# MurpheyLab/trep

Hardware: AMD Instinct MI355X
Metric: DEL-steps/sec x batch (puppet ~40-DOF, fp64) (higher is better)
Workload: dtype f64

## Files before the change

trep_amd/csrc/mvi_core.hpp:

```cpp
#pragma once
#include <cmath>

#include "program.hpp"
#include "dual.hpp"
#include "lanes.hpp"

#if defined(TG_MOCK_TIMING) || defined(TG_MOCK_REAL_LDS) || defined(TG_MOCK_LDS_D1) || defined(TG_MOCK_LDS_D2) || \
    defined(TG_BBD_FUSED_UPDATE) || defined(TG_BBD_INLINE) || defined(TG_BBD_ASM) || \
    defined(TG_WEV_NO_RC_IDENT) || defined(TG_WEV_CLEAR_EARLY) || defined(TG_WEV_MERGE_C) || \
    defined(TG_NO_BBD) || defined(TG_NO_CMP) || defined(TG_NO_GJ_PANEL) || defined(TG_NO_QUAD_SWEEP) || defined(TG_NO_DUAL_SWEEP) || \
    defined(TG_NO_AB_MFMA) || defined(TG_NO_HZ_MFMA) || defined(GJR_EXEC32) || defined(GJP_SKIP_STEPS) || defined(GJP_SKIP_UPDATE) || \
    defined(TG_FRESH_PHASES) || defined(TG_FRESH_STEP) || \
    defined(TG_CHAIN_PRIO) || defined(TG_PREFIX_GROUP) || defined(TG_LT_TRIPS) || defined(TG_ROLLOUT_WAVES) || defined(TG_DERIV_WAVES)
#error "a retired experiment switch is defined (TG_MOCK_*, TG_BBD_FUSED_UPDATE / _INLINE / _ASM, TG_WEV_*, TG_NO_* except TG_NO_WEV, GJR_ / GJP_*, TG_FRESH_*, or a former -D tunable): these variants were removed -- verdicts in docs/LOG.md, their source in commit 89f6ce0"
#endif

#if defined(TG_HELPER_WAVES)
constexpr int TG_NW = TG_HELPER_WAVES;
#else
constexpr int TG_NW = 1;
#endif

#if defined(__HIPCC__)
__device__ __forceinline__ double *tg_lds_base() {
#if defined(__HIP_DEVICE_COMPILE__)
    typedef __attribute__((address_space(3))) double lds_double;
    extern __shared__ double tg_dynamic_lds[];
    if ((__UINTPTR_TYPE__)(lds_double *)tg_dynamic_lds != 0) __builtin_trap();
    return (double *)((lds_double *)(__UINTPTR_TYPE__)8 - 1);
#else
    return nullptr;
#endif
}
#endif

TG_HD int tg_xcd_block(int b, int G) {
    const int q = G >> 3, r = G & 7, x = b & 7, i = b >> 3;
    const int n = q + (x < r ? 1 : 0);
    const int q2 = n >> 5, r2 = n & 31, u = i & 31, s_ = i >> 5;
    return x * q + (x < r ? x : r) + u * q2 + (u < r2 ? u : r2) + s_;
}

#if defined(__HIP_DEVICE_COMPILE__)
__device__ __forceinline__ int tg_opaque(int x) { asm volatile("" : "+v"(x)); return x; }
#else
inline int tg_opaque(int x) { return x; }
#endif
constexpr int TG_CHAIN_PRIO = 2;
constexpr int TG_PREFIX_GROUP = 5;
constexpr int TG_LT_TRIPS = 4;
#define TG_FOR(idx, n) for (int idx = tg_opaque(lane); idx < (n); idx += TEAM)
#define TG_FORW(idx, n) for (int idx = tg_opaque(lane + TEAM * wave); idx < (n); idx += TEAM * nw)

#if defined(TG_PROFILE) && defined(__HIP_DEVICE_COMPILE__)
#define TG_STAMP(id) do { long long t_ = (long long)__builtin_amdgcn_s_memtime(); prof[id] += t_ - prof_last; prof_last = t_; } while (0)
#ifndef TG_PROF_TRAJ
#define TG_PROF_TRAJ 0
#endif
#else
#define TG_STAMP(id) ((void)0)
#endif

#include <type_traits>
#include "bbd_solve.hpp"
#include "gj_solve.hpp"

namespace tg {
template <class P, class = void> struct tg_static_bbd { static constexpr bool value = false; };
template <class P> struct tg_static_bbd<P, typename std::enable_if<(P::bbd_ok >= 0)>::type> { static constexpr bool value = P::bbd_ok != 0; };
template <bool USE, class P, class = void> struct tg_static_bbd_cols { static constexpr int value = 1; };
template <class P> struct tg_static_bbd_cols<true, P, typename std::enable_if<(P::bbd_ok > 0)>::type> { static constexpr int value = P::bbd_ng + P::bbd_nb; };
template <class P, class = void> struct tg_is_spec { static constexpr bool value = false; };
template <class P> struct tg_is_spec<P, typename std::enable_if<(P::nq >= 0)>::type> { static constexpr bool value = true; };
template <class P, class = void> struct tg_items_aligned { static constexpr bool value = false; };
template <class P> struct tg_items_aligned<P, typename std::enable_if<(P::nq >= 0)>::type> { static constexpr bool value = (P::o_J % 2 == 0) && (P::o_W % 2 == 0); };
template <class P, class = void> struct tg_static_sweep { static constexpr bool value = false; };
template <class P> struct tg_static_sweep<P, typename std::enable_if<(P::sw_ok > 0)>::type> { static constexpr bool value = true; };
template <class P, class = void> struct tg_static_cmp { static constexpr bool value = false; };
template <class P> struct tg_static_cmp<P, typename std::enable_if<(P::cmp_ok >= 0)>::type> { static constexpr bool value = P::cmp_ok != 0 && P::tab_ok != 0; };

template <class P, class = void> struct tg_static_wev { static constexpr bool value = false; };
#if !defined(TG_NO_WEV)
template <class P> struct tg_static_wev<P, typename std::enable_if<(P::wev_ok >= 0)>::type> { static constexpr bool value = P::wev_ok != 0 && P::cmp_ok != 0 && P::tab_ok != 0; };
#endif

template <class P, class = void> struct tg_static_pk { static constexpr bool value = false; };
#if defined(TG_BBD_PACKED)
template <class P> struct tg_static_pk<P, typename std::enable_if<(P::bbd_pk_ok >= 0)>::type> { static constexpr bool value = P::bbd_pk_ok != 0 && tg_static_wev<P>::value && tg_static_bbd<P>::value; };
#endif

template <class P, class = void> struct tg_static_fb { static constexpr bool value = false; };
template <class P> struct tg_static_fb<P, typename std::enable_if<(P::fb_on >= 0)>::type> { static constexpr bool value = P::fb_on != 0 && tg_static_wev<P>::value; };

enum { MODE_ROLLOUT = 0, MODE_CALC_P2 = 1, MODE_CALC_F = 2, MODE_DERIV1 = 3, MODE_DERIV2Z = 4, MODE_DYNAMICS = 5, MODE_DYN_DERIV1 = 6, MODE_ENERGY = 7, MODE_LAGRANGIAN = 8 };

struct RunArgs {
    int batch, n_steps, max_iterations, mode;
    int predictor;
    double dt, t1, t2, tolerance;
    double *q1, *q2, *p1, *p2, *lam, *u1;
    const double *U, *K;
    const double *q2_hint, *lam_hint;
    const double *Kproj, *bX, *bU;
    double *Uout;
    int group_size;
    const int *group_map;
    double *X;
    double *f_out;
    double *d1[12];
    double *A_out, *B_out;
    const double *z;
    double *hz;
    int *iters, *status;
    long long *prof_out;
    const double *dt_steps;
    int dt_period;
    int exact_pivot;
    const double *zl;
    const double *dq_in, *ddqk_in;
    double *ddq_out, *lam_out;
    double *g1[8];
    double *energy_out;
    double *lag1_out, *lag2_out;
    double *mirror;
    int remap_len, remap_stride, remap_off, remap_count;
    int *fallbacks;
    const int *seed1, *seed2;
};
struct ParTable {
    const double *rows;
    int group, stride;
};
template <class ARGS> TG_HD int tg_remap_trajectory(const ARGS &A, int i) {
    if (A.remap_len <= 0) return i;
    return i < A.remap_count ? (i / A.remap_len) * A.remap_stride + A.remap_off + i % A.remap_len : A.batch;
}

#if defined(__HIP_DEVICE_COMPILE__)
typedef const __attribute__((address_space(4))) DevProg CProg;
typedef const RunArgs CArgs;
template <class T> __device__ __forceinline__ T &tg_fresh_always(T &r) { T *p = &r; asm volatile("" : "+s"(p)); return *p; }
typedef const __attribute__((address_space(4))) RunArgs KArgs;
__device__ __forceinline__ KArgs &tg_fresh_args(KArgs &r) { return tg_fresh_always(r); }
template <class T> __device__ __forceinline__ T &tg_fresh_args(T &r) { return r; }
template <class T> __device__ __forceinline__ T &tg_rebind(T &r) { return r; }
#else
typedef const DevProg CProg;
typedef const RunArgs CArgs;
typedef const RunArgs KArgs;
template <class T> inline T &tg_fresh_args(T &r) { return r; }
template <class T> inline T &tg_rebind(T &r) { return r; }
#endif

TG_HD void tg_sincos(double x, double *s, double *c) {
    if (!(fabs(x) < 131072.0)) {
#if defined(__HIP_DEVICE_COMPILE__)
        sincos(x, s, c);
#else
        *s = std::sin(x);
        *c = std::cos(x);
#endif
        return;
    }
    const double kf = rint(x * 6.36619772367581382433e-01);
    double r = fma(-kf, 1.57079632673412561417e+00, x);
    r = fma(-kf, 6.07710050630396597660e-11, r);
    const double t = fma(-kf, 2.02226624871116645580e-21, r);
    const double z = t * t;
    const double ps = fma(z, fma(z, fma(z, fma(z, fma(z, 1.58969099521155010221e-10, -2.50507602534068634195e-08),
                      2.75573137070700676789e-06), -1.98412698298579493134e-04), 8.33333333332248946124e-03), -1.66666666666666324348e-01);
    const double sn = fma(t * z, ps, t);
    const double pc = fma(z, fma(z, fma(z, fma(z, fma(z, -1.13596475577881948265e-11, 2.08757232129817482790e-09),
                      -2.75573143513906633035e-07), 2.48015872894767294178e-05), -1.38888888888741095749e-03), 4.16666666666666019037e-02);
    const double cs = fma(z * z, pc, fma(-0.5, z, 1.0));
    const int q = (int)kf & 3;
// ... 75 lines not shown
    TG_HD int n_wpair() const { return SPRINGS ? P.n_wpair : 0; }
    const double *d2w = nullptr;
    PROG &P;
    Real *S;
    int lane;
    int seed1 = -1, seed2 = -1;
    TG_HD Real seeded(double v, int var) const { return tgdual::Seed<Real>::make(v, var == seed1, var == seed2); }
    double dt;
    int oGc;
    int dsA = 0, dsB = 2;
    int jck[2] = {0, 0}, bio[2] = {0, 0}, tck[2][2] = {{0, 0}, {0, 0}}, tpair[4] = {0, 0, 0, 0};
    int sc_rot2 = 0;
    int sj_n = 0;
    bool sj_quads = false;
    int swc[16] = {0, 0, 0, 0, 0, 0, 0, 0, 0, 0, 0, 0, 0, 0, 0, 0}, swr = 0, swcol = 0;
    bool swact = false;
    double tdamp = 0.0;
    const double *par = nullptr;
    template <class PP> TG_HD double grav_of(PP &Pl, int k) const { if constexpr (PAR) return par[k]; else return Pl.grav[k]; }
    template <class PP> TG_HD double damp_of(PP &Pl, int i) const { if constexpr (PAR) return par[3 + i]; else return Pl.damp[i]; }
    int wvl[4] = {0, 0, 0, 0}, wpair[4] = {0, 0, 0, 0};
    int wfb[2] = {0, 0};
    int wdhx[2] = {0, 0}, wrhs = 0, wone = -1;
    double wev_w[6] = {0.0, 0.0, 0.0, 0.0, 0.0, 0.0};
    bool pk_image = false;
    bool wev_on = false;
    long long prof[16] = {0, 0, 0, 0, 0, 0, 0, 0, 0, 0, 0, 0, 0, 0, 0, 0};
    bool rates_ready = false;
    double res_f2 = 0.0;
    bool res_hoff = false;
    long long prof_last = 0;

    bool d1_compact = false;
    int wave = 0, nw = 1;
    TG_HD void wave_part(int first, int split, int last, int &lo, int &hi) const {
        lo = first; hi = last;
        if (nw > 1) { lo = wave ? split : first; hi = wave ? last : split; }
    }
    TG_HD Core(PROG &p, Real *s, int l, double dt_) : P(p), S(s), lane(l), dt(dt_), oGc(p.o_G), inv_dt(1.0 / dt_) {}
    double inv_dt;
    TG_HD double over_dt(double x) const { const double q = x * inv_dt; return fma(fma(-q, dt, x), inv_dt, q); }

    template <class Compute, class Store>
    TG_HD void for_pairs(int n, Compute compute, Store store) {
        for (int i0 = tg_opaque(lane); i0 < n; i0 += 2 * TEAM) {
            const int i1 = i0 + TEAM;
            const bool two = i1 < n;
            const auto r0 = compute(i0);
            const auto r1 = compute(two ? i1 : i0);
            store(i0, r0);
            if (two) store(i1, r1);
        }
    }

    TG_HD Real qval(int sel, int c) const {
        Real a = S[P.o_q1 + c], b = S[P.o_q2 + c];
        return sel == 0 ? 0.5 * (b + a) : (sel == 1 ? a : b);
    }

    TG_HD void init_sweep_schedule(bool rollout = false) {
        if constexpr (PAR) { TG_FOR(i, 4 * P.n_bodies) S[P.o_I + i] = par[i - 4 * P.n_bodies]; }
        else TG_FOR(i, 4 * P.n_bodies) S[P.o_I + i] = P.b_inertia[i];
        TG_FOR(c, P.nc) S[P.o_ctol + c] = P.c_tol[c];
#if defined(__HIP_DEVICE_COMPILE__)
        if constexpr (TEAM == 64 && tg_static_bbd<typename std::remove_cv<PROG>::type>::value) {
            if (rollout) { int *tab = (int *)(S + P.o_bbd); TG_FOR(i, 128) tab[i] = P.bbd_tab[i]; }
        }
        if constexpr (TEAM == 64 && !SPRINGS && tg_static_cmp<typename std::remove_cv<PROG>::type>::value) {
            if (rollout) { int *tab = (int *)(S + P.o_cmpt); TG_FOR(i, P.nd) { const int it = P.cmp_rep[i]; tab[i] = it | (P.it_pack[4 * (size_t)it] << 12) | (P.cmp_grp[i] << 20); } }
        }
        if (TEAM == 64 && P.tab_ok) {
            sj_n = rollout ? P.n_sj : 2 * P.n_joints;
            if (rollout) sc_rot2 = P.n_sj_rot;
            else { int n_rot = 0; for (int j = 0; j < P.n_joints; j++) n_rot += P.j_kind[j] >= TG_RX ? 1 : 0; sc_rot2 = 2 * n_rot; }
            sj_quads = rollout;
            if constexpr (tg_static_sweep<typename std::remove_cv<PROG>::type>::value) {
                typedef typename std::remove_cv<PROG>::type SP;
                if (rollout) {
                    const int l = tg_opaque(lane);
                    swact = l < 60;
                    const int q = swact ? l / 12 : 4, rc = swact ? l - 12 * q : 0;
                    swr = rc >> 2; swcol = rc & 3;
#pragma unroll
                    for (int i = 0; i < 16; i++) swc[i] = (i & 3) < SP::sw_np[i >> 2] ? sw_code<SP>(i * 5, q) : 15;
                }
            }
#pragma unroll
            for (int u = 0; u < 2; u++) {
                const int pos = lane + u * TEAM;
                jck[u] = pos < sj_n ? (rollout ? P.sj_list[pos] : P.sj_full[pos]) : 0;
                const int n = lane + u * TEAM < P.n_dhr ? lane + u * TEAM : 0;
                if (P.n_dhr) { tck[u][0] = P.dhr_pack[8 * (size_t)n] | (P.dhr_pack[8 * (size_t)n + 7] << 8); tck[u][1] = P.dhr_pack[8 * (size_t)n + 1]; }
            }
            const int b = lane < 6 * P.n_bodies ? lane / 6 : 0;
            bio[0] = P.b_item_off[b]; bio[1] = P.b_item_off[b + 1];
            tdamp = damp_of(P, lane < P.nd ? lane : 0);
            if constexpr (tg_static_wev<typename std::remove_cv<PROG>::type>::value) {
                typedef typename std::remove_cv<PROG>::type SP;
                static_assert((SP::n_cmpairs + TEAM - 1) / TEAM <= 4, "eval_world: at most four trips of config pairs");
                if (rollout) {
#pragma unroll
                    for (int i = 0; i < 4; i++) wvl[i] = P.wev_lane[4 * lane + i];
                    constexpr bool FB = tg_static_fb<SP>::value;
                    constexpr int NP = FB ? SP::fb_npairs : SP::n_cmpairs;
                    const int *pairs = FB ? P.fb_pair : P.cmp_pair, *pairsx = FB ? P.fb_pairx : P.wev_pairx;
                    if constexpr (FB) {
#pragma unroll
                        for (int i = 0; i < 3; i++) wvl[i] = P.fb_lane[4 * lane + i];
#pragma unroll
                        for (int i = 0; i < 2; i++) wfb[i] = P.fb_abx[2 * (lane < SP::nd ? lane : 0) + i];
                        if (lane >= SP::nd) wfb[0] = 0;
                    }
                    constexpr int TP = FB ? (NP + TEAM - 1) / TEAM : 4;
#pragma unroll
                    for (int u = 0; u < TP; u++) wpair[u] = pairs[lane + u * TEAM < NP ? lane + u * TEAM : 0];
                    if constexpr (tg_static_pk<SP>::value) {
#pragma unroll
                        for (int u = 0; u < TP; u++) wpair[u] = pairsx[lane + u * TEAM < NP ? lane + u * TEAM : 0];
#pragma unroll
                        for (int u = 0; u < 2; u++) wdhx[u] = P.wev_dhx[lane + u * TEAM < SP::n_dhr ? lane + u * TEAM : 0];
                        wrhs = P.bbd_map[(lane < SP::nf ? lane : 0) * (SP::nf + 1) + SP::nf];
                        wone = lane < SP::bbd_pk_nones ? P.bbd_ones[lane < SP::bbd_pk_nones ? lane : 0] : -1;
                    }
                }
            }
            if (P.n_npairs) { const int *p0 = P.pair4 + 4 * (size_t)(lane < P.n_npairs ? lane : 0); tpair[0] = p0[0]; tpair[1] = p0[1]; tpair[2] = p0[2]; tpair[3] = p0[3]; }
        }
#endif
        if (!P.sched_ok || TEAM != 64) { TG_SYNC(); return; }
        int *sched = (int *)(S + P.o_sched);
        TG_FOR(idx, 16 * P.n_rounds) {
            const int r = idx >> 4, c = P.round_off[r] + (idx & 15);
            int w0 = 0, w1 = -1;
            if (c < P.round_off[r + 1]) {
                w0 = (12 * P.ch_first[c]) | (P.ch_len[c] << 16);
                w1 = P.ch_parent[c] >= 0 ? 12 * P.ch_parent[c] : -1;
            }
            sched[2 * idx] = w0; sched[2 * idx + 1] = w1;
        }
        TG_SYNC();
    }

    TG_HD void pose_sweep(bool on, int sel) {
        Real *sc = S + P.o_sc, *G = S + P.o_G;
        if (on) TG_FOR(j, P.n_joints) {
            const Real x = qval(sel, P.j_cfg[j]);
            if (P.j_kind[j] >= TG_RX) tg_sincos(x, &sc[2 * j], &sc[2 * j + 1]);
            else { sc[2 * j] = x; sc[2 * j + 1] = 0.0; }
        }
        TG_SYNC();
        if (on) {
            const int n12 = 12 * P.n_joints;
            for (int base = lane; base < n12; base += 4 * TEAM) {
                double k0[4], k1[4], k2[4];
                int jj[4];
#pragma unroll
                for (int u = 0; u < 4; u++) {
                    const int idx = base + u * TEAM;
                    const bool ok = idx < n12;
                    const int j = ok ? idx / 12 : 0, e = ok ? idx % 12 : 0;
                    const double *k = P.jcoef + 4 * (size_t)(16 * j + e);
                    k0[u] = k[0]; k1[u] = k[1]; k2[u] = k[2]; jj[u] = j;
                }
#pragma unroll
                for (int u = 0; u < 4; u++) {
                    const int idx = base + u * TEAM;
                    if (idx < n12) G[idx] = k0[u] + k1[u] * sc[2 * jj[u] + 1] + k2[u] * sc[2 * jj[u]];
                }
            }
        }
        TG_SYNC();
#if defined(__HIP_DEVICE_COMPILE__)
        if (TEAM == 64) {
            const int *sched = (const int *)(S + P.o_sched);
            for (int r = 0; r < P.n_rounds; r++) {
                const int nch = P.sched_ok ? 16 : P.round_off[r + 1] - P.round_off[r];
                if (on) TG_FOR(idx, 4 * nch) {
                    const int row = idx & 3;
                    int o0, len, opar;
                    if (P.sched_ok) {
                        const int w0 = sched[2 * (16 * r + (idx >> 2))];
                        opar = sched[2 * (16 * r + (idx >> 2)) + 1];
                        o0 = w0 & 0xFFFF; len = w0 >> 16;
                    } else {
                        const int ch = P.round_off[r] + (idx >> 2);
                        o0 = 12 * P.ch_first[ch]; len = P.ch_len[ch]; opar = P.ch_parent[ch] >= 0 ? 12 * P.ch_parent[ch] : -1;
                    }
                    if (row < 3 && len > 0) {
                        Real p0, p1, p2, p3;
                        if (opar >= 0) { const Real *gp = G + opar + 4 * row; p0 = gp[0]; p1 = gp[1]; p2 = gp[2]; p3 = gp[3]; }
                        else { p0 = row == 0 ? 1.0 : 0.0; p1 = row == 1 ? 1.0 : 0.0; p2 = row == 2 ? 1.0 : 0.0; p3 = 0.0; }
                        Real m[12];
#pragma unroll
                        for (int e = 0; e < 12; e++) m[e] = G[o0 + e];
                        for (int s = 0; s < len; s++) {
                            Real *gj = G + o0 + 12 * s;
                            Real n[12];
                            const Real *gn = s + 1 < len ? gj + 12 : gj;
#pragma unroll
                            for (int e = 0; e < 12; e++) n[e] = gn[e];
                            const Real v0 = p0 * m[0] + p1 * m[4] + p2 * m[8];
                            const Real v1 = p0 * m[1] + p1 * m[5] + p2 * m[9];
                            const Real v2 = p0 * m[2] + p1 * m[6] + p2 * m[10];
                            const Real v3 = p0 * m[3] + p1 * m[7] + p2 * m[11] + p3;
                            Real *out = gj + 4 * row;
                            out[0] = v0; out[1] = v1; out[2] = v2; out[3] = v3;
                            p0 = v0; p1 = v1; p2 = v2; p3 = v3;
#pragma unroll
                            for (int e = 0; e < 12; e++) m[e] = n[e];
                        }
                    }
                }
                TG_SYNC();
            }
            return;
        }
#endif
        for (int L = 1; L < P.n_levels; L++) {
            const int l0 = P.level_off[L], cnt = P.level_off[L + 1] - l0;
            if (on) TG_FOR(idx, 4 * cnt) {
                const int j = P.lvl_joints[l0 + (idx >> 2)], cc = idx & 3;
                if (P.j_parent[j] < 0) continue;
                const Real *gp = G + 12 * P.j_parent[j];
                Real *gj = G + 12 * j;
                const Real m0 = gj[cc], m1 = gj[4 + cc], m2 = gj[8 + cc], u3 = (cc == 3) ? 1.0 : 0.0;
                const Real v0 = gp[0] * m0 + gp[1] * m1 + gp[2] * m2 + u3 * gp[3];
                const Real v1 = gp[4] * m0 + gp[5] * m1 + gp[6] * m2 + u3 * gp[7];
                const Real v2 = gp[8] * m0 + gp[9] * m1 + gp[10] * m2 + u3 * gp[11];
                gj[cc] = v0; gj[4 + cc] = v1; gj[8 + cc] = v2;
            }
            TG_SYNC();
        }
    }

#if defined(__HIP_DEVICE_COMPILE__)
    TG_HD void pose_sweep_dual(bool on, bool rollout_lists) {
        const int sjn = rollout_lists ? P.n_sj : 2 * P.n_joints;
        double *sc = S + P.o_sc, *sc2 = S + P.o_J, *G = S + P.o_G, *G2 = S + P.o_W;
        const int nj = P.n_joints;
        const int n12 = 12 * nj, n24 = 2 * n12;
        SwDesc sw0;
        if constexpr (tg_static_sweep<typename std::remove_cv<PROG>::type>::value) {
            if (rollout_lists) sw0 = sw_fetch<typename std::remove_cv<PROG>::type, 0>((const int *)(S + P.o_sched));
        }
        if (P.tab_ok) {
            double pr[2][12];
#pragma unroll
            for (int u = 0; u < 2; u++) {
                const double *src = P.j_prm + 12 * (size_t)((jck[u] >> 16) & 0xFFF);
#pragma unroll
                for (int e = 0; e < 12; e++) pr[u][e] = src[e];
            }
            if (on) {
#pragma unroll
                for (int u = 0; u < 2; u++) {
                    const int idx = lane + u * TEAM;
                    if (u * TEAM < sjn && idx < sjn) {
                        const bool second = (jck[u] >> 28) != 0;
                        const int j = (jck[u] >> 16) & 0xFFF, kind = (jck[u] >> 12) & 0xF;
                        const double x = qval(second ? dsB : dsA, jck[u] & 0xFFF);
                        const bool rotary = kind >= TG_RX;
                        const int a = rotary ? kind - TG_RX : kind - TG_TX, b = a == 2 ? 0 : a + 1, c = a == 0 ? 2 : a - 1;
                        double *g = (second ? G2 : G) + 12 * j;
                        if (u * TEAM < sc_rot2) {
                            double sn = 0.0, cs = 1.0;
                            if (rotary) tg_sincos(x, &sn, &cs);
                            const double tq = rotary ? 0.0 : x;
#pragma unroll
                            for (int l = 0; l < 3; l++) {
                                const double A_ = pr[u][4 * l], B_ = pr[u][4 * l + 1], C_ = pr[u][4 * l + 2], D_ = pr[u][4 * l + 3];
                                g[4 * l + a] = A_;
                                g[4 * l + b] = rotary ? fma(C_, sn, B_ * cs) : B_;
                                g[4 * l + c] = rotary ? fma(-B_, sn, C_ * cs) : C_;
                                g[4 * l + 3] = fma(A_, tq, D_);
                            }
                        } else {
#pragma unroll
                            for (int l = 0; l < 3; l++) {
                                const double A_ = pr[u][4 * l], B_ = pr[u][4 * l + 1], C_ = pr[u][4 * l + 2], D_ = pr[u][4 * l + 3];
                                g[4 * l + a] = A_; g[4 * l + b] = B_; g[4 * l + c] = C_;
                                g[4 * l + 3] = fma(A_, x, D_);
                            }
                        }
                    }
                }
            }
            TG_SYNC();
            TG_STAMP(5);
            TG_STAMP(15);
        } else {
        constexpr int LT = TG_LT_TRIPS;
        struct Rows { double k0[LT], k1[LT], k2[LT]; int j[LT]; };
        auto rows_of = [&](int first) {
            Rows r;
#pragma unroll
            for (int u = 0; u < LT; u++) {
                const int idx2 = first + u * TEAM;
                const int idx = idx2 < n24 ? (idx2 >= n12 ? idx2 - n12 : idx2) : 0;
                const int j = idx / 12, e = idx % 12;
                const double *k = P.jcoef + 4 * (size_t)(16 * j + e);
                r.k0[u] = k[0]; r.k1[u] = k[1]; r.k2[u] = k[2]; r.j[u] = j;
            }
            return r;
        };
        Rows cur = rows_of(lane);
        if (on) TG_FOR(idx, 2 * nj) {
            const bool second = idx >= nj;
            const int j = second ? idx - nj : idx;
            const double x = qval(second ? dsB : dsA, P.j_cfg[j]);
            double *dst = (second ? sc2 : sc) + 2 * j;
            if (P.j_kind[j] >= TG_RX) tg_sincos(x, &dst[0], &dst[1]);
            else { dst[0] = x; dst[1] = 0.0; }
        }
        TG_SYNC();
        TG_STAMP(5);
        for (int b0 = 0; b0 < n24; b0 += LT * TEAM) {
            const Rows nxt = b0 + LT * TEAM < n24 ? rows_of(b0 + LT * TEAM + lane) : cur;
            if (on) {
#pragma unroll
                for (int u = 0; u < LT; u++) {
                    const int idx2 = b0 + lane + u * TEAM;
                    if (idx2 < n24) {
                        const bool second = idx2 >= n12;
                        const double *scx = second ? sc2 : sc;
                        (second ? G2 : G)[second ? idx2 - n12 : idx2] = cur.k0[u] + cur.k1[u] * scx[2 * cur.j[u] + 1] + cur.k2[u] * scx[2 * cur.j[u]];
                    }
                }
            }
            cur = nxt;
        }
        TG_SYNC();
        TG_STAMP(15);
        }
        const int *sched = (const int *)(S + P.o_sched);
        if constexpr (tg_static_sweep<typename std::remove_cv<PROG>::type>::value) {
            if (rollout_lists) {
                typedef typename std::remove_cv<PROG>::type SP;
                __builtin_amdgcn_s_setprio(TG_CHAIN_PRIO);
                chain_round_quads<SP, 0>(on, sched, sw0);
                __builtin_amdgcn_s_setprio(0);
                return;
            }
        }
        if (P.sched_ok == 2) {
            double *Gh = lane >= 32 ? G2 : G;
            const int slot = (lane & 31) >> 2, row = lane & 3;
            for (int r = 0; r < P.n_rounds; r++) {
                if (on) {
                    const int w0 = sched[2 * (16 * r + slot)];
                    const int opar = sched[2 * (16 * r + slot) + 1];
                    const int o0 = w0 & 0xFFFF, len = w0 >> 16;
                    if (row < 3 && len > 0) {
                        double p0, p1, p2, p3;
                        if (opar >= 0) { const double *gp = Gh + opar + 4 * row; p0 = gp[0]; p1 = gp[1]; p2 = gp[2]; p3 = gp[3]; }
                        else { p0 = row == 0 ? 1.0 : 0.0; p1 = row == 1 ? 1.0 : 0.0; p2 = row == 2 ? 1.0 : 0.0; p3 = 0.0; }
                        double m[12];
#pragma unroll
                        for (int e = 0; e < 12; e++) m[e] = Gh[o0 + e];
                        for (int s = 0; s < len; s++) {
                            double *gj = Gh + o0 + 12 * s;
                            double n[12];
                            const int nx = s + 1 < len ? 12 : 0;
#pragma unroll
                            for (int e = 0; e < 12; e++) n[e] = gj[nx + e];
                            const double v0 = p0 * m[0] + p1 * m[4] + p2 * m[8];
                            const double v1 = p0 * m[1] + p1 * m[5] + p2 * m[9];
                            const double v2 = p0 * m[2] + p1 * m[6] + p2 * m[10];
                            const double v3 = p0 * m[3] + p1 * m[7] + p2 * m[11] + p3;
                            double *out = gj + 4 * row;
                            out[0] = v0; out[1] = v1; out[2] = v2; out[3] = v3;
                            p0 = v0; p1 = v1; p2 = v2; p3 = v3;
#pragma unroll
                            for (int e = 0; e < 12; e++) m[e] = n[e];
                        }
                    }
                }
                TG_SYNC();
            }
            return;
        }
        for (int r = 0; r < P.n_rounds; r++) {
            if (on) TG_FOR(idx, 64) {
                const int row = idx & 3;
                const int w0 = sched[2 * (16 * r + (idx >> 2))];
                const int opar = sched[2 * (16 * r + (idx >> 2)) + 1];
                const int o0 = w0 & 0xFFFF, len = w0 >> 16;
                if (row < 3 && len > 0) {
                    double p0, p1, p2, p3, q0, q1, q2, q3;
                    if (opar >= 0) {
                        const double *gp = G + opar + 4 * row, *gq = G2 + opar + 4 * row;
                        p0 = gp[0]; p1 = gp[1]; p2 = gp[2]; p3 = gp[3]; q0 = gq[0]; q1 = gq[1]; q2 = gq[2]; q3 = gq[3];
                    } else {
                        p0 = q0 = row == 0 ? 1.0 : 0.0; p1 = q1 = row == 1 ? 1.0 : 0.0; p2 = q2 = row == 2 ? 1.0 : 0.0; p3 = q3 = 0.0;
                    }
                    double m[12], h[12];
#pragma unroll
                    for (int e = 0; e < 12; e++) { m[e] = G[o0 + e]; h[e] = G2[o0 + e]; }
                    for (int s = 0; s < len; s++) {
                        double *gj = G + o0 + 12 * s, *hj = G2 + o0 + 12 * s;
                        double n[12], g[12];
                        const int nxt = s + 1 < len ? 12 : 0;
#pragma unroll
                        for (int e = 0; e < 12; e++) { n[e] = gj[nxt + e]; g[e] = hj[nxt + e]; }
                        const double v0 = p0 * m[0] + p1 * m[4] + p2 * m[8];
                        const double w0_ = q0 * h[0] + q1 * h[4] + q2 * h[8];
                        const double v1 = p0 * m[1] + p1 * m[5] + p2 * m[9];
                        const double w1 = q0 * h[1] + q1 * h[5] + q2 * h[9];
                        const double v2 = p0 * m[2] + p1 * m[6] + p2 * m[10];
                        const double w2 = q0 * h[2] + q1 * h[6] + q2 * h[10];
                        const double v3 = p0 * m[3] + p1 * m[7] + p2 * m[11] + p3;
                        const double w3 = q0 * h[3] + q1 * h[7] + q2 * h[11] + q3;
                        double *out = gj + 4 * row, *out2 = hj + 4 * row;
                        out[0] = v0; out[1] = v1; out[2] = v2; out[3] = v3;
                        out2[0] = w0_; out2[1] = w1; out2[2] = w2; out2[3] = w3;
                        p0 = v0; p1 = v1; p2 = v2; p3 = v3; q0 = w0_; q1 = w1; q2 = w2; q3 = w3;
#pragma unroll
                        for (int e = 0; e < 12; e++) { m[e] = n[e]; h[e] = g[e]; }
                    }
                }
            }
            TG_SYNC();
        }
    }
    struct SwDesc { int w0[4], par[4]; };
    template <class SP> TG_HD static int sw_code(int base, int q) {
        auto w = [&](int i) { const int c = SP::sw_inst[base + i]; return c ? (c & 0x1FF) : 15; };
        return q == 0 ? w(0) : q == 1 ? w(1) : q == 2 ? w(2) : q == 3 ? w(3) : w(4);
    }
    template <class SP, int RD> TG_HD SwDesc sw_fetch(const int *sched) const {
        SwDesc d;
#pragma unroll
        for (int ps = 0; ps < 4; ps++) {
            d.w0[ps] = 0; d.par[ps] = -1;
            if (ps < SP::sw_np[RD < 4 ? RD : 0]) {
                const int slot = swc[4 * (RD < 4 ? RD : 0) + ps] & 0xFF;
                d.w0[ps] = sched[2 * (16 * RD + slot)]; d.par[ps] = sched[2 * (16 * RD + slot) + 1];
            }
        }
        return d;
    }
    template <class SP, int RD> TG_HD void chain_round_quads(bool on, const int *sched, const SwDesc &d) {
        if constexpr (RD < SP::n_rounds) {
            constexpr int NP = SP::sw_np[RD], ML = SP::sw_maxlen;
            SwDesc nxt = d;
            if constexpr (RD + 1 < SP::n_rounds) nxt = sw_fetch<SP, RD + 1>(sched);
            const int r = swr, c = swcol;
            const bool act = swact;
            if (on) {
                double m[4][ML][3], p[4];
                int base[4], lim[4];
                const int dead = P.o_sc + (lane < 2 * P.n_joints ? lane : 0);
#pragma unroll
                for (int ps = 0; ps < 4; ps++) {
                    if (ps < NP) {
                        const int set = (swc[4 * RD + ps] >> 8) ? P.o_W : P.o_G, opar = d.par[ps];
                        lim[ps] = act ? d.w0[ps] >> 16 : 0;
                        base[ps] = set + (d.w0[ps] & 0xFFFF);
                        const double pv = S[set + (opar >= 0 ? opar : 0) + 4 * r + c];
                        p[ps] = opar >= 0 ? pv : (r == c ? 1.0 : 0.0);
#pragma unroll
                        for (int s = 0; s < ML; s++) {
                            if (s < SP::sw_len[4 * RD + ps]) {
                                const int o = base[ps] + 12 * s + c;
                                m[ps][s][0] = S[o]; m[ps][s][1] = S[o + 4]; m[ps][s][2] = S[o + 8];
                            }
                        }
                    }
                }
#pragma unroll
                for (int s = 0; s < ML; s++) {
#pragma unroll
                    for (int ps = 0; ps < 4; ps++) {
                        if (ps < NP && s < SP::sw_len[4 * RD + ps]) {
                            const double b0 = tg_quad_bcast<0>(p[ps]), b1 = tg_quad_bcast<1>(p[ps]), b2 = tg_quad_bcast<2>(p[ps]);
                            const double last = c == 3 ? p[ps] : 0.0;
                            const double v = fma(b2, m[ps][s][2], fma(b1, m[ps][s][1], fma(b0, m[ps][s][0], last)));
                            S[s < lim[ps] ? base[ps] + 12 * s + 4 * r + c : dead] = v;
                            p[ps] = v;
                        }
                    }
                }
            }
            TG_SYNC();
            chain_round_quads<SP, RD + 1>(on, sched, nxt);
        }
    }
    TG_HD bool dual_ok() const { return TEAM == 64 && !SPRINGS && P.sched_ok && P.nc > 0 && 6 * P.n_items >= 12 * P.n_joints; }

    TG_HD void eval_both(bool on) {
        if (on) TG_FOR(i, P.nq) S[P.o_dq + i] = (S[P.o_q2 + i] - S[P.o_q1 + i]) / dt;
        TG_SYNC();
        TG_STAMP(0);
        pose_sweep_dual(on, true);
        TG_STAMP(1);
        oGc = P.o_W;
        attach_points(on, true, true);
        constraints(on, 2, true, S + P.o_Dh2, 0);
        oGc = P.o_G;
        TG_STAMP(6);
        jacobians(on);
        TG_STAMP(2);
        velocities(on);
        TG_STAMP(3);
        residual_dyn(on);
        TG_STAMP(4);
    }
    struct AttachTab { double ce[2], c0[2], c1[2], c2[2]; int ga[2]; double o0, o1, o2, orr; int ea; };
    struct ConTab { int e1, e2, type, comp, cfg; double dist; int rec[2][6]; };
    struct ItemTab { int rec[2][4]; };
    struct ResTab { int n0, n1; int look[8]; };
    TG_HD AttachTab fetch_attach() const {
        AttachTab t;
        const int l = tg_opaque(lane);
#pragma unroll
        for (int u = 0; u < 2; u++) {
            const int ii = l + u * TEAM < 12 * P.n_bodies ? l + u * TEAM : 0;
            const double *C = P.at_d + 4 * (size_t)ii;
            t.ce[u] = C[0]; t.c0[u] = C[1]; t.c1[u] = C[2]; t.c2[u] = C[3]; t.ga[u] = P.at_i[ii];
        }
        const int ii = l < 3 * P.n_endpoints ? l : 0;
        const double *o = P.ae_d + 4 * (size_t)ii;
        t.o0 = o[0]; t.o1 = o[1]; t.o2 = o[2]; t.orr = o[3]; t.ea = P.ae_i[ii];
        return t;
    }
    TG_HD ConTab fetch_constraints() const {
        ConTab t;
        const int l = tg_opaque(lane);
        const int c = l < P.nc ? l : 0;
        t.e1 = P.c_e1[c]; t.e2 = P.c_e2[c]; t.type = P.c_type[c]; t.comp = P.c_comp[c]; t.cfg = P.c_cfg[c]; t.dist = P.c_dist[c];
#pragma unroll
        for (int u = 0; u < 2; u++) {
            const int *rec = P.dhr_pack + 8 * (size_t)(l + u * TEAM < P.n_dhr ? l + u * TEAM : 0);
#pragma unroll
            for (int i = 1; i < 6; i++) t.rec[u][i] = rec[i];
            t.rec[u][0] = rec[7];
        }
        return t;
    }
    TG_HD ItemTab fetch_items() const {
        ItemTab t;
        const int l = tg_opaque(lane);
#pragma unroll
        for (int u = 0; u < 2; u++) {
            const int *rec = P.it_pack + 4 * (size_t)(l + u * TEAM < P.n_items ? l + u * TEAM : 0);
#pragma unroll
            for (int i = 0; i < 4; i++) t.rec[u][i] = rec[i];
        }
        return t;
    }
    TG_HD ResTab fetch_residual() const {
        ResTab t;
        const int l = tg_opaque(lane);
        const int i = l < P.nd ? l : 0;
        t.n0 = P.cfg_item_off[i]; t.n1 = P.cfg_item_off[i + 1];
#pragma unroll
        for (int c = 0; c < 8; c++) t.look[c] = c < P.nc ? P.dh_lookup[c * P.nq + i] : -1;
// ... 3381 lines not shown
```

trep_amd/csrc/program.hpp:

```cpp
#pragma once
#include <cmath>
#include <cstdlib>
#include <cstdint>
#include <algorithm>
#include <cstring>
#include <functional>
#include <map>
#include <stdexcept>
#include <string>
#include <vector>

#include "../../include/trep_amd.h"
#include "bbd.hpp"

namespace tg {

struct DevProg {
    int nq, nd, nk, nu, nc, nf, nX;
    int n_joints, n_levels, n_bodies, n_items, n_pairs, n_endpoints, n_dh, n_cf, n_cfgitems;
    double grav[3];
    const int *level_off;
    const int *lvl_joints;
    const int *round_off, *ch_first, *ch_len, *ch_parent;
    int n_rounds, n_chains;
// ... 8 lines not shown
    const double *b_C;
    const double *b_inertia;
    const int *b_item_off;
    const int *b_pair_off;
    const int *it_body;
    const int *it_joint;
    const int *it_cfg;
    const int *pair_a;
    const int *pair_b;
    const int *pair4;
    int n_npairs;
    const int *tri4, *cpair4;
    const int *it_pack, *dh_pack;
    const double *at_d, *ae_d;
    const int *at_i, *ae_i;
    const int *dhr_pack;
    int n_dhr;
    const int *cpath_off, *cpath_items, *dh_pos;
    int n_cpath, o_cps;
    const int *tchunk, *tri_off;
    int n_tchunk, o_tps;
    int n_tri, n_cpair;
    const int *wp_a, *wp_b, *wt_a, *wt_b, *wt_split, *wcp4;
    int wp_split, wc_split;
    const int *cfg_item_off;
    const int *cfg_items;
    const int *it_slot;
    const int *e_anchor;
    const double *e_off;
    const int *c_type, *c_e1, *c_e2, *c_cfg, *c_comp;
    const double *c_dist, *c_tol;
    const int *dh_lookup;
    const int *dh_c, *dh_cfg, *dh_joint, *dh_side;
    const double *damp;
    const int *cf_cfg, *cf_in;
    int o_q1, o_q2, o_p1, o_lam, o_u, o_dq, o_f, o_sc, o_G, o_gB, o_pE, o_J, o_W, o_vB, o_gam, o_Ldq, o_Lddq,
        o_Dh1, o_Dh2, o_Df, o_scal, o_misc, o_dqi, o_nu, o_sched, o_I, o_ctol, gjc_ok;
    int tab_ok;
    int sched_ok;
    int df_ld;
    int dh_ld;
    int lds_per_team;
    int d_o_Dh1, d_o_Dh2, d_o_AUG, d_aug_ld, d_o_T12, d_o_T22, d_nrhs, d_lds_per_team;
    const int *cu_off;
    const double *cs_k, *cs_kq0;
    const double *s_k, *s_x0;
    int n_springs, n_sdh, n_spair, o_sV, o_sH, has_cs;
    int g_nrhs, g_ld, g_o_AUG, g_o_P, g_o_X, g_o_aF, g_o_x, g_lds_per_team, g_max_cu;
    const double *c_nloc;
    int has_plane, o_nE;
    const int *wr_in; const double *wr_const;
    const int *wr_kind;
    const double *wr_Rloc; int o_wR;
    int n_wrenches, n_wdh, n_wpair, o_wF, o_wH, o_wD, e_o_wT, e_o_Hu;
    const double *s_c; int has_damper, o_sX, o_sVq, o_sXX, o_svel, o_sF;
    int n_true_springs, e_o_sT, e_o_sWX, e_o_sWXq;
    const int *tab_i; const double *tab_d; int n_tab_i, n_tab_d;
    int e_o_H11, e_o_H12, e_o_H22, e_o_G1, e_o_w, e_o_zq, e_o_zp, e_o_vec, e_o_vec2, e_lds_per_team;
    const double *cs_c0;
    const int *ncs_i; const double *ncs_mb, *ncs_tab; int n_ncs;
    int cmp_ok, n_cgroups, n_cmpairs, o_cmp, o_csw, o_ccz, o_cmpt;
    int cmp_gmask[32];
    const int *cmp_rep, *cmp_grp, *cmp_goff, *cmp_gbody, *cmp_pair;
    int sw_ok, sw_maxlen;
    int sw_np[4];
    int sw_len[16];
    int sw_inst[80];
    int n_sj, n_sj_rot;
    const int *sj_list;
    const int *sj_full;
    int max_cfg_items;
    int bbd_ok, bbd_g, bbd_ng, bbd_nb, bbd_t, o_bbd;
    int bbd_tvar[16];
    const int *bbd_tab;
    int wev_ok, wev_depth, wev_rc_ident;
    const int *wev_lane;
    int bbd_pk_ok, bbd_pk_nr, bbd_pk_nc2, bbd_pk_tb, bbd_pk_tc2, bbd_pk_xs, bbd_pk_size, bbd_pk_nones;
    const int *bbd_map, *bbd_ones, *wev_pairx, *wev_dhx;
    int fb_n, fb_on, fb_npairs, fb_depth, dhr_sides, dhr_types;
    int fb_cfg[3];
    int fb_axis[3];
    const int *fb_pair, *fb_pairx, *fb_abx, *fb_lane;
    int a_ok, a_o_T12, a_o_AUG, a_aug_ld, a_o_T22, a_lds_per_team;
};

struct HostProgram {
    DevProg p{};
    std::vector<int> level_off, lvl_joints, round_off, ch_first, ch_len, ch_parent, j_parent, j_kind, j_cfg, j_pre_ident;
    std::vector<double> j_pre;
    std::vector<int> b_anchor;
    std::vector<double> b_C, b_inertia;
    std::vector<int> b_item_off, b_pair_off, it_body, it_joint, it_cfg, pair_a, pair_b, cfg_item_off, cfg_items, it_slot, pair4, tri4, cpair4, it_pack, dh_pack, cpath_off, cpath_items, dh_pos, tchunk, tri_off, dhr_pack, at_i, ae_i, sj_list, sj_full;
    std::vector<int> wp_a, wp_b, wt_a, wt_b, wt_split, wcp4;
    std::vector<int> e_anchor;
    std::vector<double> e_off;
    std::vector<int> c_type, c_e1, c_e2, c_cfg, c_comp;
    std::vector<double> c_dist, c_tol;
    std::vector<int> dh_c, dh_cfg, dh_joint, dh_side, dh_lookup, cu_off;
    std::vector<double> damp, cs_k, cs_kq0, cs_c0, s_k, s_x0, s_c, c_nloc, wr_const, wr_Rloc, ncs_mb, ncs_tab;
    std::vector<int> ncs_i, bbd_tab, cmp_rep, cmp_grp, cmp_goff, cmp_gbody, cmp_pair, wev_lane, bbd_map, bbd_ones, wev_pairx, wev_dhx;
    std::vector<int> fb_pair, fb_pairx, fb_abx, fb_lane;
    std::vector<unsigned char> newton_pattern;
    std::vector<int> wr_in, wr_kind;
    std::vector<int> cf_cfg, cf_in;
    std::vector<double> jcoef;
    std::vector<double> at_d, ae_d;
    std::vector<double> j_prm;
    int max_depth = 0;
    std::vector<int> ipool;
    std::vector<double> dpool;
    std::vector<size_t> ioff, doff;
    void pack();
    void bind(DevProg &P, const int *I, const double *D) const;
};

namespace detail {
struct M34 {
    double m[12];
};
inline M34 ident() {
    M34 r{};
    r.m[0] = r.m[5] = r.m[10] = 1.0;
    return r;
}
inline M34 mul(const M34 &a, const M34 &b) {
    M34 r{};
    for (int i = 0; i < 3; i++)
        for (int j = 0; j < 4; j++) {
            double s = (j == 3) ? a.m[4 * i + 3] : 0.0;
            for (int k = 0; k < 3; k++) s += a.m[4 * i + k] * b.m[4 * k + j];
            r.m[4 * i + j] = s;
        }
    return r;
}
inline bool is_ident(const M34 &a) {
    M34 i = ident();
    return std::memcmp(a.m, i.m, sizeof(a.m)) == 0;
}
inline M34 fixed_local(const tg_system_desc *d, int f) {
    int t = d->frame_transform[f];
    M34 r = ident();
    double x = d->frame_value[f];
    if (t == TG_CONST_SE3) {
        std::memcpy(r.m, d->frame_lg + 12 * (size_t)f, sizeof(r.m));
    } else if (t == TG_TX || t == TG_TY || t == TG_TZ) {
        r.m[4 * (t - TG_TX) + 3] = x;
    } else if (t == TG_RX) {
        r.m[5] = std::cos(x); r.m[6] = -std::sin(x); r.m[9] = std::sin(x); r.m[10] = std::cos(x);
    } else if (t == TG_RY) {
        r.m[0] = std::cos(x); r.m[2] = std::sin(x); r.m[8] = -std::sin(x); r.m[10] = std::cos(x);
    } else if (t == TG_RZ) {
        r.m[0] = std::cos(x); r.m[1] = -std::sin(x); r.m[4] = std::sin(x); r.m[5] = std::cos(x);
    }
    return r;
}
}

inline HostProgram build_program(const tg_system_desc *d) {
    using namespace detail;
    HostProgram H;
    const int nfr = d->n_frames, nq = d->n_configs, nd = d->n_dyn, nc = d->n_constraints;
    if (nd + d->n_kin != nq) throw std::runtime_error("n_dyn + n_kin != n_configs");
    for (int f = 0; f < nfr; f++) {
        int t = d->frame_transform[f];
        if (t < TG_WORLD || t > TG_CONST_SE3) throw std::runtime_error("unknown frame transform");
        if (d->frame_config[f] >= 0 && (t < TG_TX || t > TG_RZ)) throw std::runtime_error("config on a non-parametric frame");
        if (f > 0 && (d->frame_parent[f] < 0 || d->frame_parent[f] >= f)) throw std::runtime_error("frames must be listed parent-first");
    }
    std::vector<int> jframes;
    int n_levels = 0;
    for (int f = 0; f < nfr; f++)
        if (d->frame_config[f] >= 0) {
            jframes.push_back(f);
            n_levels = std::max(n_levels, d->config_gen[d->frame_config[f]] + 1);
        }
    std::vector<int> order;
    {
        std::vector<int> vparent(nfr, -1);
        std::vector<int> nearest(nfr, -1);
        for (int f = 1; f < nfr; f++) {
            const int p = d->frame_parent[f];
            vparent[f] = nearest[p];
            nearest[f] = d->frame_config[f] >= 0 ? f : nearest[p];
        }
// ... 626 lines not shown
                    H.fb_abx[2 * b] = (int)((unsigned)m << 30);
                }
                if ((int)H.cmp_pair.size() - P.fb_npairs != closed || listed != closed) throw std::runtime_error("floating-base prefix: pair bookkeeping error");
            }
        }
    }
    {
        const int nf = P.nf;
        H.bbd_tab.assign(128, 0);
        for (int i = 0; i < 16; i++) P.bbd_tvar[i] = 0;
        P.bbd_ok = 0; P.bbd_g = P.bbd_ng = P.bbd_nb = P.bbd_t = 0; P.o_bbd = 0;
        if (nf >= 17 && nf <= 31 && nd >= 2) {
            std::vector<unsigned char> pat((size_t)nf * nf, 0);
            auto mark = [&](int i, int j) { if (i < nf && j < nf) { pat[(size_t)i * nf + j] = 1; pat[(size_t)j * nf + i] = 1; } };
            for (int i = 0; i < nd; i++) mark(i, i);
            for (int n = 0; n < P.n_npairs; n++) mark(H.pair4[4 * n + 2] & 0xFFFF, H.pair4[4 * n + 2] >> 16);
            for (int n = 0; n < n_dh_con; n++) if (H.dh_cfg[n] < nd) mark(H.dh_cfg[n], nd + H.dh_c[n]);
            for (size_t n = (size_t)n_cpair_con; n < H.cpair4.size() / 4; n++) {
                const int ka = H.cpair4[4 * n + 3] & 0xFFFF, kb = H.cpair4[4 * n + 3] >> 16;
                if (ka < nd && kb < nd) mark(ka, kb);
            }
            H.newton_pattern = pat;
            const BbdPlan plan = bbd_plan(nf, nd, pat);
            if (plan.ok && plan.t * (plan.t + 2) <= 12 * nitems) {
                P.bbd_ok = 1; P.bbd_g = plan.g; P.bbd_ng = plan.ng; P.bbd_nb = plan.nb; P.bbd_t = plan.t;
                H.bbd_tab.assign(plan.tab, plan.tab + 128);
                for (int i = 0; i < 16; i++) P.bbd_tvar[i] = plan.tvar[i];
                P.o_bbd = P.lds_per_team;
                P.lds_per_team += 64;
            }
        }
        {
            P.bbd_pk_ok = 0; P.bbd_pk_nr = P.bbd_pk_nc2 = P.bbd_pk_tb = P.bbd_pk_tc2 = P.bbd_pk_xs = P.bbd_pk_size = P.bbd_pk_nones = 0;
            H.bbd_map.assign(1, -1); H.bbd_ones.assign(1, -1); H.wev_pairx.assign(1, 0); H.wev_dhx.assign(1, 0);
            if (P.bbd_ok && P.wev_ok) {
                BbdPlan plan;
                plan.ok = 1; plan.g = P.bbd_g; plan.ng = P.bbd_ng; plan.nb = P.bbd_nb; plan.t = P.bbd_t;
                for (int i = 0; i < 16; i++) plan.tvar[i] = P.bbd_tvar[i];
                for (int i = 0; i < 128; i++) plan.tab[i] = H.bbd_tab[i];
                const BbdPacked K = bbd_pack(plan, nf);
                bool ok = K.ok && K.size <= P.nf * P.df_ld && K.size < 1024 && nd < 64 && P.n_dh < 256 && (int)K.ones.size() <= 64 &&
                          P.bbd_t * (P.bbd_t + 2) <= 17 * nb;
                std::vector<int> pairx, dhx;
                for (int n = 0; n < P.n_cmpairs && ok; n++) {
                    const int a = H.cmp_pair[n] & 0xFFFF, b = H.cmp_pair[n] >> 16;
                    const int ab = K.map[(size_t)a * (nf + 1) + b], ba = K.map[(size_t)b * (nf + 1) + a];
                    if (ab < 0 || ba < 0) { ok = false; break; }
                    pairx.push_back((int)((unsigned)a | ((unsigned)b << 6) | ((unsigned)ab << 12) | ((unsigned)ba << 22)));
                }
                for (int n = 0; n < P.n_dhr && ok; n++) {
                    const int c = H.dhr_pack[8 * (size_t)n], k = H.dhr_pack[8 * (size_t)n + 1], item = H.dhr_pack[8 * (size_t)n + 7];
                    const int kc = K.map[(size_t)k * (nf + 1) + nd + c], ck = K.map[(size_t)(nd + c) * (nf + 1) + k];
                    if (kc < 0 || ck < 0) { ok = false; break; }
                    dhx.push_back(item | (kc << 8) | (ck << 18));
                }
                for (int i = 0; i < nf && ok; i++) if (K.map[(size_t)i * (nf + 1) + nf] < 0) ok = false;
                if (ok) {
                    P.bbd_pk_ok = 1; P.bbd_pk_nr = K.nr; P.bbd_pk_nc2 = K.nc2; P.bbd_pk_tb = K.tb; P.bbd_pk_tc2 = K.tc2; P.bbd_pk_xs = P.o_scal - P.o_Df; P.bbd_pk_size = K.size;
                    P.bbd_pk_nones = K.ones[0] < 0 ? 0 : (int)K.ones.size();
                    H.bbd_map = K.map; H.bbd_ones = K.ones; H.wev_pairx = pairx.empty() ? std::vector<int>(1, 0) : pairx; H.wev_dhx = dhx.empty() ? std::vector<int>(1, 0) : dhx;
                    if (P.fb_on) {
                        H.fb_pairx.clear();
                        for (int w : H.fb_pair) {
                            const int a = w & 0xFFFF, b = w >> 16;
                            H.fb_pairx.push_back((int)((unsigned)a | ((unsigned)b << 6) | ((unsigned)K.map[(size_t)a * (nf + 1) + b] << 12) | ((unsigned)K.map[(size_t)b * (nf + 1) + a] << 22)));
                        }
                        for (int b = 0; b < nd; b++) {
                            const int m = (int)((unsigned)H.fb_abx[2 * b] >> 30);
                            unsigned at[6] = {0, 0, 0, 0, 0, 0};
                            for (int i = 0; i < m; i++) { at[2 * i] = (unsigned)K.map[(size_t)P.fb_cfg[i] * (nf + 1) + b]; at[2 * i + 1] = (unsigned)K.map[(size_t)b * (nf + 1) + P.fb_cfg[i]]; }
                            H.fb_abx[2 * b] = (int)(at[0] | (at[1] << 10) | (at[2] << 20) | ((unsigned)m << 30));
                            H.fb_abx[2 * b + 1] = (int)(at[3] | (at[4] << 10) | (at[5] << 20));
                        }
                    }
                }
            }
        }
        if (P.cmp_ok) {
            P.o_cmpt = P.lds_per_team;
            P.lds_per_team += (nd + 1) / 2;
            P.lds_per_team = (P.lds_per_team + 1) & ~1;
        }
    }
    H.pack();
    return H;
}

}

namespace tg {
namespace detail {
template <typename T>
inline void pool_append(std::vector<T> &pool, std::vector<size_t> &offs, const std::vector<T> &v) {
    offs.push_back(pool.size());
    pool.insert(pool.end(), v.begin(), v.end());
    while (pool.size() % 4) pool.push_back(T());
}
}

#define TG_INT_TABLES(X)                                                                                     \
    X(level_off) X(lvl_joints) X(round_off) X(ch_first) X(ch_len) X(ch_parent) X(j_parent) X(j_kind) X(j_cfg) X(j_pre_ident) X(b_anchor) X(b_item_off) X(b_pair_off) X(it_body) \
    X(it_joint) X(it_cfg) X(pair_a) X(pair_b) X(cfg_item_off) X(cfg_items) X(e_anchor) X(c_type) X(c_e1) X(c_e2) \
    X(c_cfg) X(c_comp) X(dh_c) X(dh_cfg) X(dh_joint) X(dh_side) X(cf_cfg) X(cf_in) X(dh_lookup) X(cu_off) X(it_slot) X(pair4) \
    X(tri4) X(cpair4) X(it_pack) X(dh_pack) X(cpath_off) X(cpath_items) X(dh_pos) X(tchunk) X(tri_off) X(wr_in) X(wr_kind) X(ncs_i) \
    X(wp_a) X(wp_b) X(wt_a) X(wt_b) X(wt_split) X(wcp4) X(bbd_tab) X(cmp_rep) X(cmp_grp) X(cmp_goff) X(cmp_gbody) X(cmp_pair) X(dhr_pack) X(at_i) X(ae_i) X(sj_list) X(sj_full) X(wev_lane) X(bbd_map) X(bbd_ones) X(wev_pairx) X(wev_dhx) \
    X(fb_pair) X(fb_pairx) X(fb_abx) X(fb_lane)
#define TG_DBL_TABLES(X) X(j_pre) X(jcoef) X(j_prm) X(at_d) X(ae_d) X(b_C) X(b_inertia) X(e_off) X(c_dist) X(c_tol) X(damp) X(cs_k) X(cs_kq0) X(cs_c0) X(s_k) X(s_x0) X(c_nloc) X(wr_const) X(s_c) X(wr_Rloc) X(ncs_mb) X(ncs_tab)

inline void HostProgram::pack() {
    ipool.clear(); dpool.clear(); ioff.clear(); doff.clear();
#define X(name) detail::pool_append(ipool, ioff, name);
    TG_INT_TABLES(X)
#undef X
#define X(name) detail::pool_append(dpool, doff, name);
    TG_DBL_TABLES(X)
#undef X
    ipool.push_back(0); dpool.push_back(0.0);
}

inline void HostProgram::bind(DevProg &P, const int *I, const double *D) const {
    size_t k = 0;
#define X(name) P.name = I + ioff[k++];
    TG_INT_TABLES(X)
#undef X
    k = 0;
#define X(name) P.name = D + doff[k++];
    TG_DBL_TABLES(X)
#undef X
    P.tab_i = I; P.tab_d = D; P.n_tab_i = (int)ipool.size(); P.n_tab_d = (int)dpool.size();
}
}
```

trep_amd/csrc/spec_emit.inc:

```
static void emit_spec_header(const tg::HostProgram &H, std::string &out) {
    char line[256];
    tg::DevProg P = H.p;
    H.bind(P, H.ipool.data(), H.dpool.data());
    out += "// specialised schedule: sizes, counts, LDS offsets and tables as compile-time constants\n";
    std::snprintf(line, sizeof(line), "__device__ const int spec_ipool[%zu] = {", H.ipool.size() ? H.ipool.size() : (size_t)1); out += line;
    for (size_t i = 0; i < H.ipool.size(); i++) { std::snprintf(line, sizeof(line), "%s%d", i ? ((i % 32) ? "," : ",\n") : "\n", H.ipool[i]); out += line; }
    if (H.ipool.empty()) out += "0";
    out += "};\n";
    std::snprintf(line, sizeof(line), "__device__ const double spec_dpool[%zu] = {", H.dpool.size() ? H.dpool.size() : (size_t)1); out += line;
    for (size_t i = 0; i < H.dpool.size(); i++) { std::snprintf(line, sizeof(line), "%s%a", i ? ((i % 8) ? "," : ",\n") : "\n", H.dpool[i]); out += line; }
    if (H.dpool.empty()) out += "0";
    out += "};\n";
    out += "struct SpecProg {\n";
    std::snprintf(line, sizeof(line), "    static constexpr int nq = %d;\n", P.nq); out += line;
    std::snprintf(line, sizeof(line), "    static constexpr int nd = %d;\n", P.nd); out += line;
    std::snprintf(line, sizeof(line), "    static constexpr int nk = %d;\n", P.nk); out += line;
    std::snprintf(line, sizeof(line), "    static constexpr int nu = %d;\n", P.nu); out += line;
    std::snprintf(line, sizeof(line), "    static constexpr int nc = %d;\n", P.nc); out += line;
    std::snprintf(line, sizeof(line), "    static constexpr int nf = %d;\n", P.nf); out += line;
    std::snprintf(line, sizeof(line), "    static constexpr int nX = %d;\n", P.nX); out += line;
    std::snprintf(line, sizeof(line), "    static constexpr int n_joints = %d;\n", P.n_joints); out += line;
    std::snprintf(line, sizeof(line), "    static constexpr int n_levels = %d;\n", P.n_levels); out += line;
    std::snprintf(line, sizeof(line), "    static constexpr int n_bodies = %d;\n", P.n_bodies); out += line;
    std::snprintf(line, sizeof(line), "    static constexpr int n_items = %d;\n", P.n_items); out += line;
// ... 65 lines not shown
    std::snprintf(line, sizeof(line), "    static constexpr int g_ld = %d;\n", P.g_ld); out += line;
    std::snprintf(line, sizeof(line), "    static constexpr int g_o_AUG = %d;\n", P.g_o_AUG); out += line;
    std::snprintf(line, sizeof(line), "    static constexpr int g_o_P = %d;\n", P.g_o_P); out += line;
    std::snprintf(line, sizeof(line), "    static constexpr int g_o_X = %d;\n", P.g_o_X); out += line;
    std::snprintf(line, sizeof(line), "    static constexpr int g_o_aF = %d;\n", P.g_o_aF); out += line;
    std::snprintf(line, sizeof(line), "    static constexpr int g_o_x = %d;\n", P.g_o_x); out += line;
    std::snprintf(line, sizeof(line), "    static constexpr int g_lds_per_team = %d;\n", P.g_lds_per_team); out += line;
    std::snprintf(line, sizeof(line), "    static constexpr int g_max_cu = %d;\n", P.g_max_cu); out += line;
    std::snprintf(line, sizeof(line), "    static constexpr int has_plane = %d;\n", P.has_plane); out += line;
    std::snprintf(line, sizeof(line), "    static constexpr int o_nE = %d;\n", P.o_nE); out += line;
    std::snprintf(line, sizeof(line), "    static constexpr int o_wR = %d;\n", P.o_wR); out += line;
    std::snprintf(line, sizeof(line), "    static constexpr int n_wrenches = %d;\n", P.n_wrenches); out += line;
    std::snprintf(line, sizeof(line), "    static constexpr int n_wdh = %d;\n", P.n_wdh); out += line;
    std::snprintf(line, sizeof(line), "    static constexpr int n_wpair = %d;\n", P.n_wpair); out += line;
    std::snprintf(line, sizeof(line), "    static constexpr int o_wF = %d;\n", P.o_wF); out += line;
    std::snprintf(line, sizeof(line), "    static constexpr int o_wH = %d;\n", P.o_wH); out += line;
    std::snprintf(line, sizeof(line), "    static constexpr int o_wD = %d;\n", P.o_wD); out += line;
    std::snprintf(line, sizeof(line), "    static constexpr int e_o_wT = %d;\n", P.e_o_wT); out += line;
    std::snprintf(line, sizeof(line), "    static constexpr int e_o_Hu = %d;\n", P.e_o_Hu); out += line;
    std::snprintf(line, sizeof(line), "    static constexpr int has_damper = %d;\n", P.has_damper); out += line;
    std::snprintf(line, sizeof(line), "    static constexpr int o_sX = %d;\n", P.o_sX); out += line;
    std::snprintf(line, sizeof(line), "    static constexpr int o_sVq = %d;\n", P.o_sVq); out += line;
    std::snprintf(line, sizeof(line), "    static constexpr int o_sXX = %d;\n", P.o_sXX); out += line;
    std::snprintf(line, sizeof(line), "    static constexpr int o_svel = %d;\n", P.o_svel); out += line;
    std::snprintf(line, sizeof(line), "    static constexpr int o_sF = %d;\n", P.o_sF); out += line;
    std::snprintf(line, sizeof(line), "    static constexpr int n_true_springs = %d;\n", P.n_true_springs); out += line;
    std::snprintf(line, sizeof(line), "    static constexpr int e_o_sT = %d;\n", P.e_o_sT); out += line;
    std::snprintf(line, sizeof(line), "    static constexpr int e_o_sWX = %d;\n", P.e_o_sWX); out += line;
    std::snprintf(line, sizeof(line), "    static constexpr int e_o_sWXq = %d;\n", P.e_o_sWXq); out += line;
    std::snprintf(line, sizeof(line), "    static constexpr int n_tab_i = %d;\n", P.n_tab_i); out += line;
    std::snprintf(line, sizeof(line), "    static constexpr int n_tab_d = %d;\n", P.n_tab_d); out += line;
    std::snprintf(line, sizeof(line), "    static constexpr int e_o_H11 = %d;\n", P.e_o_H11); out += line;
    std::snprintf(line, sizeof(line), "    static constexpr int e_o_H12 = %d;\n", P.e_o_H12); out += line;
    std::snprintf(line, sizeof(line), "    static constexpr int e_o_H22 = %d;\n", P.e_o_H22); out += line;
    std::snprintf(line, sizeof(line), "    static constexpr int e_o_G1 = %d;\n", P.e_o_G1); out += line;
    std::snprintf(line, sizeof(line), "    static constexpr int e_o_w = %d;\n", P.e_o_w); out += line;
    std::snprintf(line, sizeof(line), "    static constexpr int e_o_zq = %d;\n", P.e_o_zq); out += line;
    std::snprintf(line, sizeof(line), "    static constexpr int e_o_zp = %d;\n", P.e_o_zp); out += line;
    std::snprintf(line, sizeof(line), "    static constexpr int e_o_vec = %d;\n", P.e_o_vec); out += line;
    std::snprintf(line, sizeof(line), "    static constexpr int e_o_vec2 = %d;\n", P.e_o_vec2); out += line;
    std::snprintf(line, sizeof(line), "    static constexpr int e_lds_per_team = %d;\n", P.e_lds_per_team); out += line;
    std::snprintf(line, sizeof(line), "    static constexpr int n_ncs = %d;\n", P.n_ncs); out += line;
    std::snprintf(line, sizeof(line), "    static constexpr int cmp_ok = %d;\n", P.cmp_ok); out += line;
    std::snprintf(line, sizeof(line), "    static constexpr int n_cgroups = %d;\n", P.n_cgroups); out += line;
    std::snprintf(line, sizeof(line), "    static constexpr int n_cmpairs = %d;\n", P.n_cmpairs); out += line;
    std::snprintf(line, sizeof(line), "    static constexpr int o_cmp = %d;\n", P.o_cmp); out += line;
    std::snprintf(line, sizeof(line), "    static constexpr int o_csw = %d;\n", P.o_csw); out += line;
    std::snprintf(line, sizeof(line), "    static constexpr int o_ccz = %d;\n", P.o_ccz); out += line;
    std::snprintf(line, sizeof(line), "    static constexpr int o_cmpt = %d;\n", P.o_cmpt); out += line;
    std::snprintf(line, sizeof(line), "    static constexpr int sw_ok = %d;\n", P.sw_ok); out += line;
    std::snprintf(line, sizeof(line), "    static constexpr int sw_maxlen = %d;\n", P.sw_maxlen); out += line;
    std::snprintf(line, sizeof(line), "    static constexpr int n_sj = %d;\n", P.n_sj); out += line;
    std::snprintf(line, sizeof(line), "    static constexpr int n_sj_rot = %d;\n", P.n_sj_rot); out += line;
    std::snprintf(line, sizeof(line), "    static constexpr int max_cfg_items = %d;\n", P.max_cfg_items); out += line;
    std::snprintf(line, sizeof(line), "    static constexpr int bbd_ok = %d;\n", P.bbd_ok); out += line;
    std::snprintf(line, sizeof(line), "    static constexpr int bbd_g = %d;\n", P.bbd_g); out += line;
    std::snprintf(line, sizeof(line), "    static constexpr int bbd_ng = %d;\n", P.bbd_ng); out += line;
    std::snprintf(line, sizeof(line), "    static constexpr int bbd_nb = %d;\n", P.bbd_nb); out += line;
    std::snprintf(line, sizeof(line), "    static constexpr int bbd_t = %d;\n", P.bbd_t); out += line;
    std::snprintf(line, sizeof(line), "    static constexpr int o_bbd = %d;\n", P.o_bbd); out += line;
    std::snprintf(line, sizeof(line), "    static constexpr int wev_ok = %d;\n", P.wev_ok); out += line;
    std::snprintf(line, sizeof(line), "    static constexpr int wev_depth = %d;\n", P.wev_depth); out += line;
    std::snprintf(line, sizeof(line), "    static constexpr int wev_rc_ident = %d;\n", P.wev_rc_ident); out += line;
    std::snprintf(line, sizeof(line), "    static constexpr int bbd_pk_ok = %d;\n", P.bbd_pk_ok); out += line;
    std::snprintf(line, sizeof(line), "    static constexpr int bbd_pk_nr = %d;\n", P.bbd_pk_nr); out += line;
    std::snprintf(line, sizeof(line), "    static constexpr int bbd_pk_nc2 = %d;\n", P.bbd_pk_nc2); out += line;
    std::snprintf(line, sizeof(line), "    static constexpr int bbd_pk_tb = %d;\n", P.bbd_pk_tb); out += line;
    std::snprintf(line, sizeof(line), "    static constexpr int bbd_pk_tc2 = %d;\n", P.bbd_pk_tc2); out += line;
    std::snprintf(line, sizeof(line), "    static constexpr int bbd_pk_xs = %d;\n", P.bbd_pk_xs); out += line;
    std::snprintf(line, sizeof(line), "    static constexpr int bbd_pk_size = %d;\n", P.bbd_pk_size); out += line;
    std::snprintf(line, sizeof(line), "    static constexpr int bbd_pk_nones = %d;\n", P.bbd_pk_nones); out += line;
    std::snprintf(line, sizeof(line), "    static constexpr int fb_n = %d;\n", P.fb_n); out += line;
    std::snprintf(line, sizeof(line), "    static constexpr int fb_on = %d;\n", P.fb_on); out += line;
    std::snprintf(line, sizeof(line), "    static constexpr int fb_npairs = %d;\n", P.fb_npairs); out += line;
    std::snprintf(line, sizeof(line), "    static constexpr int fb_depth = %d;\n", P.fb_depth); out += line;
    std::snprintf(line, sizeof(line), "    static constexpr int dhr_sides = %d;\n", P.dhr_sides); out += line;
    std::snprintf(line, sizeof(line), "    static constexpr int dhr_types = %d;\n", P.dhr_types); out += line;
    std::snprintf(line, sizeof(line), "    static constexpr int a_ok = %d;\n", P.a_ok); out += line;
    std::snprintf(line, sizeof(line), "    static constexpr int a_o_T12 = %d;\n", P.a_o_T12); out += line;
    std::snprintf(line, sizeof(line), "    static constexpr int a_o_AUG = %d;\n", P.a_o_AUG); out += line;
    std::snprintf(line, sizeof(line), "    static constexpr int a_aug_ld = %d;\n", P.a_aug_ld); out += line;
    std::snprintf(line, sizeof(line), "    static constexpr int a_o_T22 = %d;\n", P.a_o_T22); out += line;
    std::snprintf(line, sizeof(line), "    static constexpr int a_lds_per_team = %d;\n", P.a_lds_per_team); out += line;
    std::snprintf(line, sizeof(line), "    static constexpr double grav_0 = %a;\n", P.grav[0]); out += line;
    std::snprintf(line, sizeof(line), "    static constexpr double grav_1 = %a;\n", P.grav[1]); out += line;
    std::snprintf(line, sizeof(line), "    static constexpr double grav_2 = %a;\n", P.grav[2]); out += line;
    out += "    struct grav_t { __host__ __device__ constexpr double operator[](int i) const { return i == 0 ? grav_0 : i == 1 ? grav_1 : grav_2; } };\n";
    out += "    static constexpr grav_t grav{};\n";
    std::snprintf(line, sizeof(line), "    static constexpr int cmp_gmask_0 = %d;\n", P.cmp_gmask[0]); out += line;
    std::snprintf(line, sizeof(line), "    static constexpr int cmp_gmask_1 = %d;\n", P.cmp_gmask[1]); out += line;
    std::snprintf(line, sizeof(line), "    static constexpr int cmp_gmask_2 = %d;\n", P.cmp_gmask[2]); out += line;
    std::snprintf(line, sizeof(line), "    static constexpr int cmp_gmask_3 = %d;\n", P.cmp_gmask[3]); out += line;
    std::snprintf(line, sizeof(line), "    static constexpr int cmp_gmask_4 = %d;\n", P.cmp_gmask[4]); out += line;
    std::snprintf(line, sizeof(line), "    static constexpr int cmp_gmask_5 = %d;\n", P.cmp_gmask[5]); out += line;
    std::snprintf(line, sizeof(line), "    static constexpr int cmp_gmask_6 = %d;\n", P.cmp_gmask[6]); out += line;
    std::snprintf(line, sizeof(line), "    static constexpr int cmp_gmask_7 = %d;\n", P.cmp_gmask[7]); out += line;
    std::snprintf(line, sizeof(line), "    static constexpr int cmp_gmask_8 = %d;\n", P.cmp_gmask[8]); out += line;
    std::snprintf(line, sizeof(line), "    static constexpr int cmp_gmask_9 = %d;\n", P.cmp_gmask[9]); out += line;
    std::snprintf(line, sizeof(line), "    static constexpr int cmp_gmask_10 = %d;\n", P.cmp_gmask[10]); out += line;
    std::snprintf(line, sizeof(line), "    static constexpr int cmp_gmask_11 = %d;\n", P.cmp_gmask[11]); out += line;
    std::snprintf(line, sizeof(line), "    static constexpr int cmp_gmask_12 = %d;\n", P.cmp_gmask[12]); out += line;
    std::snprintf(line, sizeof(line), "    static constexpr int cmp_gmask_13 = %d;\n", P.cmp_gmask[13]); out += line;
    std::snprintf(line, sizeof(line), "    static constexpr int cmp_gmask_14 = %d;\n", P.cmp_gmask[14]); out += line;
    std::snprintf(line, sizeof(line), "    static constexpr int cmp_gmask_15 = %d;\n", P.cmp_gmask[15]); out += line;
    std::snprintf(line, sizeof(line), "    static constexpr int cmp_gmask_16 = %d;\n", P.cmp_gmask[16]); out += line;
    std::snprintf(line, sizeof(line), "    static constexpr int cmp_gmask_17 = %d;\n", P.cmp_gmask[17]); out += line;
    std::snprintf(line, sizeof(line), "    static constexpr int cmp_gmask_18 = %d;\n", P.cmp_gmask[18]); out += line;
    std::snprintf(line, sizeof(line), "    static constexpr int cmp_gmask_19 = %d;\n", P.cmp_gmask[19]); out += line;
    std::snprintf(line, sizeof(line), "    static constexpr int cmp_gmask_20 = %d;\n", P.cmp_gmask[20]); out += line;
    std::snprintf(line, sizeof(line), "    static constexpr int cmp_gmask_21 = %d;\n", P.cmp_gmask[21]); out += line;
    std::snprintf(line, sizeof(line), "    static constexpr int cmp_gmask_22 = %d;\n", P.cmp_gmask[22]); out += line;
    std::snprintf(line, sizeof(line), "    static constexpr int cmp_gmask_23 = %d;\n", P.cmp_gmask[23]); out += line;
    std::snprintf(line, sizeof(line), "    static constexpr int cmp_gmask_24 = %d;\n", P.cmp_gmask[24]); out += line;
    std::snprintf(line, sizeof(line), "    static constexpr int cmp_gmask_25 = %d;\n", P.cmp_gmask[25]); out += line;
    std::snprintf(line, sizeof(line), "    static constexpr int cmp_gmask_26 = %d;\n", P.cmp_gmask[26]); out += line;
    std::snprintf(line, sizeof(line), "    static constexpr int cmp_gmask_27 = %d;\n", P.cmp_gmask[27]); out += line;
    std::snprintf(line, sizeof(line), "    static constexpr int cmp_gmask_28 = %d;\n", P.cmp_gmask[28]); out += line;
    std::snprintf(line, sizeof(line), "    static constexpr int cmp_gmask_29 = %d;\n", P.cmp_gmask[29]); out += line;
    std::snprintf(line, sizeof(line), "    static constexpr int cmp_gmask_30 = %d;\n", P.cmp_gmask[30]); out += line;
    std::snprintf(line, sizeof(line), "    static constexpr int cmp_gmask_31 = %d;\n", P.cmp_gmask[31]); out += line;
    out += "    struct cmp_gmask_t { __host__ __device__ constexpr int operator[](int i) const { return i == 0 ? cmp_gmask_0 : i == 1 ? cmp_gmask_1 : i == 2 ? cmp_gmask_2 : i == 3 ? cmp_gmask_3 : i == 4 ? cmp_gmask_4 : i == 5 ? cmp_gmask_5 : i == 6 ? cmp_gmask_6 : i == 7 ? cmp_gmask_7 : i == 8 ? cmp_gmask_8 : i == 9 ? cmp_gmask_9 : i == 10 ? cmp_gmask_10 : i == 11 ? cmp_gmask_11 : i == 12 ? cmp_gmask_12 : i == 13 ? cmp_gmask_13 : i == 14 ? cmp_gmask_14 : i == 15 ? cmp_gmask_15 : i == 16 ? cmp_gmask_16 : i == 17 ? cmp_gmask_17 : i == 18 ? cmp_gmask_18 : i == 19 ? cmp_gmask_19 : i == 20 ? cmp_gmask_20 : i == 21 ? cmp_gmask_21 : i == 22 ? cmp_gmask_22 : i == 23 ? cmp_gmask_23 : i == 24 ? cmp_gmask_24 : i == 25 ? cmp_gmask_25 : i == 26 ? cmp_gmask_26 : i == 27 ? cmp_gmask_27 : i == 28 ? cmp_gmask_28 : i == 29 ? cmp_gmask_29 : i == 30 ? cmp_gmask_30 : cmp_gmask_31; } };\n";
    out += "    static constexpr cmp_gmask_t cmp_gmask{};\n";
    std::snprintf(line, sizeof(line), "    static constexpr int sw_np_0 = %d;\n", P.sw_np[0]); out += line;
    std::snprintf(line, sizeof(line), "    static constexpr int sw_np_1 = %d;\n", P.sw_np[1]); out += line;
    std::snprintf(line, sizeof(line), "    static constexpr int sw_np_2 = %d;\n", P.sw_np[2]); out += line;
    std::snprintf(line, sizeof(line), "    static constexpr int sw_np_3 = %d;\n", P.sw_np[3]); out += line;
    out += "    struct sw_np_t { __host__ __device__ constexpr int operator[](int i) const { return i == 0 ? sw_np_0 : i == 1 ? sw_np_1 : i == 2 ? sw_np_2 : sw_np_3; } };\n";
    out += "    static constexpr sw_np_t sw_np{};\n";
    std::snprintf(line, sizeof(line), "    static constexpr int sw_len_0 = %d;\n", P.sw_len[0]); out += line;
    std::snprintf(line, sizeof(line), "    static constexpr int sw_len_1 = %d;\n", P.sw_len[1]); out += line;
    std::snprintf(line, sizeof(line), "    static constexpr int sw_len_2 = %d;\n", P.sw_len[2]); out += line;
    std::snprintf(line, sizeof(line), "    static constexpr int sw_len_3 = %d;\n", P.sw_len[3]); out += line;
    std::snprintf(line, sizeof(line), "    static constexpr int sw_len_4 = %d;\n", P.sw_len[4]); out += line;
    std::snprintf(line, sizeof(line), "    static constexpr int sw_len_5 = %d;\n", P.sw_len[5]); out += line;
    std::snprintf(line, sizeof(line), "    static constexpr int sw_len_6 = %d;\n", P.sw_len[6]); out += line;
    std::snprintf(line, sizeof(line), "    static constexpr int sw_len_7 = %d;\n", P.sw_len[7]); out += line;
    std::snprintf(line, sizeof(line), "    static constexpr int sw_len_8 = %d;\n", P.sw_len[8]); out += line;
    std::snprintf(line, sizeof(line), "    static constexpr int sw_len_9 = %d;\n", P.sw_len[9]); out += line;
    std::snprintf(line, sizeof(line), "    static constexpr int sw_len_10 = %d;\n", P.sw_len[10]); out += line;
    std::snprintf(line, sizeof(line), "    static constexpr int sw_len_11 = %d;\n", P.sw_len[11]); out += line;
    std::snprintf(line, sizeof(line), "    static constexpr int sw_len_12 = %d;\n", P.sw_len[12]); out += line;
    std::snprintf(line, sizeof(line), "    static constexpr int sw_len_13 = %d;\n", P.sw_len[13]); out += line;
    std::snprintf(line, sizeof(line), "    static constexpr int sw_len_14 = %d;\n", P.sw_len[14]); out += line;
    std::snprintf(line, sizeof(line), "    static constexpr int sw_len_15 = %d;\n", P.sw_len[15]); out += line;
    out += "    struct sw_len_t { __host__ __device__ constexpr int operator[](int i) const { return i == 0 ? sw_len_0 : i == 1 ? sw_len_1 : i == 2 ? sw_len_2 : i == 3 ? sw_len_3 : i == 4 ? sw_len_4 : i == 5 ? sw_len_5 : i == 6 ? sw_len_6 : i == 7 ? sw_len_7 : i == 8 ? sw_len_8 : i == 9 ? sw_len_9 : i == 10 ? sw_len_10 : i == 11 ? sw_len_11 : i == 12 ? sw_len_12 : i == 13 ? sw_len_13 : i == 14 ? sw_len_14 : sw_len_15; } };\n";
    out += "    static constexpr sw_len_t sw_len{};\n";
    std::snprintf(line, sizeof(line), "    static constexpr int sw_inst_0 = %d;\n", P.sw_inst[0]); out += line;
    std::snprintf(line, sizeof(line), "    static constexpr int sw_inst_1 = %d;\n", P.sw_inst[1]); out += line;
    std::snprintf(line, sizeof(line), "    static constexpr int sw_inst_2 = %d;\n", P.sw_inst[2]); out += line;
    std::snprintf(line, sizeof(line), "    static constexpr int sw_inst_3 = %d;\n", P.sw_inst[3]); out += line;
    std::snprintf(line, sizeof(line), "    static constexpr int sw_inst_4 = %d;\n", P.sw_inst[4]); out += line;
    std::snprintf(line, sizeof(line), "    static constexpr int sw_inst_5 = %d;\n", P.sw_inst[5]); out += line;
    std::snprintf(line, sizeof(line), "    static constexpr int sw_inst_6 = %d;\n", P.sw_inst[6]); out += line;
    std::snprintf(line, sizeof(line), "    static constexpr int sw_inst_7 = %d;\n", P.sw_inst[7]); out += line;
    std::snprintf(line, sizeof(line), "    static constexpr int sw_inst_8 = %d;\n", P.sw_inst[8]); out += line;
    std::snprintf(line, sizeof(line), "    static constexpr int sw_inst_9 = %d;\n", P.sw_inst[9]); out += line;
    std::snprintf(line, sizeof(line), "    static constexpr int sw_inst_10 = %d;\n", P.sw_inst[10]); out += line;
    std::snprintf(line, sizeof(line), "    static constexpr int sw_inst_11 = %d;\n", P.sw_inst[11]); out += line;
    std::snprintf(line, sizeof(line), "    static constexpr int sw_inst_12 = %d;\n", P.sw_inst[12]); out += line;
    std::snprintf(line, sizeof(line), "    static constexpr int sw_inst_13 = %d;\n", P.sw_inst[13]); out += line;
    std::snprintf(line, sizeof(line), "    static constexpr int sw_inst_14 = %d;\n", P.sw_inst[14]); out += line;
    std::snprintf(line, sizeof(line), "    static constexpr int sw_inst_15 = %d;\n", P.sw_inst[15]); out += line;
    std::snprintf(line, sizeof(line), "    static constexpr int sw_inst_16 = %d;\n", P.sw_inst[16]); out += line;
    std::snprintf(line, sizeof(line), "    static constexpr int sw_inst_17 = %d;\n", P.sw_inst[17]); out += line;
    std::snprintf(line, sizeof(line), "    static constexpr int sw_inst_18 = %d;\n", P.sw_inst[18]); out += line;
    std::snprintf(line, sizeof(line), "    static constexpr int sw_inst_19 = %d;\n", P.sw_inst[19]); out += line;
// ... 7 lines not shown
    std::snprintf(line, sizeof(line), "    static constexpr int sw_inst_27 = %d;\n", P.sw_inst[27]); out += line;
    std::snprintf(line, sizeof(line), "    static constexpr int sw_inst_28 = %d;\n", P.sw_inst[28]); out += line;
    std::snprintf(line, sizeof(line), "    static constexpr int sw_inst_29 = %d;\n", P.sw_inst[29]); out += line;
    std::snprintf(line, sizeof(line), "    static constexpr int sw_inst_30 = %d;\n", P.sw_inst[30]); out += line;
    std::snprintf(line, sizeof(line), "    static constexpr int sw_inst_31 = %d;\n", P.sw_inst[31]); out += line;
    std::snprintf(line, sizeof(line), "    static constexpr int sw_inst_32 = %d;\n", P.sw_inst[32]); out += line;
    std::snprintf(line, sizeof(line), "    static constexpr int sw_inst_33 = %d;\n", P.sw_inst[33]); out += line;
    std::snprintf(line, sizeof(line), "    static constexpr int sw_inst_34 = %d;\n", P.sw_inst[34]); out += line;
    std::snprintf(line, sizeof(line), "    static constexpr int sw_inst_35 = %d;\n", P.sw_inst[35]); out += line;
    std::snprintf(line, sizeof(line), "    static constexpr int sw_inst_36 = %d;\n", P.sw_inst[36]); out += line;
    std::snprintf(line, sizeof(line), "    static constexpr int sw_inst_37 = %d;\n", P.sw_inst[37]); out += line;
    std::snprintf(line, sizeof(line), "    static constexpr int sw_inst_38 = %d;\n", P.sw_inst[38]); out += line;
    std::snprintf(line, sizeof(line), "    static constexpr int sw_inst_39 = %d;\n", P.sw_inst[39]); out += line;
    std::snprintf(line, sizeof(line), "    static constexpr int sw_inst_40 = %d;\n", P.sw_inst[40]); out += line;
    std::snprintf(line, sizeof(line), "    static constexpr int sw_inst_41 = %d;\n", P.sw_inst[41]); out += line;
    std::snprintf(line, sizeof(line), "    static constexpr int sw_inst_42 = %d;\n", P.sw_inst[42]); out += line;
    std::snprintf(line, sizeof(line), "    static constexpr int sw_inst_43 = %d;\n", P.sw_inst[43]); out += line;
    std::snprintf(line, sizeof(line), "    static constexpr int sw_inst_44 = %d;\n", P.sw_inst[44]); out += line;
    std::snprintf(line, sizeof(line), "    static constexpr int sw_inst_45 = %d;\n", P.sw_inst[45]); out += line;
    std::snprintf(line, sizeof(line), "    static constexpr int sw_inst_46 = %d;\n", P.sw_inst[46]); out += line;
    std::snprintf(line, sizeof(line), "    static constexpr int sw_inst_47 = %d;\n", P.sw_inst[47]); out += line;
    std::snprintf(line, sizeof(line), "    static constexpr int sw_inst_48 = %d;\n", P.sw_inst[48]); out += line;
    std::snprintf(line, sizeof(line), "    static constexpr int sw_inst_49 = %d;\n", P.sw_inst[49]); out += line;
    std::snprintf(line, sizeof(line), "    static constexpr int sw_inst_50 = %d;\n", P.sw_inst[50]); out += line;
    std::snprintf(line, sizeof(line), "    static constexpr int sw_inst_51 = %d;\n", P.sw_inst[51]); out += line;
    std::snprintf(line, sizeof(line), "    static constexpr int sw_inst_52 = %d;\n", P.sw_inst[52]); out += line;
    std::snprintf(line, sizeof(line), "    static constexpr int sw_inst_53 = %d;\n", P.sw_inst[53]); out += line;
    std::snprintf(line, sizeof(line), "    static constexpr int sw_inst_54 = %d;\n", P.sw_inst[54]); out += line;
    std::snprintf(line, sizeof(line), "    static constexpr int sw_inst_55 = %d;\n", P.sw_inst[55]); out += line;
    std::snprintf(line, sizeof(line), "    static constexpr int sw_inst_56 = %d;\n", P.sw_inst[56]); out += line;
    std::snprintf(line, sizeof(line), "    static constexpr int sw_inst_57 = %d;\n", P.sw_inst[57]); out += line;
    std::snprintf(line, sizeof(line), "    static constexpr int sw_inst_58 = %d;\n", P.sw_inst[58]); out += line;
    std::snprintf(line, sizeof(line), "    static constexpr int sw_inst_59 = %d;\n", P.sw_inst[59]); out += line;
    std::snprintf(line, sizeof(line), "    static constexpr int sw_inst_60 = %d;\n", P.sw_inst[60]); out += line;
    std::snprintf(line, sizeof(line), "    static constexpr int sw_inst_61 = %d;\n", P.sw_inst[61]); out += line;
    std::snprintf(line, sizeof(line), "    static constexpr int sw_inst_62 = %d;\n", P.sw_inst[62]); out += line;
    std::snprintf(line, sizeof(line), "    static constexpr int sw_inst_63 = %d;\n", P.sw_inst[63]); out += line;
    std::snprintf(line, sizeof(line), "    static constexpr int sw_inst_64 = %d;\n", P.sw_inst[64]); out += line;
    std::snprintf(line, sizeof(line), "    static constexpr int sw_inst_65 = %d;\n", P.sw_inst[65]); out += line;
    std::snprintf(line, sizeof(line), "    static constexpr int sw_inst_66 = %d;\n", P.sw_inst[66]); out += line;
    std::snprintf(line, sizeof(line), "    static constexpr int sw_inst_67 = %d;\n", P.sw_inst[67]); out += line;
    std::snprintf(line, sizeof(line), "    static constexpr int sw_inst_68 = %d;\n", P.sw_inst[68]); out += line;
    std::snprintf(line, sizeof(line), "    static constexpr int sw_inst_69 = %d;\n", P.sw_inst[69]); out += line;
    std::snprintf(line, sizeof(line), "    static constexpr int sw_inst_70 = %d;\n", P.sw_inst[70]); out += line;
    std::snprintf(line, sizeof(line), "    static constexpr int sw_inst_71 = %d;\n", P.sw_inst[71]); out += line;
    std::snprintf(line, sizeof(line), "    static constexpr int sw_inst_72 = %d;\n", P.sw_inst[72]); out += line;
    std::snprintf(line, sizeof(line), "    static constexpr int sw_inst_73 = %d;\n", P.sw_inst[73]); out += line;
    std::snprintf(line, sizeof(line), "    static constexpr int sw_inst_74 = %d;\n", P.sw_inst[74]); out += line;
    std::snprintf(line, sizeof(line), "    static constexpr int sw_inst_75 = %d;\n", P.sw_inst[75]); out += line;
    std::snprintf(line, sizeof(line), "    static constexpr int sw_inst_76 = %d;\n", P.sw_inst[76]); out += line;
    std::snprintf(line, sizeof(line), "    static constexpr int sw_inst_77 = %d;\n", P.sw_inst[77]); out += line;
    std::snprintf(line, sizeof(line), "    static constexpr int sw_inst_78 = %d;\n", P.sw_inst[78]); out += line;
    std::snprintf(line, sizeof(line), "    static constexpr int sw_inst_79 = %d;\n", P.sw_inst[79]); out += line;
    out += "    struct sw_inst_t { __host__ __device__ constexpr int operator[](int i) const { return i == 0 ? sw_inst_0 : i == 1 ? sw_inst_1 : i == 2 ? sw_inst_2 : i == 3 ? sw_inst_3 : i == 4 ? sw_inst_4 : i == 5 ? sw_inst_5 : i == 6 ? sw_inst_6 : i == 7 ? sw_inst_7 : i == 8 ? sw_inst_8 : i == 9 ? sw_inst_9 : i == 10 ? sw_inst_10 : i == 11 ? sw_inst_11 : i == 12 ? sw_inst_12 : i == 13 ? sw_inst_13 : i == 14 ? sw_inst_14 : i == 15 ? sw_inst_15 : i == 16 ? sw_inst_16 : i == 17 ? sw_inst_17 : i == 18 ? sw_inst_18 : i == 19 ? sw_inst_19 : i == 20 ? sw_inst_20 : i == 21 ? sw_inst_21 : i == 22 ? sw_inst_22 : i == 23 ? sw_inst_23 : i == 24 ? sw_inst_24 : i == 25 ? sw_inst_25 : i == 26 ? sw_inst_26 : i == 27 ? sw_inst_27 : i == 28 ? sw_inst_28 : i == 29 ? sw_inst_29 : i == 30 ? sw_inst_30 : i == 31 ? sw_inst_31 : i == 32 ? sw_inst_32 : i == 33 ? sw_inst_33 : i == 34 ? sw_inst_34 : i == 35 ? sw_inst_35 : i == 36 ? sw_inst_36 : i == 37 ? sw_inst_37 : i == 38 ? sw_inst_38 : i == 39 ? sw_inst_39 : i == 40 ? sw_inst_40 : i == 41 ? sw_inst_41 : i == 42 ? sw_inst_42 : i == 43 ? sw_inst_43 : i == 44 ? sw_inst_44 : i == 45 ? sw_inst_45 : i == 46 ? sw_inst_46 : i == 47 ? sw_inst_47 : i == 48 ? sw_inst_48 : i == 49 ? sw_inst_49 : i == 50 ? sw_inst_50 : i == 51 ? sw_inst_51 : i == 52 ? sw_inst_52 : i == 53 ? sw_inst_53 : i == 54 ? sw_inst_54 : i == 55 ? sw_inst_55 : i == 56 ? sw_inst_56 : i == 57 ? sw_inst_57 : i == 58 ? sw_inst_58 : i == 59 ? sw_inst_59 : i == 60 ? sw_inst_60 : i == 61 ? sw_inst_61 : i == 62 ? sw_inst_62 : i == 63 ? sw_inst_63 : i == 64 ? sw_inst_64 : i == 65 ? sw_inst_65 : i == 66 ? sw_inst_66 : i == 67 ? sw_inst_67 : i == 68 ? sw_inst_68 : i == 69 ? sw_inst_69 : i == 70 ? sw_inst_70 : i == 71 ? sw_inst_71 : i == 72 ? sw_inst_72 : i == 73 ? sw_inst_73 : i == 74 ? sw_inst_74 : i == 75 ? sw_inst_75 : i == 76 ? sw_inst_76 : i == 77 ? sw_inst_77 : i == 78 ? sw_inst_78 : sw_inst_79; } };\n";
    out += "    static constexpr sw_inst_t sw_inst{};\n";
    std::snprintf(line, sizeof(line), "    static constexpr int bbd_tvar_0 = %d;\n", P.bbd_tvar[0]); out += line;
    std::snprintf(line, sizeof(line), "    static constexpr int bbd_tvar_1 = %d;\n", P.bbd_tvar[1]); out += line;
    std::snprintf(line, sizeof(line), "    static constexpr int bbd_tvar_2 = %d;\n", P.bbd_tvar[2]); out += line;
    std::snprintf(line, sizeof(line), "    static constexpr int bbd_tvar_3 = %d;\n", P.bbd_tvar[3]); out += line;
    std::snprintf(line, sizeof(line), "    static constexpr int bbd_tvar_4 = %d;\n", P.bbd_tvar[4]); out += line;
    std::snprintf(line, sizeof(line), "    static constexpr int bbd_tvar_5 = %d;\n", P.bbd_tvar[5]); out += line;
    std::snprintf(line, sizeof(line), "    static constexpr int bbd_tvar_6 = %d;\n", P.bbd_tvar[6]); out += line;
    std::snprintf(line, sizeof(line), "    static constexpr int bbd_tvar_7 = %d;\n", P.bbd_tvar[7]); out += line;
    std::snprintf(line, sizeof(line), "    static constexpr int bbd_tvar_8 = %d;\n", P.bbd_tvar[8]); out += line;
    std::snprintf(line, sizeof(line), "    static constexpr int bbd_tvar_9 = %d;\n", P.bbd_tvar[9]); out += line;
    std::snprintf(line, sizeof(line), "    static constexpr int bbd_tvar_10 = %d;\n", P.bbd_tvar[10]); out += line;
    std::snprintf(line, sizeof(line), "    static constexpr int bbd_tvar_11 = %d;\n", P.bbd_tvar[11]); out += line;
    std::snprintf(line, sizeof(line), "    static constexpr int bbd_tvar_12 = %d;\n", P.bbd_tvar[12]); out += line;
    std::snprintf(line, sizeof(line), "    static constexpr int bbd_tvar_13 = %d;\n", P.bbd_tvar[13]); out += line;
    std::snprintf(line, sizeof(line), "    static constexpr int bbd_tvar_14 = %d;\n", P.bbd_tvar[14]); out += line;
    std::snprintf(line, sizeof(line), "    static constexpr int bbd_tvar_15 = %d;\n", P.bbd_tvar[15]); out += line;
    out += "    struct bbd_tvar_t { __host__ __device__ constexpr int operator[](int i) const { return i == 0 ? bbd_tvar_0 : i == 1 ? bbd_tvar_1 : i == 2 ? bbd_tvar_2 : i == 3 ? bbd_tvar_3 : i == 4 ? bbd_tvar_4 : i == 5 ? bbd_tvar_5 : i == 6 ? bbd_tvar_6 : i == 7 ? bbd_tvar_7 : i == 8 ? bbd_tvar_8 : i == 9 ? bbd_tvar_9 : i == 10 ? bbd_tvar_10 : i == 11 ? bbd_tvar_11 : i == 12 ? bbd_tvar_12 : i == 13 ? bbd_tvar_13 : i == 14 ? bbd_tvar_14 : bbd_tvar_15; } };\n";
    out += "    static constexpr bbd_tvar_t bbd_tvar{};\n";
    std::snprintf(line, sizeof(line), "    static constexpr int fb_cfg_0 = %d;\n", P.fb_cfg[0]); out += line;
    std::snprintf(line, sizeof(line), "    static constexpr int fb_cfg_1 = %d;\n", P.fb_cfg[1]); out += line;
    std::snprintf(line, sizeof(line), "    static constexpr int fb_cfg_2 = %d;\n", P.fb_cfg[2]); out += line;
    out += "    struct fb_cfg_t { __host__ __device__ constexpr int operator[](int i) const { return i == 0 ? fb_cfg_0 : i == 1 ? fb_cfg_1 : fb_cfg_2; } };\n";
    out += "    static constexpr fb_cfg_t fb_cfg{};\n";
    std::snprintf(line, sizeof(line), "    static constexpr int fb_axis_0 = %d;\n", P.fb_axis[0]); out += line;
    std::snprintf(line, sizeof(line), "    static constexpr int fb_axis_1 = %d;\n", P.fb_axis[1]); out += line;
    std::snprintf(line, sizeof(line), "    static constexpr int fb_axis_2 = %d;\n", P.fb_axis[2]); out += line;
    out += "    struct fb_axis_t { __host__ __device__ constexpr int operator[](int i) const { return i == 0 ? fb_axis_0 : i == 1 ? fb_axis_1 : fb_axis_2; } };\n";
    out += "    static constexpr fb_axis_t fb_axis{};\n";
    if (P.level_off) { std::snprintf(line, sizeof(line), "    static constexpr const int *level_off = spec_ipool + %zu;\n", (size_t)(P.level_off - H.ipool.data())); out += line; }
    else out += "    static constexpr const int *level_off = nullptr;\n";
    if (P.lvl_joints) { std::snprintf(line, sizeof(line), "    static constexpr const int *lvl_joints = spec_ipool + %zu;\n", (size_t)(P.lvl_joints - H.ipool.data())); out += line; }
    else out += "    static constexpr const int *lvl_joints = nullptr;\n";
    if (P.round_off) { std::snprintf(line, sizeof(line), "    static constexpr const int *round_off = spec_ipool + %zu;\n", (size_t)(P.round_off - H.ipool.data())); out += line; }
    else out += "    static constexpr const int *round_off = nullptr;\n";
    if (P.ch_first) { std::snprintf(line, sizeof(line), "    static constexpr const int *ch_first = spec_ipool + %zu;\n", (size_t)(P.ch_first - H.ipool.data())); out += line; }
    else out += "    static constexpr const int *ch_first = nullptr;\n";
    if (P.ch_len) { std::snprintf(line, sizeof(line), "    static constexpr const int *ch_len = spec_ipool + %zu;\n", (size_t)(P.ch_len - H.ipool.data())); out += line; }
    else out += "    static constexpr const int *ch_len = nullptr;\n";
    if (P.ch_parent) { std::snprintf(line, sizeof(line), "    static constexpr const int *ch_parent = spec_ipool + %zu;\n", (size_t)(P.ch_parent - H.ipool.data())); out += line; }
    else out += "    static constexpr const int *ch_parent = nullptr;\n";
    if (P.j_parent) { std::snprintf(line, sizeof(line), "    static constexpr const int *j_parent = spec_ipool + %zu;\n", (size_t)(P.j_parent - H.ipool.data())); out += line; }
    else out += "    static constexpr const int *j_parent = nullptr;\n";
    if (P.j_kind) { std::snprintf(line, sizeof(line), "    static constexpr const int *j_kind = spec_ipool + %zu;\n", (size_t)(P.j_kind - H.ipool.data())); out += line; }
    else out += "    static constexpr const int *j_kind = nullptr;\n";
    if (P.j_cfg) { std::snprintf(line, sizeof(line), "    static constexpr const int *j_cfg = spec_ipool + %zu;\n", (size_t)(P.j_cfg - H.ipool.data())); out += line; }
    else out += "    static constexpr const int *j_cfg = nullptr;\n";
    if (P.j_pre_ident) { std::snprintf(line, sizeof(line), "    static constexpr const int *j_pre_ident = spec_ipool + %zu;\n", (size_t)(P.j_pre_ident - H.ipool.data())); out += line; }
    else out += "    static constexpr const int *j_pre_ident = nullptr;\n";
    if (P.j_pre) { std::snprintf(line, sizeof(line), "    static constexpr const double *j_pre = spec_dpool + %zu;\n", (size_t)(P.j_pre - H.dpool.data())); out += line; }
    else out += "    static constexpr const double *j_pre = nullptr;\n";
    if (P.jcoef) { std::snprintf(line, sizeof(line), "    static constexpr const double *jcoef = spec_dpool + %zu;\n", (size_t)(P.jcoef - H.dpool.data())); out += line; }
    else out += "    static constexpr const double *jcoef = nullptr;\n";
    if (P.j_prm) { std::snprintf(line, sizeof(line), "    static constexpr const double *j_prm = spec_dpool + %zu;\n", (size_t)(P.j_prm - H.dpool.data())); out += line; }
    else out += "    static constexpr const double *j_prm = nullptr;\n";
    if (P.b_anchor) { std::snprintf(line, sizeof(line), "    static constexpr const int *b_anchor = spec_ipool + %zu;\n", (size_t)(P.b_anchor - H.ipool.data())); out += line; }
    else out += "    static constexpr const int *b_anchor = nullptr;\n";
    if (P.b_C) { std::snprintf(line, sizeof(line), "    static constexpr const double *b_C = spec_dpool + %zu;\n", (size_t)(P.b_C - H.dpool.data())); out += line; }
    else out += "    static constexpr const double *b_C = nullptr;\n";
    if (P.b_inertia) { std::snprintf(line, sizeof(line), "    static constexpr const double *b_inertia = spec_dpool + %zu;\n", (size_t)(P.b_inertia - H.dpool.data())); out += line; }
    else out += "    static constexpr const double *b_inertia = nullptr;\n";
    if (P.b_item_off) { std::snprintf(line, sizeof(line), "    static constexpr const int *b_item_off = spec_ipool + %zu;\n", (size_t)(P.b_item_off - H.ipool.data())); out += line; }
    else out += "    static constexpr const int *b_item_off = nullptr;\n";
    if (P.b_pair_off) { std::snprintf(line, sizeof(line), "    static constexpr const int *b_pair_off = spec_ipool + %zu;\n", (size_t)(P.b_pair_off - H.ipool.data())); out += line; }
    else out += "    static constexpr const int *b_pair_off = nullptr;\n";
    if (P.it_body) { std::snprintf(line, sizeof(line), "    static constexpr const int *it_body = spec_ipool + %zu;\n", (size_t)(P.it_body - H.ipool.data())); out += line; }
    else out += "    static constexpr const int *it_body = nullptr;\n";
    if (P.it_joint) { std::snprintf(line, sizeof(line), "    static constexpr const int *it_joint = spec_ipool + %zu;\n", (size_t)(P.it_joint - H.ipool.data())); out += line; }
    else out += "    static constexpr const int *it_joint = nullptr;\n";
    if (P.it_cfg) { std::snprintf(line, sizeof(line), "    static constexpr const int *it_cfg = spec_ipool + %zu;\n", (size_t)(P.it_cfg - H.ipool.data())); out += line; }
    else out += "    static constexpr const int *it_cfg = nullptr;\n";
    if (P.pair_a) { std::snprintf(line, sizeof(line), "    static constexpr const int *pair_a = spec_ipool + %zu;\n", (size_t)(P.pair_a - H.ipool.data())); out += line; }
    else out += "    static constexpr const int *pair_a = nullptr;\n";
    if (P.pair_b) { std::snprintf(line, sizeof(line), "    static constexpr const int *pair_b = spec_ipool + %zu;\n", (size_t)(P.pair_b - H.ipool.data())); out += line; }
    else out += "    static constexpr const int *pair_b = nullptr;\n";
    if (P.pair4) { std::snprintf(line, sizeof(line), "    static constexpr const int *pair4 = spec_ipool + %zu;\n", (size_t)(P.pair4 - H.ipool.data())); out += line; }
    else out += "    static constexpr const int *pair4 = nullptr;\n";
    if (P.tri4) { std::snprintf(line, sizeof(line), "    static constexpr const int *tri4 = spec_ipool + %zu;\n", (size_t)(P.tri4 - H.ipool.data())); out += line; }
    else out += "    static constexpr const int *tri4 = nullptr;\n";
    if (P.cpair4) { std::snprintf(line, sizeof(line), "    static constexpr const int *cpair4 = spec_ipool + %zu;\n", (size_t)(P.cpair4 - H.ipool.data())); out += line; }
    else out += "    static constexpr const int *cpair4 = nullptr;\n";
    if (P.it_pack) { std::snprintf(line, sizeof(line), "    static constexpr const int *it_pack = spec_ipool + %zu;\n", (size_t)(P.it_pack - H.ipool.data())); out += line; }
    else out += "    static constexpr const int *it_pack = nullptr;\n";
    if (P.dh_pack) { std::snprintf(line, sizeof(line), "    static constexpr const int *dh_pack = spec_ipool + %zu;\n", (size_t)(P.dh_pack - H.ipool.data())); out += line; }
    else out += "    static constexpr const int *dh_pack = nullptr;\n";
    if (P.at_d) { std::snprintf(line, sizeof(line), "    static constexpr const double *at_d = spec_dpool + %zu;\n", (size_t)(P.at_d - H.dpool.data())); out += line; }
    else out += "    static constexpr const double *at_d = nullptr;\n";
    if (P.ae_d) { std::snprintf(line, sizeof(line), "    static constexpr const double *ae_d = spec_dpool + %zu;\n", (size_t)(P.ae_d - H.dpool.data())); out += line; }
    else out += "    static constexpr const double *ae_d = nullptr;\n";
    if (P.at_i) { std::snprintf(line, sizeof(line), "    static constexpr const int *at_i = spec_ipool + %zu;\n", (size_t)(P.at_i - H.ipool.data())); out += line; }
    else out += "    static constexpr const int *at_i = nullptr;\n";
    if (P.ae_i) { std::snprintf(line, sizeof(line), "    static constexpr const int *ae_i = spec_ipool + %zu;\n", (size_t)(P.ae_i - H.ipool.data())); out += line; }
    else out += "    static constexpr const int *ae_i = nullptr;\n";
    if (P.dhr_pack) { std::snprintf(line, sizeof(line), "    static constexpr const int *dhr_pack = spec_ipool + %zu;\n", (size_t)(P.dhr_pack - H.ipool.data())); out += line; }
    else out += "    static constexpr const int *dhr_pack = nullptr;\n";
    if (P.cpath_off) { std::snprintf(line, sizeof(line), "    static constexpr const int *cpath_off = spec_ipool + %zu;\n", (size_t)(P.cpath_off - H.ipool.data())); out += line; }
    else out += "    static constexpr const int *cpath_off = nullptr;\n";
    if (P.cpath_items) { std::snprintf(line, sizeof(line), "    static constexpr const int *cpath_items = spec_ipool + %zu;\n", (size_t)(P.cpath_items - H.ipool.data())); out += line; }
    else out += "    static constexpr const int *cpath_items = nullptr;\n";
    if (P.dh_pos) { std::snprintf(line, sizeof(line), "    static constexpr const int *dh_pos = spec_ipool + %zu;\n", (size_t)(P.dh_pos - H.ipool.data())); out += line; }
    else out += "    static constexpr const int *dh_pos = nullptr;\n";
    if (P.tchunk) { std::snprintf(line, sizeof(line), "    static constexpr const int *tchunk = spec_ipool + %zu;\n", (size_t)(P.tchunk - H.ipool.data())); out += line; }
    else out += "    static constexpr const int *tchunk = nullptr;\n";
    if (P.tri_off) { std::snprintf(line, sizeof(line), "    static constexpr const int *tri_off = spec_ipool + %zu;\n", (size_t)(P.tri_off - H.ipool.data())); out += line; }
    else out += "    static constexpr const int *tri_off = nullptr;\n";
    if (P.wp_a) { std::snprintf(line, sizeof(line), "    static constexpr const int *wp_a = spec_ipool + %zu;\n", (size_t)(P.wp_a - H.ipool.data())); out += line; }
    else out += "    static constexpr const int *wp_a = nullptr;\n";
    if (P.wp_b) { std::snprintf(line, sizeof(line), "    static constexpr const int *wp_b = spec_ipool + %zu;\n", (size_t)(P.wp_b - H.ipool.data())); out += line; }
    else out += "    static constexpr const int *wp_b = nullptr;\n";
    if (P.wt_a) { std::snprintf(line, sizeof(line), "    static constexpr const int *wt_a = spec_ipool + %zu;\n", (size_t)(P.wt_a - H.ipool.data())); out += line; }
    else out += "    static constexpr const int *wt_a = nullptr;\n";
    if (P.wt_b) { std::snprintf(line, sizeof(line), "    static constexpr const int *wt_b = spec_ipool + %zu;\n", (size_t)(P.wt_b - H.ipool.data())); out += line; }
// ... 30 lines not shown
    else out += "    static constexpr const int *dh_lookup = nullptr;\n";
    if (P.dh_c) { std::snprintf(line, sizeof(line), "    static constexpr const int *dh_c = spec_ipool + %zu;\n", (size_t)(P.dh_c - H.ipool.data())); out += line; }
    else out += "    static constexpr const int *dh_c = nullptr;\n";
    if (P.dh_cfg) { std::snprintf(line, sizeof(line), "    static constexpr const int *dh_cfg = spec_ipool + %zu;\n", (size_t)(P.dh_cfg - H.ipool.data())); out += line; }
    else out += "    static constexpr const int *dh_cfg = nullptr;\n";
    if (P.dh_joint) { std::snprintf(line, sizeof(line), "    static constexpr const int *dh_joint = spec_ipool + %zu;\n", (size_t)(P.dh_joint - H.ipool.data())); out += line; }
    else out += "    static constexpr const int *dh_joint = nullptr;\n";
    if (P.dh_side) { std::snprintf(line, sizeof(line), "    static constexpr const int *dh_side = spec_ipool + %zu;\n", (size_t)(P.dh_side - H.ipool.data())); out += line; }
    else out += "    static constexpr const int *dh_side = nullptr;\n";
    if (P.damp) { std::snprintf(line, sizeof(line), "    static constexpr const double *damp = spec_dpool + %zu;\n", (size_t)(P.damp - H.dpool.data())); out += line; }
    else out += "    static constexpr const double *damp = nullptr;\n";
    if (P.cf_cfg) { std::snprintf(line, sizeof(line), "    static constexpr const int *cf_cfg = spec_ipool + %zu;\n", (size_t)(P.cf_cfg - H.ipool.data())); out += line; }
    else out += "    static constexpr const int *cf_cfg = nullptr;\n";
    if (P.cf_in) { std::snprintf(line, sizeof(line), "    static constexpr const int *cf_in = spec_ipool + %zu;\n", (size_t)(P.cf_in - H.ipool.data())); out += line; }
    else out += "    static constexpr const int *cf_in = nullptr;\n";
    if (P.cu_off) { std::snprintf(line, sizeof(line), "    static constexpr const int *cu_off = spec_ipool + %zu;\n", (size_t)(P.cu_off - H.ipool.data())); out += line; }
    else out += "    static constexpr const int *cu_off = nullptr;\n";
    if (P.cs_k) { std::snprintf(line, sizeof(line), "    static constexpr const double *cs_k = spec_dpool + %zu;\n", (size_t)(P.cs_k - H.dpool.data())); out += line; }
    else out += "    static constexpr const double *cs_k = nullptr;\n";
    if (P.cs_kq0) { std::snprintf(line, sizeof(line), "    static constexpr const double *cs_kq0 = spec_dpool + %zu;\n", (size_t)(P.cs_kq0 - H.dpool.data())); out += line; }
    else out += "    static constexpr const double *cs_kq0 = nullptr;\n";
    if (P.s_k) { std::snprintf(line, sizeof(line), "    static constexpr const double *s_k = spec_dpool + %zu;\n", (size_t)(P.s_k - H.dpool.data())); out += line; }
    else out += "    static constexpr const double *s_k = nullptr;\n";
    if (P.s_x0) { std::snprintf(line, sizeof(line), "    static constexpr const double *s_x0 = spec_dpool + %zu;\n", (size_t)(P.s_x0 - H.dpool.data())); out += line; }
    else out += "    static constexpr const double *s_x0 = nullptr;\n";
    if (P.c_nloc) { std::snprintf(line, sizeof(line), "    static constexpr const double *c_nloc = spec_dpool + %zu;\n", (size_t)(P.c_nloc - H.dpool.data())); out += line; }
    else out += "    static constexpr const double *c_nloc = nullptr;\n";
    if (P.wr_in) { std::snprintf(line, sizeof(line), "    static constexpr const int *wr_in = spec_ipool + %zu;\n", (size_t)(P.wr_in - H.ipool.data())); out += line; }
    else out += "    static constexpr const int *wr_in = nullptr;\n";
    if (P.wr_const) { std::snprintf(line, sizeof(line), "    static constexpr const double *wr_const = spec_dpool + %zu;\n", (size_t)(P.wr_const - H.dpool.data())); out += line; }
    else out += "    static constexpr const double *wr_const = nullptr;\n";
    if (P.wr_kind) { std::snprintf(line, sizeof(line), "    static constexpr const int *wr_kind = spec_ipool + %zu;\n", (size_t)(P.wr_kind - H.ipool.data())); out += line; }
    else out += "    static constexpr const int *wr_kind = nullptr;\n";
    if (P.wr_Rloc) { std::snprintf(line, sizeof(line), "    static constexpr const double *wr_Rloc = spec_dpool + %zu;\n", (size_t)(P.wr_Rloc - H.dpool.data())); out += line; }
    else out += "    static constexpr const double *wr_Rloc = nullptr;\n";
    if (P.s_c) { std::snprintf(line, sizeof(line), "    static constexpr const double *s_c = spec_dpool + %zu;\n", (size_t)(P.s_c - H.dpool.data())); out += line; }
    else out += "    static constexpr const double *s_c = nullptr;\n";
    if (P.tab_i) { std::snprintf(line, sizeof(line), "    static constexpr const int *tab_i = spec_ipool + %zu;\n", (size_t)(P.tab_i - H.ipool.data())); out += line; }
    else out += "    static constexpr const int *tab_i = nullptr;\n";
    if (P.tab_d) { std::snprintf(line, sizeof(line), "    static constexpr const double *tab_d = spec_dpool + %zu;\n", (size_t)(P.tab_d - H.dpool.data())); out += line; }
    else out += "    static constexpr const double *tab_d = nullptr;\n";
    if (P.cs_c0) { std::snprintf(line, sizeof(line), "    static constexpr const double *cs_c0 = spec_dpool + %zu;\n", (size_t)(P.cs_c0 - H.dpool.data())); out += line; }
    else out += "    static constexpr const double *cs_c0 = nullptr;\n";
    if (P.ncs_i) { std::snprintf(line, sizeof(line), "    static constexpr const int *ncs_i = spec_ipool + %zu;\n", (size_t)(P.ncs_i - H.ipool.data())); out += line; }
    else out += "    static constexpr const int *ncs_i = nullptr;\n";
    if (P.ncs_mb) { std::snprintf(line, sizeof(line), "    static constexpr const double *ncs_mb = spec_dpool + %zu;\n", (size_t)(P.ncs_mb - H.dpool.data())); out += line; }
    else out += "    static constexpr const double *ncs_mb = nullptr;\n";
    if (P.ncs_tab) { std::snprintf(line, sizeof(line), "    static constexpr const double *ncs_tab = spec_dpool + %zu;\n", (size_t)(P.ncs_tab - H.dpool.data())); out += line; }
    else out += "    static constexpr const double *ncs_tab = nullptr;\n";
    if (P.cmp_rep) { std::snprintf(line, sizeof(line), "    static constexpr const int *cmp_rep = spec_ipool + %zu;\n", (size_t)(P.cmp_rep - H.ipool.data())); out += line; }
    else out += "    static constexpr const int *cmp_rep = nullptr;\n";
    if (P.cmp_grp) { std::snprintf(line, sizeof(line), "    static constexpr const int *cmp_grp = spec_ipool + %zu;\n", (size_t)(P.cmp_grp - H.ipool.data())); out += line; }
    else out += "    static constexpr const int *cmp_grp = nullptr;\n";
    if (P.cmp_goff) { std::snprintf(line, sizeof(line), "    static constexpr const int *cmp_goff = spec_ipool + %zu;\n", (size_t)(P.cmp_goff - H.ipool.data())); out += line; }
    else out += "    static constexpr const int *cmp_goff = nullptr;\n";
    if (P.cmp_gbody) { std::snprintf(line, sizeof(line), "    static constexpr const int *cmp_gbody = spec_ipool + %zu;\n", (size_t)(P.cmp_gbody - H.ipool.data())); out += line; }
    else out += "    static constexpr const int *cmp_gbody = nullptr;\n";
    if (P.cmp_pair) { std::snprintf(line, sizeof(line), "    static constexpr const int *cmp_pair = spec_ipool + %zu;\n", (size_t)(P.cmp_pair - H.ipool.data())); out += line; }
    else out += "    static constexpr const int *cmp_pair = nullptr;\n";
    if (P.sj_list) { std::snprintf(line, sizeof(line), "    static constexpr const int *sj_list = spec_ipool + %zu;\n", (size_t)(P.sj_list - H.ipool.data())); out += line; }
    else out += "    static constexpr const int *sj_list = nullptr;\n";
    if (P.sj_full) { std::snprintf(line, sizeof(line), "    static constexpr const int *sj_full = spec_ipool + %zu;\n", (size_t)(P.sj_full - H.ipool.data())); out += line; }
    else out += "    static constexpr const int *sj_full = nullptr;\n";
    if (P.bbd_tab) { std::snprintf(line, sizeof(line), "    static constexpr const int *bbd_tab = spec_ipool + %zu;\n", (size_t)(P.bbd_tab - H.ipool.data())); out += line; }
    else out += "    static constexpr const int *bbd_tab = nullptr;\n";
    if (P.wev_lane) { std::snprintf(line, sizeof(line), "    static constexpr const int *wev_lane = spec_ipool + %zu;\n", (size_t)(P.wev_lane - H.ipool.data())); out += line; }
    else out += "    static constexpr const int *wev_lane = nullptr;\n";
    if (P.bbd_map) { std::snprintf(line, sizeof(line), "    static constexpr const int *bbd_map = spec_ipool + %zu;\n", (size_t)(P.bbd_map - H.ipool.data())); out += line; }
    else out += "    static constexpr const int *bbd_map = nullptr;\n";
    if (P.bbd_ones) { std::snprintf(line, sizeof(line), "    static constexpr const int *bbd_ones = spec_ipool + %zu;\n", (size_t)(P.bbd_ones - H.ipool.data())); out += line; }
    else out += "    static constexpr const int *bbd_ones = nullptr;\n";
    if (P.wev_pairx) { std::snprintf(line, sizeof(line), "    static constexpr const int *wev_pairx = spec_ipool + %zu;\n", (size_t)(P.wev_pairx - H.ipool.data())); out += line; }
    else out += "    static constexpr const int *wev_pairx = nullptr;\n";
    if (P.wev_dhx) { std::snprintf(line, sizeof(line), "    static constexpr const int *wev_dhx = spec_ipool + %zu;\n", (size_t)(P.wev_dhx - H.ipool.data())); out += line; }
    else out += "    static constexpr const int *wev_dhx = nullptr;\n";
    if (P.fb_pair) { std::snprintf(line, sizeof(line), "    static constexpr const int *fb_pair = spec_ipool + %zu;\n", (size_t)(P.fb_pair - H.ipool.data())); out += line; }
    else out += "    static constexpr const int *fb_pair = nullptr;\n";
    if (P.fb_pairx) { std::snprintf(line, sizeof(line), "    static constexpr const int *fb_pairx = spec_ipool + %zu;\n", (size_t)(P.fb_pairx - H.ipool.data())); out += line; }
    else out += "    static constexpr const int *fb_pairx = nullptr;\n";
    if (P.fb_abx) { std::snprintf(line, sizeof(line), "    static constexpr const int *fb_abx = spec_ipool + %zu;\n", (size_t)(P.fb_abx - H.ipool.data())); out += line; }
    else out += "    static constexpr const int *fb_abx = nullptr;\n";
    if (P.fb_lane) { std::snprintf(line, sizeof(line), "    static constexpr const int *fb_lane = spec_ipool + %zu;\n", (size_t)(P.fb_lane - H.ipool.data())); out += line; }
    else out += "    static constexpr const int *fb_lane = nullptr;\n";
    out += "};\n";
}
```

trep_amd/csrc/spec_kernel.hip:

```cpp
#include <hip/hip_runtime.h>

#include <type_traits>

#define TG_GJ_PANEL_DEFAULT 1
#include "mvi_core.hpp"
#include TG_SPEC_HEADER

namespace {
#if defined(SPEC_ARGS_IN_MEMORY)
#define SPEC_KERNEL_ARGS const tg::RunArgs *__restrict__ Ag
#define SPEC_ARGS_REF tg::KArgs &A = *(tg::KArgs *)Ag
#else
#define SPEC_KERNEL_ARGS const tg::RunArgs A
#define SPEC_ARGS_REF ((void)0)
#endif

template <int MODE> constexpr int spec_waves() { return ((MODE == tg::MODE_DERIV1 || MODE == tg::MODE_DERIV2Z) && SPEC_TEAM == 64) ? TG_NW : 1; }
static_assert(TG_NW >= 1 && TG_NW <= 2, "helper waves: the pair lists of program.hpp are split in exactly two parts (wave_part, wp_* / wt_* / wcp4)");
static_assert(TG_NW == 1 || SPEC_TEAM == 64, "helper waves are for full-wave teams (trep_amd/specialize.py passes TG_HELPER_WAVES only then)");

constexpr int TG_ROLLOUT_WAVES = 2;
constexpr int TG_DERIV_WAVES = 1;
template <int MODE, int PIVOT = 0>
__global__ __launch_bounds__(64 * spec_waves<MODE>(), MODE == tg::MODE_DERIV1 ? (SpecProg::a_ok ? 2 : 1) : (MODE == tg::MODE_DERIV2Z ? TG_DERIV_WAVES : TG_ROLLOUT_WAVES)) void k_spec(SPEC_KERNEL_ARGS) {
// ... 34 lines not shown
    const SpecProg P{};
    constexpr int nf = SpecProg::nf, ld = SpecProg::df_ld, nb4 = (nf + 3) >> 2;
    const int lane = threadIdx.x;
    const double *src = A_in + (size_t)blockIdx.x * nf * (nf + 1);
    constexpr bool PKI = tg::tg_static_pk<SpecProg>::value;
    auto load_dense = [&]() {
        for (int e = lane; e < nf * ld; e += 64) S[P.o_Df + e] = 0.0;
        __syncthreads();
        for (int e = lane; e < nf * (nf + 1); e += 64) S[P.o_Df + (e / (nf + 1)) * ld + e % (nf + 1)] = src[e];
    };
    int path = 0;
    bool ok = false;
    if constexpr (SPEC_TEAM == 64 && SpecProg::bbd_ok != 0) {
        int *tab = (int *)(S + P.o_bbd);
        for (int e = lane; e < 128; e += 64) tab[e] = P.bbd_tab[e];
        if constexpr (PKI) {
            for (int e = lane; e < SpecProg::bbd_pk_size; e += 64) S[P.o_Df + e] = 0.0;
            __syncthreads();
            for (int e = lane; e < nf * (nf + 1); e += 64) { const int at = P.bbd_map[e]; if (at >= 0) S[P.o_Df + at] = src[e]; }
            for (int e = lane; e < SpecProg::bbd_pk_nones; e += 64) S[P.o_Df + P.bbd_ones[e]] = 1.0;
        } else load_dense();
        __syncthreads();
        typedef typename std::conditional<PKI, tg::BbdPackedImage<SpecProg::bbd_pk_nr, SpecProg::bbd_pk_nc2, SpecProg::bbd_pk_tb, SpecProg::bbd_pk_tc2, SpecProg::bbd_pk_xs>, tg::BbdDenseImage>::type Img;
        if (!skip_structured && tg::gj_bbd<nf, ld, SpecProg::bbd_ng, SpecProg::bbd_nb, SpecProg::bbd_t, Img>(S + P.o_Df, tg::bbd_rows<SpecProg::bbd_ng + SpecProg::bbd_nb>(tab, lane), PKI ? S + P.o_W + 12 * P.n_joints : S + P.o_J, lane, P.bbd_tvar)) { ok = true; path = 1; }
        __syncthreads();
        if (PKI && ok && lane < nf) x_out[(size_t)blockIdx.x * nf + lane] = S[P.o_Df + SpecProg::bbd_pk_xs + lane];
        if (PKI && !ok) load_dense();
    } else load_dense();
    __syncthreads();
    if (!ok) {
        if constexpr (SPEC_TEAM == 64 && nb4 >= 5 && nf <= 31 && 12 * SpecProg::n_items >= 128) ok = tg::gj_panel<4 * nb4>(true, S + P.o_Df, nf, ld, lane, S + P.o_J);
        else if constexpr (SPEC_TEAM == 64 && nb4 <= 8) ok = tg::gj_rows<64, 4 * nb4>(true, S + P.o_Df, nf, ld, lane);
        path = ok ? 2 : -1;
    }
    __syncthreads();
    if (lane < nf && !(PKI && path == 1)) x_out[(size_t)blockIdx.x * nf + lane] = S[P.o_Df + lane * ld + nf];
    if (lane == 0) path_out[blockIdx.x] = path;
#endif
}

template <int MODE, int PIVOT = 0>
int launch_mode(const tg::RunArgs *A, tg::RunArgs *slot, int grid, size_t lds, hipStream_t stream) {
    if (lds > 64 * 1024 &&
        hipFuncSetAttribute(reinterpret_cast<const void *>(&k_spec<MODE, PIVOT>), hipFuncAttributeMaxDynamicSharedMemorySize, (int)lds) != hipSuccess) return 1;
#if defined(SPEC_ARGS_IN_MEMORY)
    if (!slot) return 3;
    if (hipMemcpyAsync(slot, A, sizeof(tg::RunArgs), hipMemcpyHostToDevice, stream) != hipSuccess) return 1;
    hipLaunchKernelGGL((k_spec<MODE, PIVOT>), dim3(grid), dim3(64 * spec_waves<MODE>()), lds, stream, (const tg::RunArgs *)slot);
#else
    hipLaunchKernelGGL((k_spec<MODE, PIVOT>), dim3(grid), dim3(64 * spec_waves<MODE>()), lds, stream, *A);
#endif
    return hipGetLastError() == hipSuccess ? 0 : 1;
}
template <int MODE, int PIVOT = 0>
int launch_mode_par(const tg::RunArgs *A, tg::RunArgs *slot, int grid, size_t lds, hipStream_t stream, const tg::ParTable &T) {
    if (lds > 64 * 1024 &&
        hipFuncSetAttribute(reinterpret_cast<const void *>(&k_spec_par<MODE, PIVOT>), hipFuncAttributeMaxDynamicSharedMemorySize, (int)lds) != hipSuccess) return 1;
#if defined(SPEC_ARGS_IN_MEMORY)
    if (!slot) return 3;
    if (hipMemcpyAsync(slot, A, sizeof(tg::RunArgs), hipMemcpyHostToDevice, stream) != hipSuccess) return 1;
    hipLaunchKernelGGL((k_spec_par<MODE, PIVOT>), dim3(grid), dim3(64 * spec_waves<MODE>()), lds, stream, (const tg::RunArgs *)slot, T);
#else
    hipLaunchKernelGGL((k_spec_par<MODE, PIVOT>), dim3(grid), dim3(64 * spec_waves<MODE>()), lds, stream, *A, T);
#endif
    return hipGetLastError() == hipSuccess ? 0 : 1;
}
}

extern "C" {
const int *tg_spec_sizes(void) {
    static const int s[8] = {(int)sizeof(tg::DevProg), (int)sizeof(tg::RunArgs), SpecProg::nq, SpecProg::nd, SpecProg::nc, SpecProg::n_items,
                             SpecProg::n_pairs, SpecProg::lds_per_team};
    return s;
}
unsigned long long tg_spec_key(void) {
#if defined(TG_SPEC_KEY)
    return TG_SPEC_KEY;
#else
    return 0ull;
#endif
}
int tg_spec_waves(void) { return spec_waves<tg::MODE_DERIV2Z>(); }
int tg_spec_fb_n(void) { return tg::tg_static_fb<SpecProg>::value ? SpecProg::fb_n : 0; }
int tg_spec_modes(void) {
    int m = 1 << tg::MODE_ROLLOUT;
#if defined(SPEC_DERIVATIVES)
    m |= (1 << tg::MODE_DERIV1) | (1 << tg::MODE_DERIV2Z);
#endif
    return m;
}
int tg_spec_par_modes(void) { return tg_spec_modes(); }
int tg_spec_debug_solve(const double *A_dev, double *x_dev, int *path_dev, int n_mats, int skip_structured) {
    const size_t lds = sizeof(double) * (size_t)SpecProg::lds_per_team;
    if (lds > 64 * 1024 &&
        hipFuncSetAttribute(reinterpret_cast<const void *>(&k_spec_debug_solve), hipFuncAttributeMaxDynamicSharedMemorySize, (int)lds) != hipSuccess) return 1;
    hipLaunchKernelGGL(k_spec_debug_solve, dim3(n_mats), dim3(64), lds, 0, A_dev, x_dev, path_dev, skip_structured);
    return hipGetLastError() == hipSuccess ? 0 : 1;
}
int tg_spec_launch(int mode, const tg::RunArgs *A, tg::RunArgs *device_slot, int grid, size_t lds, void *stream) {
    switch (mode) {
    case tg::MODE_ROLLOUT:
        return A->exact_pivot ? launch_mode<tg::MODE_ROLLOUT, 1>(A, device_slot, grid, lds, (hipStream_t)stream)
                              : launch_mode<tg::MODE_ROLLOUT, 0>(A, device_slot, grid, lds, (hipStream_t)stream);
#if defined(SPEC_DERIVATIVES)
    case tg::MODE_DERIV1: return launch_mode<tg::MODE_DERIV1>(A, device_slot, grid, lds, (hipStream_t)stream);
    case tg::MODE_DERIV2Z: return launch_mode<tg::MODE_DERIV2Z>(A, device_slot, grid, lds, (hipStream_t)stream);
#endif
    default: return 2;
    }
}
int tg_spec_launch_par(int mode, const tg::RunArgs *A, tg::RunArgs *device_slot, int grid, size_t lds, void *stream, const double *rows, int group, int stride) {
    const tg::ParTable T{rows, group, stride};
    switch (mode) {
    case tg::MODE_ROLLOUT:
        return A->exact_pivot ? launch_mode_par<tg::MODE_ROLLOUT, 1>(A, device_slot, grid, lds, (hipStream_t)stream, T)
                              : launch_mode_par<tg::MODE_ROLLOUT, 0>(A, device_slot, grid, lds, (hipStream_t)stream, T);
#if defined(SPEC_DERIVATIVES)
    case tg::MODE_DERIV1: return launch_mode_par<tg::MODE_DERIV1>(A, device_slot, grid, lds, (hipStream_t)stream, T);
    case tg::MODE_DERIV2Z: return launch_mode_par<tg::MODE_DERIV2Z>(A, device_slot, grid, lds, (hipStream_t)stream, T);
#endif
    default: return 2;
    }
}
}
```

trep_amd/csrc/trepamd.hip:

```cpp
#include <hip/hip_runtime.h>

#include <cmath>
#include <cstdio>
#include <cstdlib>
#include <cstring>
#include <memory>
#include <string>
#include <vector>

#include "device_buffer.hpp"
#include "mvi_core.hpp"
#include "mvi_project.hpp"
#include "spec_emit.inc"
#include <dlfcn.h>

namespace tg_detail {
int fail(int code, const std::string &msg);
int launch_par(int team, bool springs, const tg::DevProg *d_prog, const tg::RunArgs &A, const tg::ParTable &T, int grid, size_t lds, hipStream_t stream);
int launch_project(int team, bool springs, const tg::DevProg *d_prog, const tg::RunArgs &A, const tg::ProjectArgs &J, int grid, size_t lds, hipStream_t stream);
}

namespace {

thread_local std::string g_error;

int fail(int code, const std::string &msg) {
    g_error = msg;
    return code;
}
#define HIP_TRY(expr)                                                                                   \
    do {                                                                                                \
        hipError_t e_ = (expr);                                                                         \
        if (e_ != hipSuccess) return fail(TG_ERR_HIP, std::string(#expr) + ": " + hipGetErrorString(e_)); \
    } while (0)

template <int TEAM, int MODE, bool SPRINGS>
__global__ __launch_bounds__(64, (MODE == tg::MODE_DERIV1 || MODE == tg::MODE_DERIV2Z || MODE == tg::MODE_DYN_DERIV1) ? 1 : 2) void k_run(const tg::DevProg *__restrict__ Pg, const tg::RunArgs A) {
    double *lds = tg_lds_base();
    tg::CProg &P = *(tg::CProg *)Pg;
    const int team = threadIdx.x / TEAM, lane = threadIdx.x % TEAM;
    const int block = MODE == tg::MODE_ROLLOUT ? tg_xcd_block((int)blockIdx.x, (int)gridDim.x) : (int)blockIdx.x;
    const int traj = tg::tg_remap_trajectory(A, block * (64 / TEAM) + team);
    const int stride = MODE == tg::MODE_DERIV2Z ? P.e_lds_per_team : (MODE == tg::MODE_DERIV1 ? P.a_lds_per_team : (MODE == tg::MODE_DYN_DERIV1 ? P.g_lds_per_team : P.lds_per_team));
    tg::run_trajectory<TEAM, MODE, SPRINGS>(P, A, lds + (size_t)team * stride, lane, traj);
}

template <int MODE, bool SPRINGS, class Real>
__global__ __launch_bounds__(64, 1) void k_forward(const tg::DevProg *__restrict__ Pg, const tg::RunArgs A) {
    Real *lds = (Real *)tg_lds_base();
    tg::CProg &P = *(tg::CProg *)Pg;
    tg::run_forward<64, MODE, SPRINGS>(P, A, lds, (int)threadIdx.x, (int)blockIdx.x);
}

}

struct tg_system {
    tg::HostProgram H;
    int team = 64;
    bool has_gravity = false, has_damping = false;
};

struct tg_batch {
    tg_system *sys = nullptr;
    int batch = 0, device = 0;
    tg::DevProg P{};
    tg::DeviceBuffer<tg::DevProg> d_prog;
    void *spec_lib = nullptr;
    int (*spec_launch)(int, const tg::RunArgs *, tg::RunArgs *, int, size_t, void *) = nullptr;
    int (*spec_launch_par)(int, const tg::RunArgs *, tg::RunArgs *, int, size_t, void *, const double *, int, int) = nullptr;
    int spec_par_modes = 0;
    tg::DeviceBuffer<double> par_dev;
    int par_rows = 0, par_group = 1, par_stride = 0;
    struct Launched { unsigned int modes = 0; long long n = 0; void add(int mode) { modes |= 1u << mode; n++; } } launched[2][2];
    static constexpr int ARG_SLOTS = 4;
    tg::DeviceBuffer<tg::RunArgs> d_args;
    tg::PinnedBuffer<tg::RunArgs> h_args;
    tg::Event arg_done[ARG_SLOTS];
    bool arg_used[ARG_SLOTS] = {false, false, false, false};
    int arg_next = 0;
    tg::PinnedBuffer<double> io_host;
    double *io_dev = nullptr;
    size_t io_in = 0, io_out = 0;
    bool mirror_valid = false;
    int spec_modes = 0, spec_waves = 1, spec_fb_n = 0;
    std::string spec_path;
    tg::DeviceBuffer<int> d_ints;
    tg::DeviceBuffer<double> d_dbls;
    tg::DeviceBuffer<double> q1, q2, p1, p2, lam, u1;
    tg::DeviceBuffer<double> stage_u, stage_k, stage_qh, stage_lh, f_out;
    tg::DeviceBuffer<int> iters, status, fallbacks;
    tg::DeviceBuffer<double> z_dev, hz_dev, zl_dev;
    tg::DeviceBuffer<double> dyn;
    tg::DeviceBuffer<double> dyn_d1;
    tg::DeviceBuffer<double> energy;
    tg::DeviceBuffer<double> lag;
    tg::DeviceBuffer<int> dyn_ints;
    tg::DeviceBuffer<double> proj;
    tg::DeviceBuffer<int> proj_ints;
    tg::DeviceBuffer<int> seeds;
    tg::DeviceBuffer<double> d1[12];
    bool have_d1 = false;
    tg::DeviceBuffer<long long> prof;
    tg::DeviceBuffer<double> snap;
    double snap_t1 = 0.0, snap_t2 = 0.0;
    long long total_iters = 0;
    double t1 = 0.0, t2 = 0.0, tolerance = 1.0e-10;
    int predictor = 0;
    tg::DeviceBuffer<double> dt_dev;
    std::vector<double> dt_host;
    int dt_by_trajectory = 0;
    int exact_pivot = 0;
    hipStream_t stream = nullptr;
    bool own_stream = true;
    static constexpr size_t TIMING_CAP = 4096;
    bool timing = false;
    double folded_ms = 0.0;
    long long folded_n = 0;
    std::vector<std::pair<tg::Event, tg::Event>> events;
    std::vector<tg::Event> pool;
};

namespace {

int widths(const tg_batch *b, int field) {
    const tg::DevProg &P = b->P;
    switch (field) {
    case TG_F_Q1: case TG_F_Q2: return P.nq;
    case TG_F_P1: case TG_F_P2: return P.nd;
    case TG_F_U1: return P.nu;
    case TG_F_LAMBDA1: return P.nc;
    default: break;
    }
    if (field >= TG_F_Q2_DQ1 && field <= TG_F_L1_DK2) {
        const int k = field - TG_F_Q2_DQ1, var = k % 4, out = k / 4;
        const int rows = var == 0 ? P.nq : (var == 1 ? P.nd : (var == 2 ? P.nu : P.nk));
        return rows * (out == 2 ? P.nc : P.nd);
    }
    return -1;
}
double *field_ptr(tg_batch *b, int field) {
    switch (field) {
    case TG_F_Q1: return b->q1.get();
    case TG_F_Q2: return b->q2.get();
    case TG_F_P1: return b->p1.get();
    case TG_F_P2: return b->p2.get();
    case TG_F_U1: return b->u1.get();
    case TG_F_LAMBDA1: return b->lam.get();
    default: break;
    }
    if (field >= TG_F_Q2_DQ1 && field <= TG_F_L1_DK2) return b->d1[field - TG_F_Q2_DQ1].get();
    return nullptr;
}

int pick_team(const tg::HostProgram &H) {
    if (const char *env = std::getenv("TREPAMD_TEAM")) {
        int t = std::atoi(env);
        if (t == 1 || t == 4 || t == 16 || t == 64) return t;
    }
    const tg::DevProg &P = H.p;
    int width = std::max(P.n_items, (P.nf * (P.nf + 1)) / 4);
    int team = width > 32 ? 64 : (width > 8 ? 16 : (width > 2 ? 4 : 1));
    while (team < 64 && (size_t)(64 / team) * P.lds_per_team * sizeof(double) > 64 * 1024) team *= 4;
    return team;
}

template <typename T>
void append(std::vector<T> &pool, const std::vector<T> &v, size_t &off) {
// ... 973 lines not shown
    HIP_TRY(hipMemcpy(dA.get(), A_aug_host, sizeof(double) * n * (n + 1), hipMemcpyHostToDevice));
    hipLaunchKernelGGL(k_debug_solve, dim3(1), dim3(64), sizeof(double) * (n * ld + 16 + 192), 0, n, ld, (int)exact, dA.get(), dx.get(), dp.get(), ds.get());
    HIP_TRY(hipGetLastError());
    HIP_TRY(hipMemcpy(x_host, dx.get(), sizeof(double) * n, hipMemcpyDeviceToHost));
    HIP_TRY(hipMemcpy(pivot_rows_host, dp.get(), sizeof(int) * n, hipMemcpyDeviceToHost));
    HIP_TRY(hipMemcpy(status_host, ds.get(), sizeof(int), hipMemcpyDeviceToHost));
    return TG_SUCCESS;
}

int tg_batch_set_pivot_rule(tg_batch *b, int32_t exact) {
    if (!b) return fail(TG_ERR_INVALID, "null batch");
    b->exact_pivot = exact ? 1 : 0;
    return TG_SUCCESS;
}

}
namespace {
std::string spec_header_text(const tg_system *sys) {
    std::string out;
    char line[160];
    std::snprintf(line, sizeof(line), "#define SPEC_TEAM %d\n#define SPEC_SPRINGS %s\n", sys->team,
                  launch_springs(sys->H.p) ? "true" : "false");
    out += line;
    emit_spec_header(sys->H, out);
    return out;
}
uint64_t fnv1a64(const std::string &t) {
    uint64_t h = 1469598103934665603ull;
    for (unsigned char c : t) { h ^= c; h *= 1099511628211ull; }
    return h;
}
}
extern "C" {

int64_t tg_system_spec_header(const tg_system *sys, char *buf, uint64_t capacity) {
    if (!sys) { fail(TG_ERR_INVALID, "null system"); return -1; }
    const std::string out = spec_header_text(sys);
    if (buf && capacity) {
        const size_t n = std::min((size_t)capacity - 1, out.size());
        std::memcpy(buf, out.data(), n);
        buf[n] = 0;
    }
    return (int64_t)out.size() + 1;
}

uint64_t tg_system_spec_key(const tg_system *sys) {
    if (!sys) { fail(TG_ERR_INVALID, "null system"); return 0; }
    return fnv1a64(spec_header_text(sys));
}

int tg_batch_load_specialized(tg_batch *b, const char *library_path) {
    if (!b || !library_path) return fail(TG_ERR_INVALID, "null argument");
    HIP_TRY(hipSetDevice(b->device));
    std::unique_ptr<void, int (*)(void *)> lib(dlopen(library_path, RTLD_NOW | RTLD_LOCAL), dlclose);
    void *h = lib.get();
    const char *why = h ? nullptr : dlerror();
    if (!h) return fail(TG_ERR_INVALID, std::string("cannot load ") + library_path + ": " + (why ? why : "?"));
    auto launch_fn = reinterpret_cast<int (*)(int, const tg::RunArgs *, tg::RunArgs *, int, size_t, void *)>(dlsym(h, "tg_spec_launch"));
    auto sizes_fn = reinterpret_cast<const int *(*)(void)>(dlsym(h, "tg_spec_sizes"));
    auto modes_fn = reinterpret_cast<int (*)(void)>(dlsym(h, "tg_spec_modes"));
    auto key_fn = reinterpret_cast<uint64_t (*)(void)>(dlsym(h, "tg_spec_key"));
    if (!launch_fn || !sizes_fn || !modes_fn || !key_fn) return fail(TG_ERR_INVALID, "not a specialised trep_amd kernel library");
    const tg::DevProg &P = b->P;
    const int want[8] = {(int)sizeof(tg::DevProg), (int)sizeof(tg::RunArgs), P.nq, P.nd, P.nc, P.n_items, P.n_pairs, P.lds_per_team};
    const int *got = sizes_fn();
    for (int i = 0; i < 8; i++) if (got[i] != want[i]) return fail(TG_ERR_INVALID, "specialised kernel was built for a different system or library version");
    if (key_fn() != tg_system_spec_key(b->sys)) return fail(TG_ERR_INVALID, "specialised kernel was built from a different schedule (header hash mismatch)");
    if (!b->d_args) {
        tg::DeviceBuffer<tg::RunArgs> d_args;
        tg::PinnedBuffer<tg::RunArgs> h_args;
        tg::Event done[tg_batch::ARG_SLOTS];
        bool ok = d_args.ensure(tg_batch::ARG_SLOTS) == hipSuccess && h_args.ensure(tg_batch::ARG_SLOTS, hipHostMallocDefault) == hipSuccess;
        for (int i = 0; i < tg_batch::ARG_SLOTS && ok; i++) ok = done[i].create(hipEventDisableTiming) == hipSuccess;
        if (!ok) return fail(TG_ERR_HIP, "allocation of the argument blocks failed");
        b->d_args = std::move(d_args); b->h_args = std::move(h_args);
        for (int i = 0; i < tg_batch::ARG_SLOTS; i++) b->arg_done[i] = std::move(done[i]);
    }
    if (b->spec_lib) { hipStreamSynchronize(b->stream); dlclose(b->spec_lib); }
    b->spec_lib = lib.release(); b->spec_launch = launch_fn; b->spec_modes = modes_fn(); b->spec_path = library_path;
    auto waves_fn = reinterpret_cast<int (*)(void)>(dlsym(h, "tg_spec_waves"));
    b->spec_waves = waves_fn ? waves_fn() : 1;
    auto fb_fn = reinterpret_cast<int (*)(void)>(dlsym(h, "tg_spec_fb_n"));
    b->spec_fb_n = fb_fn ? fb_fn() : 0;
    auto par_fn = reinterpret_cast<int (*)(int, const tg::RunArgs *, tg::RunArgs *, int, size_t, void *, const double *, int, int)>(dlsym(h, "tg_spec_launch_par"));
    auto par_modes_fn = reinterpret_cast<int (*)(void)>(dlsym(h, "tg_spec_par_modes"));
    b->spec_launch_par = par_modes_fn ? par_fn : nullptr;
    b->spec_par_modes = (par_fn && par_modes_fn) ? par_modes_fn() : 0;
    return TG_SUCCESS;
}

int tg_system_newton_plan(const tg_system *sys, int32_t out[8], uint8_t *pattern, int32_t *tab) {
    if (!sys || !out) return fail(TG_ERR_INVALID, "null argument");
    const tg::DevProg &P = sys->H.p;
    out[0] = P.bbd_ok; out[1] = P.bbd_g; out[2] = P.bbd_ng; out[3] = P.bbd_nb; out[4] = P.bbd_t; out[5] = P.nf; out[6] = P.nd; out[7] = 0;
    if (pattern) {
        std::memset(pattern, 0, (size_t)P.nf * P.nf);
        if (sys->H.newton_pattern.size() == (size_t)P.nf * P.nf) std::memcpy(pattern, sys->H.newton_pattern.data(), sys->H.newton_pattern.size());
    }
    if (tab) for (int i = 0; i < 128; i++) tab[i] = i < (int)sys->H.bbd_tab.size() ? sys->H.bbd_tab[i] : 0;
    return TG_SUCCESS;
}

int tg_batch_debug_newton_solve(tg_batch *b, int32_t n_mats, int32_t skip_structured, const double *A_aug_host, double *x_host, int32_t *path_host) {
    if (!b || n_mats <= 0 || !A_aug_host || !x_host || !path_host) return fail(TG_ERR_INVALID, "bad arguments");
    if (!b->spec_lib) return fail(TG_ERR_INVALID, "no specialised kernel library loaded");
    auto fn = reinterpret_cast<int (*)(const double *, double *, int *, int, int)>(dlsym(b->spec_lib, "tg_spec_debug_solve"));
    if (!fn) return fail(TG_ERR_INVALID, "the specialised library has no solve hook");
    const int nf = b->P.nf;
    HIP_TRY(hipSetDevice(b->device));
    tg::DeviceBuffer<double> dA, dx;
    tg::DeviceBuffer<int> dp;
    const size_t cA = (size_t)n_mats * nf * (nf + 1), cx = (size_t)n_mats * nf, cp = (size_t)n_mats;
    auto failed = [](const char *what) { (void)hipGetLastError(); return fail(TG_ERR_HIP, what); };
    if (dA.ensure(cA) != hipSuccess || dx.ensure(cx) != hipSuccess || dp.ensure(cp) != hipSuccess) return failed("solve hook: device allocation failed");
    if (hipMemcpy(dA.get(), A_aug_host, cA * sizeof(double), hipMemcpyHostToDevice) != hipSuccess) return failed("solve hook: upload failed");
    const int rc = fn(dA.get(), dx.get(), dp.get(), n_mats, skip_structured);
    if (hipDeviceSynchronize() != hipSuccess || rc != 0) return failed("solve hook launch failed");
    if (hipMemcpy(x_host, dx.get(), cx * sizeof(double), hipMemcpyDeviceToHost) != hipSuccess ||
        hipMemcpy(path_host, dp.get(), cp * sizeof(int), hipMemcpyDeviceToHost) != hipSuccess)
        return failed("solve hook: download failed");
    return TG_SUCCESS;
}

int tg_batch_info(const tg_batch *b, int32_t out[8]) {
    if (!b || !out) return fail(TG_ERR_INVALID, "null argument");
    out[0] = b->spec_launch ? b->spec_modes : 0;
    for (int spec = 0; spec < 2; spec++) { out[2 - spec] = (int32_t)b->launched[0][spec].modes; out[4 - spec] = (int32_t)std::min<long long>(b->launched[0][spec].n, 0x7fffffff); }
    out[5] = b->exact_pivot; out[6] = b->sys->team; out[7] = b->spec_launch ? b->spec_waves : 1;
    if (b->spec_launch) out[7] |= b->spec_fb_n << 8;
    return TG_SUCCESS;
}

int tg_batch_par_info(const tg_batch *b, int32_t out[8]) {
    if (!b || !out) return fail(TG_ERR_INVALID, "null argument");
    out[0] = b->spec_launch_par ? b->spec_par_modes : 0;
    for (int spec = 0; spec < 2; spec++) { out[2 - spec] = (int32_t)b->launched[1][spec].modes; out[4 - spec] = (int32_t)std::min<long long>(b->launched[1][spec].n, 0x7fffffff); }
    out[5] = b->par_rows; out[6] = b->par_rows ? b->par_group : 0; out[7] = 0;
    return TG_SUCCESS;
}

int tg_system_parameters(const tg_system *sys, int32_t sizes_out[4], double *inertia, double *gravity, double *damping) {
    if (!sys) return fail(TG_ERR_INVALID, "null system");
    const tg::HostProgram &H = sys->H;
    if (sizes_out) { sizes_out[0] = H.p.n_bodies; sizes_out[1] = H.p.nd; sizes_out[2] = sys->has_gravity; sizes_out[3] = sys->has_damping; }
    const int nb = H.p.n_bodies, nd = H.p.nd;
    std::vector<double> row(4 * (size_t)nb + 3 + nd);
    base_parameter_row(H, row.data());
    if (inertia) std::copy_n(row.begin(), 4 * nb, inertia);
    if (gravity) std::copy_n(row.begin() + 4 * nb, 3, gravity);
    if (damping) std::copy_n(row.begin() + 4 * nb + 3, nd, damping);
    return TG_SUCCESS;
}

int tg_batch_set_parameters(tg_batch *b, int32_t rows, int32_t group, const double *inertia_host, const double *gravity_host,
                            const double *damping_host) {
    if (!b) return fail(TG_ERR_INVALID, "null batch");
    if (rows <= 0 || group <= 0) return fail(TG_ERR_INVALID, "rows and group must be positive");
    if (rows != 1 && (int64_t)rows * group != b->batch) return fail(TG_ERR_INVALID, "rows * group must equal the batch size (or rows == 1)");
    if (gravity_host && !b->sys->has_gravity) return fail(TG_ERR_INVALID, "the system has no Gravity potential: no gravity block");
    if (damping_host && !b->sys->has_damping) return fail(TG_ERR_INVALID, "the system has no Damping force: no damping block");
    const tg::HostProgram &H = b->sys->H;
    const int nb = H.p.n_bodies, nd = H.p.nd, stride = 4 * nb + 3 + nd;
    std::vector<double> tab((size_t)rows * stride);
    for (int r = 0; r < rows; r++) {
        double *row = tab.data() + (size_t)r * stride;
        base_parameter_row(H, row);
        if (inertia_host) std::copy_n(inertia_host + (size_t)r * 4 * nb, 4 * nb, row);
        if (gravity_host) std::copy_n(gravity_host + 3 * (size_t)r, 3, row + 4 * nb);
        if (damping_host) std::copy_n(damping_host + (size_t)r * nd, nd, row + 4 * nb + 3);
    }
    for (double v : tab) if (!std::isfinite(v)) return fail(TG_ERR_INVALID, "parameter values must be finite");
    HIP_TRY(hipSetDevice(b->device));
    HIP_TRY(hipStreamSynchronize(b->stream));
    if (tab.size() > b->par_dev.count()) {
        if (b->par_dev) { b->par_dev.reset(); b->par_rows = 0; }
        HIP_TRY(b->par_dev.ensure(tab.size()));
    }
    HIP_TRY(hipMemcpyAsync(b->par_dev.get(), tab.data(), tab.size() * sizeof(double), hipMemcpyHostToDevice, b->stream));
    HIP_TRY(hipStreamSynchronize(b->stream));
    b->par_rows = rows; b->par_group = rows == 1 ? b->batch : group; b->par_stride = stride;
    b->mirror_valid = false;
    return TG_SUCCESS;
}

int tg_batch_clear_parameters(tg_batch *b) {
    if (!b) return fail(TG_ERR_INVALID, "null batch");
    b->par_rows = 0;
    b->mirror_valid = false;
    return TG_SUCCESS;
}

void *tg_batch_stream(tg_batch *b) { return b ? (void *)b->stream : nullptr; }

int tg_batch_timing(tg_batch *b, int32_t reset, int32_t *n_launches, double *total_ms) {
    if (!b) return fail(TG_ERR_INVALID, "null batch");
    HIP_TRY(hipSetDevice(b->device));
    HIP_TRY(hipStreamSynchronize(b->stream));
    b->timing = true;
    double ms = b->folded_ms;
    for (auto &e : b->events) {
        float t = 0.f;
        HIP_TRY(hipEventElapsedTime(&t, e.first.get(), e.second.get()));
        ms += t;
    }
    if (n_launches) *n_launches = (int32_t)(b->events.size() + b->folded_n);
    if (total_ms) *total_ms = ms;
    if (reset) {
        for (auto &e : b->events) { b->pool.push_back(std::move(e.first)); b->pool.push_back(std::move(e.second)); }
        b->events.clear();
        b->folded_ms = 0.0; b->folded_n = 0;
    }
    return TG_SUCCESS;
// ... 4 lines not shown
```

trep_amd/midpointvi.py:

```python
import collections
import os

import numpy as np

from . import _lib
from .descriptor import flatten
from .errors import ConvergenceError

Projection = collections.namedtuple("Projection", "Q dQ mu iterations status")


class BatchMidpointVI(object):

    def __init__(self, system, batch, tolerance=1e-10, device=0, specialize="auto"):
        self._system = system
        self._specialize_mode = specialize
        self._specialized = None
        self._batch = int(batch)
        self._device = int(device)
        self._L = _lib.lib()
        _lib.require_device()
        self._desc = flatten(system)
        self._structure_version = system._structure_version
        self._sys_h = self._L.tg_system_create(self._desc.byref())
# ... 44 lines not shown
        self._parameter_rows = 0
        self._structure_version = self._system._structure_version
        self._specialized = None
        if self._specialize_mode is True or (self._specialize_mode == "auto" and os.environ.get("TREPAMD_NO_SPECIALIZE") is None):
            self.specialize(build=False)
        if keep is not None:
            (t1, t2), fields, tol, pred, exact = keep
            self.set_times(t1, t2)
            for n, v in zip(("q1", "q2", "p1", "p2", "u1", "lambda1"), fields):
                setattr(self, n, v)
            self.tolerance = tol
            self.predictor = pred
            self.exact_pivot = exact
        ss = getattr(self, "_step_sizes", None)
        if ss is not None:
            self.set_step_sizes(ss[0], ss[1])
        return True

    def close(self):
        if getattr(self, "_h", None):
            for p in self._owned_dev:
                self._L.tg_device_free(self._device, p)
            self._owned_dev = []
            self._L.tg_batch_destroy(self._h)
            self._h = None
        if getattr(self, "_sys_h", None):
            self._L.tg_system_destroy(self._sys_h)
            self._sys_h = None

    def __del__(self):
        try:
            self.close()
        except Exception:
            pass

    def set_step_sizes(self, dts=None, by_trajectory=False):
        if dts is None:
            _lib.check(self._L.tg_batch_set_step_sizes(self._h, 0, None, 0))
            self._step_sizes = None
            return
        d = np.ascontiguousarray(dts, dtype=np.float64).reshape(-1)
        _lib.check(self._L.tg_batch_set_step_sizes(self._h, len(d), d.ctypes.data, 1 if by_trajectory else 0))
        self._step_sizes = (d.copy(), bool(by_trajectory))

    @staticmethod
    def _dt_argument(dt, n_steps):
        if np.ndim(dt) == 0:
            return float(dt), None
        d = np.ascontiguousarray(dt, dtype=np.float64).reshape(-1)
        if len(d) != n_steps:
            raise ValueError("expected %d step sizes, got %d" % (n_steps, len(d)))
        if np.allclose(d, d[0], rtol=1e-13, atol=0.0):
            return float(d[0]), None
        return float(d[0]), d

    @property
    def exact_pivot(self):
        return getattr(self, "_exact_pivot", False)

    @exact_pivot.setter
    def exact_pivot(self, value):
        _lib.check(self._L.tg_batch_set_pivot_rule(self._h, 1 if value else 0))
        self._exact_pivot = bool(value)

    system = property(lambda self: self._system)
    batch = property(lambda self: self._batch)
    device = property(lambda self: self._device)
    nq = property(lambda self: int(self._desc.n_configs))
    nd = property(lambda self: int(self._desc.n_dyn))
    nk = property(lambda self: int(self._desc.n_kin))
    nu = property(lambda self: int(self._desc.n_inputs))
    nc = property(lambda self: int(self._desc.n_constraints))
    nX = property(lambda self: self.nq + self.nd + self.nk)
    nU = property(lambda self: self.nu + self.nk)

    def info(self):
        out = (np.zeros(8, dtype=np.int32))
        _lib.check(self._L.tg_system_info(self._sys_h, out.ctypes.data_as(_lib._c_ip)))
        keys = ["team", "lds_bytes_per_trajectory", "joints", "levels", "bodies", "items", "pairs", "dh_items"]
        d = dict(zip(keys, (int(v) for v in out)))
        kout = np.zeros(8, dtype=np.int32)
        _lib.check(self._L.tg_batch_info(self._h, kout.ctypes.data_as(_lib._c_ip)))
        d["fb_n"] = (int(kout[7]) >> 8) & 0xFF
        return d

    MODES = {"rollout": 0, "calc_p2": 1, "calc_f": 2, "deriv1": 3, "deriv2z": 4}
    ALL_MODES = dict(MODES, dynamics=5, dynamics_deriv1=6, energy=7, lagrangian=8)

    def parameters(self):
        sizes = np.zeros(4, dtype=np.int32)
        _lib.check(self._L.tg_system_parameters(self._sys_h, sizes.ctypes.data, None, None, None))
        inertia = np.zeros((int(sizes[0]), 4))
        gravity, damping = np.zeros(3), np.zeros(int(sizes[1]))
        _lib.check(self._L.tg_system_parameters(self._sys_h, None, inertia.ctypes.data if inertia.size else None, gravity.ctypes.data,
                                                damping.ctypes.data if damping.size else None))
        return {"inertia": inertia, "gravity": gravity if sizes[2] else None, "damping": damping if sizes[3] else None}

    def set_parameters(self, inertia=None, gravity=None, damping=None, group=1):
        self.refresh()
        from . import parameters as _par
        rows, group, blocks = _par.pack(self._system, self._batch, inertia=inertia, gravity=gravity, damping=damping, group=group)
        p = lambda name: None if blocks[name] is None or blocks[name].size == 0 else blocks[name].ctypes.data
        rc = self._L.tg_batch_set_parameters(self._h, rows, group, p("inertia"), p("gravity"), p("damping"))
        if rc == _lib.ERR_INVALID:
            raise ValueError(self._L.tg_last_error().decode())
        _lib.check(rc)
        self._parameter_rows = rows

    def clear_parameters(self):
        _lib.check(self._L.tg_batch_clear_parameters(self._h))
        self._parameter_rows = 0

    @property
    def has_parameters(self):
        return getattr(self, "_parameter_rows", 0) > 0

    def kernel_info(self):
        out = np.zeros(8, dtype=np.int32)
        _lib.check(self._L.tg_batch_info(self._h, out.ctypes.data_as(_lib._c_ip)))
        names = lambda bits: sorted(n for n, m in self.MODES.items() if (int(bits) >> m) & 1)
        par = np.zeros(8, dtype=np.int32)
        _lib.check(self._L.tg_batch_par_info(self._h, par.ctypes.data_as(_lib._c_ip)))
        every = lambda bits: sorted(n for n, m in self.ALL_MODES.items() if (int(bits) >> m) & 1)
        return {"spec_modes": names(out[0]), "spec_launched": names(out[1]), "generic_launched": names(out[2]),
                "spec_launch_mask": int(out[1]), "generic_launch_mask": int(out[2]),
                "spec_launches": int(out[3]), "generic_launches": int(out[4]), "exact_pivot": bool(out[5]), "team": int(out[6]),
                "helper_waves": int(out[7]) & 0xFF, "fb_n": (int(out[7]) >> 8) & 0xFF, "spec_library": self._specialized,
                "par_spec_modes": every(par[0]), "par_spec_launched": every(par[1]), "par_generic_launched": every(par[2]),
                "par_spec_launches": int(par[3]), "par_generic_launches": int(par[4]), "parameter_rows": int(par[5]),
                "parameter_group": int(par[6])}

    @property
    def stream(self):
        return self._L.tg_batch_stream(self._h)

    @property
    def tolerance(self):
        return self._tolerance

    @tolerance.setter
    def tolerance(self, value):
        self._tolerance = float(value)
        _lib.check(self._L.tg_batch_set_tolerance(self._h, self._tolerance))

    def times(self):
        import ctypes
        a, b = ctypes.c_double(), ctypes.c_double()
        _lib.check(self._L.tg_batch_get_times(self._h, ctypes.byref(a), ctypes.byref(b)))
        return a.value, b.value

    def set_times(self, t1, t2):
        _lib.check(self._L.tg_batch_set_times(self._h, float(t1), float(t2)))

    def _get(self, field, width):
        out = np.zeros((self._batch, width))
        if width:
            _lib.check(self._L.tg_batch_get(self._h, field, out.ctypes.data))
        return out

    def _set(self, field, width, value):
        arr = np.ascontiguousarray(np.broadcast_to(np.asarray(value, dtype=np.float64), (self._batch, width)))
        if width:
            _lib.check(self._L.tg_batch_set(self._h, field, arr.ctypes.data))

    def _field(field, width_attr):
        def getter(self):
            return self._get(field, getattr(self, width_attr))

        def setter(self, value):
            self._set(field, getattr(self, width_attr), value)
        return property(getter, setter)

    q1 = _field(_lib.F_Q1, "nq")
    q2 = _field(_lib.F_Q2, "nq")
    p1 = _field(_lib.F_P1, "nd")
    p2 = _field(_lib.F_P2, "nd")
    u1 = _field(_lib.F_U1, "nu")
    lambda1 = _field(_lib.F_LAMBDA1, "nc")
    del _field

    def initialize_from_state(self, t1, q1, p1, lambda1=None):
        self.refresh()
        self.set_times(t1, t1)
        self.q1 = q1
        self.p1 = p1
        self.q2 = q1
        self.p2 = p1
        self.lambda1 = np.zeros((self._batch, self.nc)) if lambda1 is None else lambda1

    def initialize_from_configs(self, t0, q0, t1, q1, lambda1=None):
        self.refresh()
        self.set_times(t0, t1)
        self.q1 = q0
        self.q2 = q1
        _lib.check(self._L.tg_batch_calc_p2(self._h))
        self.lambda1 = np.zeros((self._batch, self.nc)) if lambda1 is None else lambda1

    def calc_p2(self):
        self.refresh()
        _lib.check(self._L.tg_batch_calc_p2(self._h))

    def calc_f(self):
        self.refresh()
        out = np.zeros((self._batch, self.nd + self.nc))
        _lib.check(self._L.tg_batch_calc_f(self._h, out.ctypes.data))
        return out

    D1_NAMES = ["q2_dq1", "q2_dp1", "q2_du1", "q2_dk2", "p2_dq1", "p2_dp1", "p2_du1", "p2_dk2",
                "l1_dq1", "l1_dp1", "l1_du1", "l1_dk2"]

# ... 473 lines not shown
```

Measured before the change: 56.47 million.

## Fold pure-translation joint prefixes out of the rollout chain sweep

Finds runs of translation joints with identity rotation at the root of the kinematic chain and records their world position as an affine function of configuration values. The pose builder then writes those translation columns straight from q, and a trimmed chain schedule skips these joints in the serial 3x4 transform products. The goal is a shorter dependent matrix-multiply chain in the rollout pose sweep, at the cost of a second LDS schedule, extra per-lane table loads and larger specialized program constants.

Result: faster. 57.91 million (median of 6 runs) (+2.5%).

```diff
diff --git a/trep_amd/csrc/mvi_core.hpp b/trep_amd/csrc/mvi_core.hpp
--- a/trep_amd/csrc/mvi_core.hpp
+++ b/trep_amd/csrc/mvi_core.hpp
@@ -91,6 +91,9 @@
 
 template <class P, class = void> struct tg_static_fb { static constexpr bool value = false; };
 template <class P> struct tg_static_fb<P, typename std::enable_if<(P::fb_on >= 0)>::type> { static constexpr bool value = P::fb_on != 0 && tg_static_wev<P>::value; };
+
+template <class P, class = void> struct tg_static_tr { static constexpr bool value = false; };
+template <class P> struct tg_static_tr<P, typename std::enable_if<(P::tr_on >= 0)>::type> { static constexpr bool value = P::tr_on != 0 && tg_static_sweep<P>::value && P::tab_ok != 0; };
 
 enum { MODE_ROLLOUT = 0, MODE_CALC_P2 = 1, MODE_CALC_F = 2, MODE_DERIV1 = 3, MODE_DERIV2Z = 4, MODE_DYNAMICS = 5, MODE_DYN_DERIV1 = 6, MODE_ENERGY = 7, MODE_LAGRANGIAN = 8 };
 
@@ -332,7 +335,7 @@
                     const int q = swact ? l / 12 : 4, rc = swact ? l - 12 * q : 0;
                     swr = rc >> 2; swcol = rc & 3;
 #pragma unroll
-                    for (int i = 0; i < 16; i++) swc[i] = (i & 3) < SP::sw_np[i >> 2] ? sw_code<SP>(i * 5, q) : 15;
+                    for (int i = 0; i < 16; i++) swc[i] = (i & 3) < SwPlan<SP>::np(i >> 2) ? sw_code<SP>(i * 5, q) : 15;
                 }
             }
 #pragma unroll
@@ -388,6 +391,11 @@
             }
             sched[2 * idx] = w0; sched[2 * idx + 1] = w1;
         }
+#if defined(__HIP_DEVICE_COMPILE__)
+        if constexpr (tg_static_tr<typename std::remove_cv<PROG>::type>::value) {
+            if (rollout) { int *sched2 = (int *)(S + P.o_sched2); TG_FOR(i, 32 * P.n_rounds) sched2[i] = P.tr_sched[i]; }
+        }
+#endif
         TG_SYNC();
     }
 
@@ -491,15 +499,18 @@
         const int n12 = 12 * nj, n24 = 2 * n12;
         SwDesc sw0;
         if constexpr (tg_static_sweep<typename std::remove_cv<PROG>::type>::value) {
-            if (rollout_lists) sw0 = sw_fetch<typename std::remove_cv<PROG>::type, 0>((const int *)(S + P.o_sched));
-        }
+            if (rollout_lists) sw0 = sw_fetch<typename std::remove_cv<PROG>::type, 0>((const int *)(S + SwPlan<typename std::remove_cv<PROG>::type>::o_sched()));
+        }
+        constexpr bool TR = tg_static_tr<typename std::remove_cv<PROG>::type>::value;
         if (P.tab_ok) {
             double pr[2][12];
+            int trw[2] = {0, 0};
 #pragma unroll
             for (int u = 0; u < 2; u++) {
-                const double *src = P.j_prm + 12 * (size_t)((jck[u] >> 16) & 0xFFF);
+                const double *src = (TR && rollout_lists ? P.tr_prm : P.j_prm) + 12 * (size_t)((jck[u] >> 16) & 0xFFF);
 #pragma unroll
                 for (int e = 0; e < 12; e++) pr[u][e] = src[e];
+                if constexpr (TR) { if (rollout_lists) trw[u] = P.tr_sj[lane + u * TEAM < sjn ? lane + u * TEAM : 0]; }
             }
             if (on) {
 #pragma unroll
@@ -512,6 +523,12 @@
                         const bool rotary = kind >= TG_RX;
                         const int a = rotary ? kind - TG_RX : kind - TG_TX, b = a == 2 ? 0 : a + 1, c = a == 0 ? 2 : a - 1;
                         double *g = (second ? G2 : G) + 12 * j;
+                        auto row_t = [&](int l, double v) {
+                            if constexpr (TR) {
+                                if (rollout_lists) { const double e = qval(second ? dsB : dsA, (trw[u] >> (8 * l)) & 0xFF); return (trw[u] >> (24 + l)) & 1 ? e : v; }
+                            }
+                            return v;
+                        };
                         if (u * TEAM < sc_rot2) {
                             double sn = 0.0, cs = 1.0;
                             if (rotary) tg_sincos(x, &sn, &cs);
@@ -522,14 +539,14 @@
                                 g[4 * l + a] = A_;
                                 g[4 * l + b] = rotary ? fma(C_, sn, B_ * cs) : B_;
                                 g[4 * l + c] = rotary ? fma(-B_, sn, C_ * cs) : C_;
-                                g[4 * l + 3] = fma(A_, tq, D_);
+                                g[4 * l + 3] = row_t(l, fma(A_, tq, D_));
                             }
                         } else {
 #pragma unroll
                             for (int l = 0; l < 3; l++) {
                                 const double A_ = pr[u][4 * l], B_ = pr[u][4 * l + 1], C_ = pr[u][4 * l + 2], D_ = pr[u][4 * l + 3];
                                 g[4 * l + a] = A_; g[4 * l + b] = B_; g[4 * l + c] = C_;
-                                g[4 * l + 3] = fma(A_, x, D_);
+                                g[4 * l + 3] = row_t(l, fma(A_, x, D_));
                             }
                         }
                     }
@@ -587,7 +604,7 @@
             if (rollout_lists) {
                 typedef typename std::remove_cv<PROG>::type SP;
                 __builtin_amdgcn_s_setprio(TG_CHAIN_PRIO);
-                chain_round_quads<SP, 0>(on, sched, sw0);
+                chain_round_quads<SP, 0>(on, (const int *)(S + SwPlan<SP>::o_sched()), sw0);
                 __builtin_amdgcn_s_setprio(0);
                 return;
             }
@@ -673,8 +690,22 @@
         }
     }
     struct SwDesc { int w0[4], par[4]; };
+    template <class SP, bool TR = tg_static_tr<SP>::value> struct SwPlan {
+        TG_HD static constexpr int np(int r) { return SP::sw_np[r]; }
+        TG_HD static constexpr int len(int i) { return SP::sw_len[i]; }
+        TG_HD static constexpr int inst(int i) { return SP::sw_inst[i]; }
+        TG_HD static constexpr int maxlen() { return SP::sw_maxlen; }
+        TG_HD static constexpr int o_sched() { return SP::o_sched; }
+    };
+    template <class SP> struct SwPlan<SP, true> {
+        TG_HD static constexpr int np(int r) { return SP::tr_np[r]; }
+        TG_HD static constexpr int len(int i) { return SP::tr_len[i]; }
+        TG_HD static constexpr int inst(int i) { return SP::tr_inst[i]; }
+        TG_HD static constexpr int maxlen() { return SP::tr_maxlen; }
+        TG_HD static constexpr int o_sched() { return SP::o_sched2; }
+    };
     template <class SP> TG_HD static int sw_code(int base, int q) {
-        auto w = [&](int i) { const int c = SP::sw_inst[base + i]; return c ? (c & 0x1FF) : 15; };
+        auto w = [&](int i) { const int c = SwPlan<SP>::inst(base + i); return c ? (c & 0x1FF) : 15; };
         return q == 0 ? w(0) : q == 1 ? w(1) : q == 2 ? w(2) : q == 3 ? w(3) : w(4);
     }
     template <class SP, int RD> TG_HD SwDesc sw_fetch(const int *sched) const {
@@ -682,7 +713,7 @@
 #pragma unroll
         for (int ps = 0; ps < 4; ps++) {
             d.w0[ps] = 0; d.par[ps] = -1;
-            if (ps < SP::sw_np[RD < 4 ? RD : 0]) {
+            if (ps < SwPlan<SP>::np(RD < 4 ? RD : 0)) {
                 const int slot = swc[4 * (RD < 4 ? RD : 0) + ps] & 0xFF;
                 d.w0[ps] = sched[2 * (16 * RD + slot)]; d.par[ps] = sched[2 * (16 * RD + slot) + 1];
             }
@@ -691,7 +722,7 @@
     }
     template <class SP, int RD> TG_HD void chain_round_quads(bool on, const int *sched, const SwDesc &d) {
         if constexpr (RD < SP::n_rounds) {
-            constexpr int NP = SP::sw_np[RD], ML = SP::sw_maxlen;
+            constexpr int NP = SwPlan<SP>::np(RD), ML = SwPlan<SP>::maxlen() > 0 ? SwPlan<SP>::maxlen() : 1;
             SwDesc nxt = d;
             if constexpr (RD + 1 < SP::n_rounds) nxt = sw_fetch<SP, RD + 1>(sched);
             const int r = swr, c = swcol;
@@ -710,7 +741,7 @@
                         p[ps] = opar >= 0 ? pv : (r == c ? 1.0 : 0.0);
 #pragma unroll
                         for (int s = 0; s < ML; s++) {
-                            if (s < SP::sw_len[4 * RD + ps]) {
+                            if (s < SwPlan<SP>::len(4 * RD + ps)) {
                                 const int o = base[ps] + 12 * s + c;
                                 m[ps][s][0] = S[o]; m[ps][s][1] = S[o + 4]; m[ps][s][2] = S[o + 8];
                             }
@@ -721,7 +752,7 @@
                 for (int s = 0; s < ML; s++) {
 #pragma unroll
                     for (int ps = 0; ps < 4; ps++) {
-                        if (ps < NP && s < SP::sw_len[4 * RD + ps]) {
+                        if (ps < NP && s < SwPlan<SP>::len(4 * RD + ps)) {
                             const double b0 = tg_quad_bcast<0>(p[ps]), b1 = tg_quad_bcast<1>(p[ps]), b2 = tg_quad_bcast<2>(p[ps]);
                             const double last = c == 3 ? p[ps] : 0.0;
                             const double v = fma(b2, m[ps][s][2], fma(b1, m[ps][s][1], fma(b0, m[ps][s][0], last)));
diff --git a/trep_amd/csrc/program.hpp b/trep_amd/csrc/program.hpp
--- a/trep_amd/csrc/program.hpp
+++ b/trep_amd/csrc/program.hpp
@@ -114,6 +114,12 @@
     int fb_axis[3];
     const int *fb_pair, *fb_pairx, *fb_abx, *fb_lane;
     int a_ok, a_o_T12, a_o_AUG, a_aug_ld, a_o_T22, a_lds_per_team;
+    int tr_n, tr_on, tr_maxlen, o_sched2;
+    int tr_np[4];
+    int tr_len[16];
+    int tr_inst[80];
+    const int *tr_joint, *tr_src, *tr_sj, *tr_sched;
+    const double *tr_const, *tr_prm;
 };
 
 struct HostProgram {
@@ -132,6 +138,8 @@
     std::vector<double> damp, cs_k, cs_kq0, cs_c0, s_k, s_x0, s_c, c_nloc, wr_const, wr_Rloc, ncs_mb, ncs_tab;
     std::vector<int> ncs_i, bbd_tab, cmp_rep, cmp_grp, cmp_goff, cmp_gbody, cmp_pair, wev_lane, bbd_map, bbd_ones, wev_pairx, wev_dhx;
     std::vector<int> fb_pair, fb_pairx, fb_abx, fb_lane;
+    std::vector<int> tr_joint, tr_src, tr_sj, tr_sched;
+    std::vector<double> tr_const, tr_prm;
     std::vector<unsigned char> newton_pattern;
     std::vector<int> wr_in, wr_kind;
     std::vector<int> cf_cfg, cf_in;
@@ -924,6 +932,80 @@
             P.lds_per_team = (P.lds_per_team + 1) & ~1;
         }
     }
+    {
+        P.tr_n = P.tr_on = P.tr_maxlen = P.o_sched2 = 0;
+        for (int i = 0; i < 4; i++) P.tr_np[i] = 0;
+        for (int i = 0; i < 16; i++) P.tr_len[i] = 0;
+        for (int i = 0; i < 80; i++) P.tr_inst[i] = 0;
+        std::vector<int> run_of(nj, -1);
+        for (int j = 0; j < nj; j++) {
+            const int kind = H.j_kind[j], par = H.j_parent[j];
+            if (kind < TG_TX || kind > TG_TZ || (par >= 0 && run_of[par] < 0)) continue;
+            const double *pre = &H.j_pre[12 * (size_t)j];
+            bool ok = true;
+            for (int l = 0; l < 3; l++) for (int c = 0; c < 3; c++) if (pre[4 * l + c] != (l == c ? 1.0 : 0.0)) ok = false;
+            int src[3];
+            double cst[3];
+            for (int r = 0; r < 3; r++) {
+                src[r] = par >= 0 ? H.tr_src[3 * (size_t)run_of[par] + r] : -1;
+                cst[r] = par >= 0 ? H.tr_const[3 * (size_t)run_of[par] + r] : 0.0;
+                const double D = pre[4 * r + 3];
+                if (D != 0.0) { if (src[r] >= 0 || cst[r] != 0.0) ok = false; else cst[r] = D; }
+            }
+            const int a = kind - TG_TX;
+            if (src[a] >= 0 || cst[a] != 0.0) ok = false;
+            if (!ok) continue;
+            src[a] = H.j_cfg[j]; cst[a] = 0.0;
+            run_of[j] = P.tr_n++;
+            H.tr_joint.push_back(j);
+            for (int r = 0; r < 3; r++) { H.tr_src.push_back(src[r]); H.tr_const.push_back(src[r] >= 0 ? 0.0 : cst[r]); }
+        }
+        H.tr_prm = H.j_prm;
+        for (int i = 0; i < P.tr_n; i++)
+            for (int l = 0; l < 3; l++) H.tr_prm[12 * (size_t)H.tr_joint[i] + 4 * l + 3] = H.tr_const[3 * (size_t)i + l];
+        H.tr_sj.assign(H.sj_list.size(), 0);
+        for (int n = 0; n < P.n_sj; n++) {
+            const int j = (H.sj_list[n] >> 16) & 0xFFF, i = run_of[j];
+            if (i < 0) continue;
+            for (int r = 0; r < 3; r++) {
+                const int c = H.tr_src[3 * (size_t)i + r];
+                if (c >= 0 && c != H.j_cfg[j]) H.tr_sj[n] |= ((c & 0xFF) << (8 * r)) | (1 << (24 + r));
+            }
+        }
+        H.tr_sched.assign(32 * (size_t)std::max(P.n_rounds, 1), 0);
+        bool on = P.sw_ok && P.wev_ok && P.tr_n > 0 && nq <= 256;
+        for (int r = 0; r < P.n_rounds && on; r++) {
+            std::vector<int> inst;
+            for (int slot = 0; slot < 16; slot++) {
+                const int c = H.round_off[r] + slot;
+                int *w = &H.tr_sched[2 * (size_t)(16 * r + slot)];
+                w[0] = 0; w[1] = -1;
+                if (c >= H.round_off[r + 1]) continue;
+                int k = 0;
+                while (k < H.ch_len[c] && run_of[H.ch_first[c] + k] >= 0) k++;
+                const int first = H.ch_first[c] + k, len = H.ch_len[c] - k, parent = k ? first - 1 : H.ch_parent[c];
+                if (len == 0) continue;
+                w[0] = (12 * first) | (len << 16); w[1] = parent >= 0 ? 12 * parent : -1;
+                for (int set = 0; set < 2; set++) if (pose_need[first] >> set & 1) inst.push_back(slot | (set << 8) | (1 << 9));
+            }
+            P.tr_np[r] = ((int)inst.size() + 4) / 5;
+            for (int p = 0; p < P.tr_np[r]; p++) {
+                int len = 0;
+                for (int q = 0; q < 5 && 5 * p + q < (int)inst.size(); q++) {
+                    P.tr_inst[(4 * r + p) * 5 + q] = inst[5 * p + q];
+                    len = std::max(len, H.tr_sched[2 * (size_t)(16 * r + (inst[5 * p + q] & 0xFF))] >> 16);
+                }
+                P.tr_len[4 * r + p] = len;
+                P.tr_maxlen = std::max(P.tr_maxlen, len);
+            }
+        }
+        if (on) {
+            P.tr_on = 1;
+            P.o_sched2 = P.lds_per_team;
+            P.lds_per_team += 16 * P.n_rounds;
+        }
+        if (H.tr_joint.empty()) { H.tr_joint.push_back(0); H.tr_src.assign(3, -1); H.tr_const.assign(3, 0.0); }
+    }
     H.pack();
     return H;
 }
@@ -946,8 +1028,8 @@
     X(c_cfg) X(c_comp) X(dh_c) X(dh_cfg) X(dh_joint) X(dh_side) X(cf_cfg) X(cf_in) X(dh_lookup) X(cu_off) X(it_slot) X(pair4) \
     X(tri4) X(cpair4) X(it_pack) X(dh_pack) X(cpath_off) X(cpath_items) X(dh_pos) X(tchunk) X(tri_off) X(wr_in) X(wr_kind) X(ncs_i) \
     X(wp_a) X(wp_b) X(wt_a) X(wt_b) X(wt_split) X(wcp4) X(bbd_tab) X(cmp_rep) X(cmp_grp) X(cmp_goff) X(cmp_gbody) X(cmp_pair) X(dhr_pack) X(at_i) X(ae_i) X(sj_list) X(sj_full) X(wev_lane) X(bbd_map) X(bbd_ones) X(wev_pairx) X(wev_dhx) \
-    X(fb_pair) X(fb_pairx) X(fb_abx) X(fb_lane)
-#define TG_DBL_TABLES(X) X(j_pre) X(jcoef) X(j_prm) X(at_d) X(ae_d) X(b_C) X(b_inertia) X(e_off) X(c_dist) X(c_tol) X(damp) X(cs_k) X(cs_kq0) X(cs_c0) X(s_k) X(s_x0) X(c_nloc) X(wr_const) X(s_c) X(wr_Rloc) X(ncs_mb) X(ncs_tab)
+    X(fb_pair) X(fb_pairx) X(fb_abx) X(fb_lane) X(tr_joint) X(tr_src) X(tr_sj) X(tr_sched)
+#define TG_DBL_TABLES(X) X(j_pre) X(jcoef) X(j_prm) X(at_d) X(ae_d) X(b_C) X(b_inertia) X(e_off) X(c_dist) X(c_tol) X(damp) X(cs_k) X(cs_kq0) X(cs_c0) X(s_k) X(s_x0) X(c_nloc) X(wr_const) X(s_c) X(wr_Rloc) X(ncs_mb) X(ncs_tab) X(tr_const) X(tr_prm)
 
 inline void HostProgram::pack() {
     ipool.clear(); dpool.clear(); ioff.clear(); doff.clear();
diff --git a/trep_amd/csrc/spec_emit.inc b/trep_amd/csrc/spec_emit.inc
--- a/trep_amd/csrc/spec_emit.inc
+++ b/trep_amd/csrc/spec_emit.inc
@@ -171,6 +171,10 @@
     std::snprintf(line, sizeof(line), "    static constexpr int a_aug_ld = %d;\n", P.a_aug_ld); out += line;
     std::snprintf(line, sizeof(line), "    static constexpr int a_o_T22 = %d;\n", P.a_o_T22); out += line;
     std::snprintf(line, sizeof(line), "    static constexpr int a_lds_per_team = %d;\n", P.a_lds_per_team); out += line;
+    std::snprintf(line, sizeof(line), "    static constexpr int tr_n = %d;\n", P.tr_n); out += line;
+    std::snprintf(line, sizeof(line), "    static constexpr int tr_on = %d;\n", P.tr_on); out += line;
+    std::snprintf(line, sizeof(line), "    static constexpr int tr_maxlen = %d;\n", P.tr_maxlen); out += line;
+    std::snprintf(line, sizeof(line), "    static constexpr int o_sched2 = %d;\n", P.o_sched2); out += line;
     std::snprintf(line, sizeof(line), "    static constexpr double grav_0 = %a;\n", P.grav[0]); out += line;
     std::snprintf(line, sizeof(line), "    static constexpr double grav_1 = %a;\n", P.grav[1]); out += line;
     std::snprintf(line, sizeof(line), "    static constexpr double grav_2 = %a;\n", P.grav[2]); out += line;
@@ -344,6 +348,112 @@
     std::snprintf(line, sizeof(line), "    static constexpr int fb_axis_2 = %d;\n", P.fb_axis[2]); out += line;
     out += "    struct fb_axis_t { __host__ __device__ constexpr int operator[](int i) const { return i == 0 ? fb_axis_0 : i == 1 ? fb_axis_1 : fb_axis_2; } };\n";
     out += "    static constexpr fb_axis_t fb_axis{};\n";
+    std::snprintf(line, sizeof(line), "    static constexpr int tr_np_0 = %d;\n", P.tr_np[0]); out += line;
+    std::snprintf(line, sizeof(line), "    static constexpr int tr_np_1 = %d;\n", P.tr_np[1]); out += line;
+    std::snprintf(line, sizeof(line), "    static constexpr int tr_np_2 = %d;\n", P.tr_np[2]); out += line;
+    std::snprintf(line, sizeof(line), "    static constexpr int tr_np_3 = %d;\n", P.tr_np[3]); out += line;
+    out += "    struct tr_np_t { __host__ __device__ constexpr int operator[](int i) const { return i == 0 ? tr_np_0 : i == 1 ? tr_np_1 : i == 2 ? tr_np_2 : tr_np_3; } };\n";
+    out += "    static constexpr tr_np_t tr_np{};\n";
+    std::snprintf(line, sizeof(line), "    static constexpr int tr_len_0 = %d;\n", P.tr_len[0]); out += line;
+    std::snprintf(line, sizeof(line), "    static constexpr int tr_len_1 = %d;\n", P.tr_len[1]); out += line;
+    std::snprintf(line, sizeof(line), "    static constexpr int tr_len_2 = %d;\n", P.tr_len[2]); out += line;
+    std::snprintf(line, sizeof(line), "    static constexpr int tr_len_3 = %d;\n", P.tr_len[3]); out += line;
+    std::snprintf(line, sizeof(line), "    static constexpr int tr_len_4 = %d;\n", P.tr_len[4]); out += line;
+    std::snprintf(line, sizeof(line), "    static constexpr int tr_len_5 = %d;\n", P.tr_len[5]); out += line;
+    std::snprintf(line, sizeof(line), "    static constexpr int tr_len_6 = %d;\n", P.tr_len[6]); out += line;
+    std::snprintf(line, sizeof(line), "    static constexpr int tr_len_7 = %d;\n", P.tr_len[7]); out += line;
+    std::snprintf(line, sizeof(line), "    static constexpr int tr_len_8 = %d;\n", P.tr_len[8]); out += line;
+    std::snprintf(line, sizeof(line), "    static constexpr int tr_len_9 = %d;\n", P.tr_len[9]); out += line;
+    std::snprintf(line, sizeof(line), "    static constexpr int tr_len_10 = %d;\n", P.tr_len[10]); out += line;
+    std::snprintf(line, sizeof(line), "    static constexpr int tr_len_11 = %d;\n", P.tr_len[11]); out += line;
+    std::snprintf(line, sizeof(line), "    static constexpr int tr_len_12 = %d;\n", P.tr_len[12]); out += line;
+    std::snprintf(line, sizeof(line), "    static constexpr int tr_len_13 = %d;\n", P.tr_len[13]); out += line;
+    std::snprintf(line, sizeof(line), "    static constexpr int tr_len_14 = %d;\n", P.tr_len[14]); out += line;
+    std::snprintf(line, sizeof(line), "    static constexpr int tr_len_15 = %d;\n", P.tr_len[15]); out += line;
+    out += "    struct tr_len_t { __host__ __device__ constexpr int operator[](int i) const { return i == 0 ? tr_len_0 : i == 1 ? tr_len_1 : i == 2 ? tr_len_2 : i == 3 ? tr_len_3 : i == 4 ? tr_len_4 : i == 5 ? tr_len_5 : i == 6 ? tr_len_6 : i == 7 ? tr_len_7 : i == 8 ? tr_len_8 : i == 9 ? tr_len_9 : i == 10 ? tr_len_10 : i == 11 ? tr_len_11 : i == 12 ? tr_len_12 : i == 13 ? tr_len_13 : i == 14 ? tr_len_14 : tr_len_15; } };\n";
+    out += "    static constexpr tr_len_t tr_len{};\n";
+    std::snprintf(line, sizeof(line), "    static constexpr int tr_inst_0 = %d;\n", P.tr_inst[0]); out += line;
+    std::snprintf(line, sizeof(line), "    static constexpr int tr_inst_1 = %d;\n", P.tr_inst[1]); out += line;
+    std::snprintf(line, sizeof(line), "    static constexpr int tr_inst_2 = %d;\n", P.tr_inst[2]); out += line;
+    std::snprintf(line, sizeof(line), "    static constexpr int tr_inst_3 = %d;\n", P.tr_inst[3]); out += line;
+    std::snprintf(line, sizeof(line), "    static constexpr int tr_inst_4 = %d;\n", P.tr_inst[4]); out += line;
+    std::snprintf(line, sizeof(line), "    static constexpr int tr_inst_5 = %d;\n", P.tr_inst[5]); out += line;
+    std::snprintf(line, sizeof(line), "    static constexpr int tr_inst_6 = %d;\n", P.tr_inst[6]); out += line;
+    std::snprintf(line, sizeof(line), "    static constexpr int tr_inst_7 = %d;\n", P.tr_inst[7]); out += line;
+    std::snprintf(line, sizeof(line), "    static constexpr int tr_inst_8 = %d;\n", P.tr_inst[8]); out += line;
+    std::snprintf(line, sizeof(line), "    static constexpr int tr_inst_9 = %d;\n", P.tr_inst[9]); out += line;
+    std::snprintf(line, sizeof(line), "    static constexpr int tr_inst_10 = %d;\n", P.tr_inst[10]); out += line;
+    std::snprintf(line, sizeof(line), "    static constexpr int tr_inst_11 = %d;\n", P.tr_inst[11]); out += line;
+    std::snprintf(line, sizeof(line), "    static constexpr int tr_inst_12 = %d;\n", P.tr_inst[12]); out += line;
+    std::snprintf(line, sizeof(line), "    static constexpr int tr_inst_13 = %d;\n", P.tr_inst[13]); out += line;
+    std::snprintf(line, sizeof(line), "    static constexpr int tr_inst_14 = %d;\n", P.tr_inst[14]); out += line;
+    std::snprintf(line, sizeof(line), "    static constexpr int tr_inst_15 = %d;\n", P.tr_inst[15]); out += line;
+    std::snprintf(line, sizeof(line), "    static constexpr int tr_inst_16 = %d;\n", P.tr_inst[16]); out += line;
+    std::snprintf(line, sizeof(line), "    static constexpr int tr_inst_17 = %d;\n", P.tr_inst[17]); out += line;
+    std::snprintf(line, sizeof(line), "    static constexpr int tr_inst_18 = %d;\n", P.tr_inst[18]); out += line;
+    std::snprintf(line, sizeof(line), "    static constexpr int tr_inst_19 = %d;\n", P.tr_inst[19]); out += line;
+    std::snprintf(line, sizeof(line), "    static constexpr int tr_inst_20 = %d;\n", P.tr_inst[20]); out += line;
+    std::snprintf(line, sizeof(line), "    static constexpr int tr_inst_21 = %d;\n", P.tr_inst[21]); out += line;
+    std::snprintf(line, sizeof(line), "    static constexpr int tr_inst_22 = %d;\n", P.tr_inst[22]); out += line;
+    std::snprintf(line, sizeof(line), "    static constexpr int tr_inst_23 = %d;\n", P.tr_inst[23]); out += line;
+    std::snprintf(line, sizeof(line), "    static constexpr int tr_inst_24 = %d;\n", P.tr_inst[24]); out += line;
+    std::snprintf(line, sizeof(line), "    static constexpr int tr_inst_25 = %d;\n", P.tr_inst[25]); out += line;
+    std::snprintf(line, sizeof(line), "    static constexpr int tr_inst_26 = %d;\n", P.tr_inst[26]); out += line;
+    std::snprintf(line, sizeof(line), "    static constexpr int tr_inst_27 = %d;\n", P.tr_inst[27]); out += line;
+    std::snprintf(line, sizeof(line), "    static constexpr int tr_inst_28 = %d;\n", P.tr_inst[28]); out += line;
+    std::snprintf(line, sizeof(line), "    static constexpr int tr_inst_29 = %d;\n", P.tr_inst[29]); out += line;
+    std::snprintf(line, sizeof(line), "    static constexpr int tr_inst_30 = %d;\n", P.tr_inst[30]); out += line;
+    std::snprintf(line, sizeof(line), "    static constexpr int tr_inst_31 = %d;\n", P.tr_inst[31]); out += line;
+    std::snprintf(line, sizeof(line), "    static constexpr int tr_inst_32 = %d;\n", P.tr_inst[32]); out += line;
+    std::snprintf(line, sizeof(line), "    static constexpr int tr_inst_33 = %d;\n", P.tr_inst[33]); out += line;
+    std::snprintf(line, sizeof(line), "    static constexpr int tr_inst_34 = %d;\n", P.tr_inst[34]); out += line;
+    std::snprintf(line, sizeof(line), "    static constexpr int tr_inst_35 = %d;\n", P.tr_inst[35]); out += line;
+    std::snprintf(line, sizeof(line), "    static constexpr int tr_inst_36 = %d;\n", P.tr_inst[36]); out += line;
+    std::snprintf(line, sizeof(line), "    static constexpr int tr_inst_37 = %d;\n", P.tr_inst[37]); out += line;
+    std::snprintf(line, sizeof(line), "    static constexpr int tr_inst_38 = %d;\n", P.tr_inst[38]); out += line;
+    std::snprintf(line, sizeof(line), "    static constexpr int tr_inst_39 = %d;\n", P.tr_inst[39]); out += line;
+    std::snprintf(line, sizeof(line), "    static constexpr int tr_inst_40 = %d;\n", P.tr_inst[40]); out += line;
+    std::snprintf(line, sizeof(line), "    static constexpr int tr_inst_41 = %d;\n", P.tr_inst[41]); out += line;
+    std::snprintf(line, sizeof(line), "    static constexpr int tr_inst_42 = %d;\n", P.tr_inst[42]); out += line;
+    std::snprintf(line, sizeof(line), "    static constexpr int tr_inst_43 = %d;\n", P.tr_inst[43]); out += line;
+    std::snprintf(line, sizeof(line), "    static constexpr int tr_inst_44 = %d;\n", P.tr_inst[44]); out += line;
+    std::snprintf(line, sizeof(line), "    static constexpr int tr_inst_45 = %d;\n", P.tr_inst[45]); out += line;
+    std::snprintf(line, sizeof(line), "    static constexpr int tr_inst_46 = %d;\n", P.tr_inst[46]); out += line;
+    std::snprintf(line, sizeof(line), "    static constexpr int tr_inst_47 = %d;\n", P.tr_inst[47]); out += line;
+    std::snprintf(line, sizeof(line), "    static constexpr int tr_inst_48 = %d;\n", P.tr_inst[48]); out += line;
+    std::snprintf(line, sizeof(line), "    static constexpr int tr_inst_49 = %d;\n", P.tr_inst[49]); out += line;
+    std::snprintf(line, sizeof(line), "    static constexpr int tr_inst_50 = %d;\n", P.tr_inst[50]); out += line;
+    std::snprintf(line, sizeof(line), "    static constexpr int tr_inst_51 = %d;\n", P.tr_inst[51]); out += line;
+    std::snprintf(line, sizeof(line), "    static constexpr int tr_inst_52 = %d;\n", P.tr_inst[52]); out += line;
+    std::snprintf(line, sizeof(line), "    static constexpr int tr_inst_53 = %d;\n", P.tr_inst[53]); out += line;
+    std::snprintf(line, sizeof(line), "    static constexpr int tr_inst_54 = %d;\n", P.tr_inst[54]); out += line;
+    std::snprintf(line, sizeof(line), "    static constexpr int tr_inst_55 = %d;\n", P.tr_inst[55]); out += line;
+    std::snprintf(line, sizeof(line), "    static constexpr int tr_inst_56 = %d;\n", P.tr_inst[56]); out += line;
+    std::snprintf(line, sizeof(line), "    static constexpr int tr_inst_57 = %d;\n", P.tr_inst[57]); out += line;
+    std::snprintf(line, sizeof(line), "    static constexpr int tr_inst_58 = %d;\n", P.tr_inst[58]); out += line;
+    std::snprintf(line, sizeof(line), "    static constexpr int tr_inst_59 = %d;\n", P.tr_inst[59]); out += line;
+    std::snprintf(line, sizeof(line), "    static constexpr int tr_inst_60 = %d;\n", P.tr_inst[60]); out += line;
+    std::snprintf(line, sizeof(line), "    static constexpr int tr_inst_61 = %d;\n", P.tr_inst[61]); out += line;
+    std::snprintf(line, sizeof(line), "    static constexpr int tr_inst_62 = %d;\n", P.tr_inst[62]); out += line;
+    std::snprintf(line, sizeof(line), "    static constexpr int tr_inst_63 = %d;\n", P.tr_inst[63]); out += line;
+    std::snprintf(line, sizeof(line), "    static constexpr int tr_inst_64 = %d;\n", P.tr_inst[64]); out += line;
+    std::snprintf(line, sizeof(line), "    static constexpr int tr_inst_65 = %d;\n", P.tr_inst[65]); out += line;
+    std::snprintf(line, sizeof(line), "    static constexpr int tr_inst_66 = %d;\n", P.tr_inst[66]); out += line;
+    std::snprintf(line, sizeof(line), "    static constexpr int tr_inst_67 = %d;\n", P.tr_inst[67]); out += line;
+    std::snprintf(line, sizeof(line), "    static constexpr int tr_inst_68 = %d;\n", P.tr_inst[68]); out += line;
+    std::snprintf(line, sizeof(line), "    static constexpr int tr_inst_69 = %d;\n", P.tr_inst[69]); out += line;
+    std::snprintf(line, sizeof(line), "    static constexpr int tr_inst_70 = %d;\n", P.tr_inst[70]); out += line;
+    std::snprintf(line, sizeof(line), "    static constexpr int tr_inst_71 = %d;\n", P.tr_inst[71]); out += line;
+    std::snprintf(line, sizeof(line), "    static constexpr int tr_inst_72 = %d;\n", P.tr_inst[72]); out += line;
+    std::snprintf(line, sizeof(line), "    static constexpr int tr_inst_73 = %d;\n", P.tr_inst[73]); out += line;
+    std::snprintf(line, sizeof(line), "    static constexpr int tr_inst_74 = %d;\n", P.tr_inst[74]); out += line;
+    std::snprintf(line, sizeof(line), "    static constexpr int tr_inst_75 = %d;\n", P.tr_inst[75]); out += line;
+    std::snprintf(line, sizeof(line), "    static constexpr int tr_inst_76 = %d;\n", P.tr_inst[76]); out += line;
+    std::snprintf(line, sizeof(line), "    static constexpr int tr_inst_77 = %d;\n", P.tr_inst[77]); out += line;
+    std::snprintf(line, sizeof(line), "    static constexpr int tr_inst_78 = %d;\n", P.tr_inst[78]); out += line;
+    std::snprintf(line, sizeof(line), "    static constexpr int tr_inst_79 = %d;\n", P.tr_inst[79]); out += line;
+    out += "    struct tr_inst_t { __host__ __device__ constexpr int operator[](int i) const { return i == 0 ? tr_inst_0 : i == 1 ? tr_inst_1 : i == 2 ? tr_inst_2 : i == 3 ? tr_inst_3 : i == 4 ? tr_inst_4 : i == 5 ? tr_inst_5 : i == 6 ? tr_inst_6 : i == 7 ? tr_inst_7 : i == 8 ? tr_inst_8 : i == 9 ? tr_inst_9 : i == 10 ? tr_inst_10 : i == 11 ? tr_inst_11 : i == 12 ? tr_inst_12 : i == 13 ? tr_inst_13 : i == 14 ? tr_inst_14 : i == 15 ? tr_inst_15 : i == 16 ? tr_inst_16 : i == 17 ? tr_inst_17 : i == 18 ? tr_inst_18 : i == 19 ? tr_inst_19 : i == 20 ? tr_inst_20 : i == 21 ? tr_inst_21 : i == 22 ? tr_inst_22 : i == 23 ? tr_inst_23 : i == 24 ? tr_inst_24 : i == 25 ? tr_inst_25 : i == 26 ? tr_inst_26 : i == 27 ? tr_inst_27 : i == 28 ? tr_inst_28 : i == 29 ? tr_inst_29 : i == 30 ? tr_inst_30 : i == 31 ? tr_inst_31 : i == 32 ? tr_inst_32 : i == 33 ? tr_inst_33 : i == 34 ? tr_inst_34 : i == 35 ? tr_inst_35 : i == 36 ? tr_inst_36 : i == 37 ? tr_inst_37 : i == 38 ? tr_inst_38 : i == 39 ? tr_inst_39 : i == 40 ? tr_inst_40 : i == 41 ? tr_inst_41 : i == 42 ? tr_inst_42 : i == 43 ? tr_inst_43 : i == 44 ? tr_inst_44 : i == 45 ? tr_inst_45 : i == 46 ? tr_inst_46 : i == 47 ? tr_inst_47 : i == 48 ? tr_inst_48 : i == 49 ? tr_inst_49 : i == 50 ? tr_inst_50 : i == 51 ? tr_inst_51 : i == 52 ? tr_inst_52 : i == 53 ? tr_inst_53 : i == 54 ? tr_inst_54 : i == 55 ? tr_inst_55 : i == 56 ? tr_inst_56 : i == 57 ? tr_inst_57 : i == 58 ? tr_inst_58 : i == 59 ? tr_inst_59 : i == 60 ? tr_inst_60 : i == 61 ? tr_inst_61 : i == 62 ? tr_inst_62 : i == 63 ? tr_inst_63 : i == 64 ? tr_inst_64 : i == 65 ? tr_inst_65 : i == 66 ? tr_inst_66 : i == 67 ? tr_inst_67 : i == 68 ? tr_inst_68 : i == 69 ? tr_inst_69 : i == 70 ? tr_inst_70 : i == 71 ? tr_inst_71 : i == 72 ? tr_inst_72 : i == 73 ? tr_inst_73 : i == 74 ? tr_inst_74 : i == 75 ? tr_inst_75 : i == 76 ? tr_inst_76 : i == 77 ? tr_inst_77 : i == 78 ? tr_inst_78 : tr_inst_79; } };\n";
+    out += "    static constexpr tr_inst_t tr_inst{};\n";
     if (P.level_off) { std::snprintf(line, sizeof(line), "    static constexpr const int *level_off = spec_ipool + %zu;\n", (size_t)(P.level_off - H.ipool.data())); out += line; }
     else out += "    static constexpr const int *level_off = nullptr;\n";
     if (P.lvl_joints) { std::snprintf(line, sizeof(line), "    static constexpr const int *lvl_joints = spec_ipool + %zu;\n", (size_t)(P.lvl_joints - H.ipool.data())); out += line; }
@@ -540,5 +650,17 @@
     else out += "    static constexpr const int *fb_abx = nullptr;\n";
     if (P.fb_lane) { std::snprintf(line, sizeof(line), "    static constexpr const int *fb_lane = spec_ipool + %zu;\n", (size_t)(P.fb_lane - H.ipool.data())); out += line; }
     else out += "    static constexpr const int *fb_lane = nullptr;\n";
+    if (P.tr_joint) { std::snprintf(line, sizeof(line), "    static constexpr const int *tr_joint = spec_ipool + %zu;\n", (size_t)(P.tr_joint - H.ipool.data())); out += line; }
+    else out += "    static constexpr const int *tr_joint = nullptr;\n";
+    if (P.tr_src) { std::snprintf(line, sizeof(line), "    static constexpr const int *tr_src = spec_ipool + %zu;\n", (size_t)(P.tr_src - H.ipool.data())); out += line; }
+    else out += "    static constexpr const int *tr_src = nullptr;\n";
+    if (P.tr_sj) { std::snprintf(line, sizeof(line), "    static constexpr const int *tr_sj = spec_ipool + %zu;\n", (size_t)(P.tr_sj - H.ipool.data())); out += line; }
+    else out += "    static constexpr const int *tr_sj = nullptr;\n";
+    if (P.tr_sched) { std::snprintf(line, sizeof(line), "    static constexpr const int *tr_sched = spec_ipool + %zu;\n", (size_t)(P.tr_sched - H.ipool.data())); out += line; }
+    else out += "    static constexpr const int *tr_sched = nullptr;\n";
+    if (P.tr_const) { std::snprintf(line, sizeof(line), "    static constexpr const double *tr_const = spec_dpool + %zu;\n", (size_t)(P.tr_const - H.dpool.data())); out += line; }
+    else out += "    static constexpr const double *tr_const = nullptr;\n";
+    if (P.tr_prm) { std::snprintf(line, sizeof(line), "    static constexpr const double *tr_prm = spec_dpool + %zu;\n", (size_t)(P.tr_prm - H.dpool.data())); out += line; }
+    else out += "    static constexpr const double *tr_prm = nullptr;\n";
     out += "};\n";
 }
diff --git a/trep_amd/csrc/spec_kernel.hip b/trep_amd/csrc/spec_kernel.hip
--- a/trep_amd/csrc/spec_kernel.hip
+++ b/trep_amd/csrc/spec_kernel.hip
@@ -140,6 +140,7 @@
 }
 int tg_spec_waves(void) { return spec_waves<tg::MODE_DERIV2Z>(); }
 int tg_spec_fb_n(void) { return tg::tg_static_fb<SpecProg>::value ? SpecProg::fb_n : 0; }
+int tg_spec_tr_n(void) { return tg::tg_static_tr<SpecProg>::value ? SpecProg::tr_n : 0; }
 int tg_spec_modes(void) {
     int m = 1 << tg::MODE_ROLLOUT;
 #if defined(SPEC_DERIVATIVES)
diff --git a/trep_amd/csrc/trepamd.hip b/trep_amd/csrc/trepamd.hip
--- a/trep_amd/csrc/trepamd.hip
+++ b/trep_amd/csrc/trepamd.hip
@@ -82,7 +82,7 @@
     double *io_dev = nullptr;
     size_t io_in = 0, io_out = 0;
     bool mirror_valid = false;
-    int spec_modes = 0, spec_waves = 1, spec_fb_n = 0;
+    int spec_modes = 0, spec_waves = 1, spec_fb_n = 0, spec_tr_n = 0;
     std::string spec_path;
     tg::DeviceBuffer<int> d_ints;
     tg::DeviceBuffer<double> d_dbls;
@@ -1222,6 +1222,8 @@
     b->spec_waves = waves_fn ? waves_fn() : 1;
     auto fb_fn = reinterpret_cast<int (*)(void)>(dlsym(h, "tg_spec_fb_n"));
     b->spec_fb_n = fb_fn ? fb_fn() : 0;
+    auto tr_fn = reinterpret_cast<int (*)(void)>(dlsym(h, "tg_spec_tr_n"));
+    b->spec_tr_n = tr_fn ? tr_fn() : 0;
     auto par_fn = reinterpret_cast<int (*)(int, const tg::RunArgs *, tg::RunArgs *, int, size_t, void *, const double *, int, int)>(dlsym(h, "tg_spec_launch_par"));
     auto par_modes_fn = reinterpret_cast<int (*)(void)>(dlsym(h, "tg_spec_par_modes"));
     b->spec_launch_par = par_modes_fn ? par_fn : nullptr;
@@ -1267,7 +1269,7 @@
     out[0] = b->spec_launch ? b->spec_modes : 0;
     for (int spec = 0; spec < 2; spec++) { out[2 - spec] = (int32_t)b->launched[0][spec].modes; out[4 - spec] = (int32_t)std::min<long long>(b->launched[0][spec].n, 0x7fffffff); }
     out[5] = b->exact_pivot; out[6] = b->sys->team; out[7] = b->spec_launch ? b->spec_waves : 1;
-    if (b->spec_launch) out[7] |= b->spec_fb_n << 8;
+    if (b->spec_launch) out[7] |= (b->spec_fb_n << 8) | ((b->spec_tr_n & 0xFF) << 16);
     return TG_SUCCESS;
 }
 
diff --git a/trep_amd/midpointvi.py b/trep_amd/midpointvi.py
--- a/trep_amd/midpointvi.py
+++ b/trep_amd/midpointvi.py
@@ -150,6 +150,7 @@
         kout = np.zeros(8, dtype=np.int32)
         _lib.check(self._L.tg_batch_info(self._h, kout.ctypes.data_as(_lib._c_ip)))
         d["fb_n"] = (int(kout[7]) >> 8) & 0xFF
+        d["tr_n"] = (int(kout[7]) >> 16) & 0xFF
         return d
 
     MODES = {"rollout": 0, "calc_p2": 1, "calc_f": 2, "deriv1": 3, "deriv2z": 4}
@@ -193,7 +194,7 @@
         return {"spec_modes": names(out[0]), "spec_launched": names(out[1]), "generic_launched": names(out[2]),
                 "spec_launch_mask": int(out[1]), "generic_launch_mask": int(out[2]),
                 "spec_launches": int(out[3]), "generic_launches": int(out[4]), "exact_pivot": bool(out[5]), "team": int(out[6]),
-                "helper_waves": int(out[7]) & 0xFF, "fb_n": (int(out[7]) >> 8) & 0xFF, "spec_library": self._specialized,
+                "helper_waves": int(out[7]) & 0xFF, "fb_n": (int(out[7]) >> 8) & 0xFF, "tr_n": (int(out[7]) >> 16) & 0xFF, "spec_library": self._specialized,
                 "par_spec_modes": every(par[0]), "par_spec_launched": every(par[1]), "par_generic_launched": every(par[2]),
                 "par_spec_launches": int(par[3]), "par_generic_launches": int(par[4]), "parameter_rows": int(par[5]),
                 "parameter_group": int(par[6])}
```
